# gabegrand/VQA-Counterexamples

Hardware: AMD Instinct MI355X
Metric: VQA-CX triplets/sec (24 candidates each), NeuralCX training step (higher is better)
Workload: dtype f32; 1 GPU; configs[1]: NeuralCX MLP train step (fwd+listwise loss/recall+bwd+Adam), synthetic 2048-d feats, 24 candidates, batch 512 per GPU (weak scaling: global batch 512), H=256, L=1, dropout 0.25, fp32; global_batch=512, per_rank_batch=512, candidates=24, dim_h=256, n_layers=1, parallelism=dp1, feature_table_rows=82783

## Files before the change

include/neuralcx.h:

```cpp
#ifndef NEURALCX_H
#define NEURALCX_H

#include <stddef.h>
#include <stdint.h>

#ifdef __cplusplus
extern "C" {
#endif

#define NCX_OK            0
#define NCX_E_NULL       -1
#define NCX_E_DIMS       -2
#define NCX_E_WORKSPACE  -3
#define NCX_E_FLAGS      -4
#define NCX_E_UNSUPPORTED -5
#define NCX_E_COMM       -6

#define NCX_F_V_MULT   (1u << 0)
#define NCX_F_V_DIST   (1u << 1)
#define NCX_F_V_RANK   (1u << 2)
#define NCX_F_A_EMB    (1u << 3)
#define NCX_F_ALL      (NCX_F_V_MULT | NCX_F_V_DIST | NCX_F_V_RANK | NCX_F_A_EMB)
#define NCX_F_BF16     (1u << 4)
#define NCX_F_REUSE_GT (1u << 5)
// ... 52 lines not shown
size_t ncx_workspace_bytes(const ncx_dims* d);

int ncx_forward(const ncx_dims* d, const ncx_inputs* in, const ncx_params* p,
                void* workspace, size_t workspace_bytes, float* scores, void* stream);

#define NCX_FWD_ALL     0
#define NCX_FWD_PRELUDE 1
#define NCX_FWD_REST    2
int ncx_forward_phase(const ncx_dims* d, const ncx_inputs* in, const ncx_params* p,
                      void* workspace, size_t workspace_bytes, float* scores, int32_t phase, void* stream);

int ncx_loss_rank(const float* scores, const int32_t* gt, int32_t B, int32_t K, float scale,
                  float* loss_rows, float* loss, float* dscores, int32_t* rank, int32_t* hits,
                  void* stream);

int ncx_backward(const ncx_dims* d, const ncx_inputs* in, const ncx_params* p,
                 void* workspace, size_t workspace_bytes, const float* dscores,
                 const ncx_grads* g, void* stream);

int ncx_backward_phase(const ncx_dims* d, const ncx_inputs* in, const ncx_params* p,
                       void* workspace, size_t workspace_bytes, const float* dscores,
                       const ncx_grads* g, int32_t phase, void* stream);

#define NCX_WS_DGT 1
#define NCX_WS_H1 2
#define NCX_WS_DPRE1 3
#define NCX_WS_DE_PERM 4
#define NCX_WS_H2 5
#define NCX_WS_H3 6
#define NCX_WS_DPRE2 7
#define NCX_WS_XC 8
#define NCX_WS_WC 9
#define NCX_WS_GT 10
int ncx_ws_region(const ncx_dims* d, int32_t which, size_t* offset, size_t* bytes);

int ncx_train_tail(const ncx_dims* d, const ncx_params* p, void* workspace, size_t workspace_bytes, const int32_t* gt,
                   float* scores, float* loss_rows, float* loss, float* dscores, int32_t* rank, int32_t* hits,
                   const ncx_grads* g, void* stream);

#define NCX_COMM_ID_BYTES 128
typedef struct ncx_comm ncx_comm;
int ncx_comm_unique_id(void* id128);
int ncx_comm_create(const void* id128, int32_t nranks, int32_t rank, ncx_comm** out);
int ncx_comm_destroy(ncx_comm* comm);
int ncx_allreduce(ncx_comm* comm, float* buf, size_t n, void* stream);

int ncx_adam_step(float* param, const float* grad, float* exp_avg, float* exp_avg_sq, size_t n,
                  float lr, float beta1, float beta2, float eps, int32_t step, float grad_scale,
                  void* stream);

typedef struct ncx_adam_state {
    float* param; const float* grad; float* exp_avg; float* exp_avg_sq;
    size_t n, n_emb;
    int32_t step;
    float lr, beta1, beta2, eps, grad_scale;
} ncx_adam_state;
int ncx_backward_adam(const ncx_dims* d, const ncx_inputs* in, const ncx_params* p,
                      void* workspace, size_t workspace_bytes, const float* dscores,
                      const ncx_grads* g, const ncx_adam_state* opt, void* stream);

typedef struct ncx_mutan_params {
    const float* wv;  const float* bv;
    const float* wq;  const float* bq;
    const float* whv; const float* bhv;
    const float* whq; const float* bhq;
    const float* wc;  const float* bc;
    int32_t dhv, dhq, R;
    int32_t act_v, act_q;
} ncx_mutan_params;

size_t ncx_vqa_workspace_bytes(const ncx_dims* d, const ncx_mutan_params* m);

int ncx_vqa_forward(const ncx_dims* d, const float* feats, const int32_t* img_idx, const float* q_emb,
                    const ncx_mutan_params* m, void* workspace, size_t workspace_bytes,
                    float* z_orig, float* z_knns, float* a_knns, float* a_orig, void* stream);

typedef struct ncx_mlb_params {
    const float* wv;  const float* bv;
    const float* wq;  const float* bq;
    const float* wc;  const float* bc;
    int32_t dh;
    int32_t act_v, act_q, act_c;
} ncx_mlb_params;

size_t ncx_mlb_workspace_bytes(const ncx_dims* d, const ncx_mlb_params* m);

int ncx_mlb_forward(const ncx_dims* d, const float* feats, const int32_t* img_idx, const float* q_emb,
                    const ncx_mlb_params* m, void* workspace, size_t workspace_bytes,
                    float* z_orig, float* z_knns, float* a_knns, float* a_orig, void* stream);

typedef struct ncx_mlb_att_dims {
    int32_t B, P, dv, dq, dh_att, G, dh_f, A, n_img;
} ncx_mlb_att_dims;
typedef struct ncx_mlb_att_params {
    const float* wv_att; const float* bv_att;
    const float* wq_att; const float* bq_att;
    const float* wa;     const float* ba;
    const float* wg;     const float* bg;
    const float* wqf;    const float* bqf;
    const float* wc;     const float* bc;
    int32_t act_v_att, act_q_att, act_mm;
    int32_t act_v, act_q, act_c;
} ncx_mlb_att_params;

size_t ncx_mlb_att_workspace_bytes(const ncx_mlb_att_dims* d, const ncx_mlb_att_params* m);

int ncx_mlb_att_forward(const ncx_mlb_att_dims* d, const float* feats, const int32_t* img_idx, const float* q_emb,
                        const ncx_mlb_att_params* m, void* workspace, size_t workspace_bytes,
                        float* logits, float* att, void* stream);
int ncx_mlb_att_forward_flags(const ncx_mlb_att_dims* d, const float* feats, const int32_t* img_idx, const float* q_emb,
                              const ncx_mlb_att_params* m, uint32_t flags, void* workspace, size_t workspace_bytes,
                              float* logits, float* att, void* stream);
int ncx_mlb_att_logits_form(const ncx_mlb_att_dims* d, uint32_t flags);

size_t ncx_knn_status_offset(int32_t n);
size_t ncx_knn_workspace_bytes(int32_t n, int32_t block_rows);
int ncx_knn(const float* table, int32_t n, const float* queries, int32_t nq, int32_t dv, int32_t k,
            int32_t norms_ready, void* workspace, size_t workspace_bytes, int64_t* out_idx, float* out_dist,
            void* stream);

size_t ncx_cosine_gram_workspace_bytes(int32_t A, int32_t da);
int ncx_cosine_gram(const float* emb, int32_t A, int32_t da, void* ws, size_t ws_bytes, float* gram, void* stream);
int ncx_semantic_scores(const float* a_knns, const int32_t* aid, int32_t B, int32_t K, int32_t A, const float* gram,
                        float lam, float* scores, float* raw, int32_t* bad_id_flag, void* stream);

int ncx_similarity_scores(const float* feats, const int32_t* img_idx, int32_t n_img, int32_t dv,
                          const float* z_orig, const float* z_knns, int32_t dz,
                          const float* a_knns, const int32_t* aid, int32_t A,
                          int32_t B, int32_t K,
                          float* scores , float* parts ,
                          int32_t* bad_id_flag, void* stream);

size_t ncx_gru_packed_bytes(int32_t dim_emb, int32_t dim_q);
int ncx_gru_pack(const float* w_ih, const float* w_hh, const float* b_ih, const float* b_hh, int32_t dim_emb, int32_t dim_q,
                 float* packed, void* stream);
size_t ncx_gru_workspace_bytes(int32_t B, int32_t T, int32_t dim_emb, int32_t dim_q);
int ncx_gru_encode(const int32_t* wids, int32_t B, int32_t T, const float* E, int32_t V1, int32_t dim_emb, int32_t dim_q,
                   const float* packed, void* workspace, size_t workspace_bytes, float* q_out, int32_t* bad_id_flag, void* stream);
int ncx_gru_encode_flags(const int32_t* wids, int32_t B, int32_t T, const float* E, int32_t V1, int32_t dim_emb, int32_t dim_q,
                         const float* packed, uint32_t flags, void* workspace, size_t workspace_bytes, float* q_out, int32_t* bad_id_flag,
                         void* stream);
int ncx_gru_step_form(int32_t B, int32_t T, int32_t dim_emb, int32_t dim_q, uint32_t flags);

size_t ncx_gru_train_workspace_bytes(int32_t B, int32_t T, int32_t dim_emb, int32_t dim_q);
size_t ncx_gru_packed_t_bytes(int32_t dim_emb, int32_t dim_q);
int ncx_gru_pack_t(const float* w_ih, const float* w_hh, int32_t dim_emb, int32_t dim_q, float* packed_t, void* stream);
int ncx_gru_train_forward(const int32_t* wids, int32_t B, int32_t T, const float* E, int32_t V1, int32_t dim_emb, int32_t dim_q,
                          const float* packed, void* workspace, size_t workspace_bytes, float* q_out, int32_t* bad_id_flag, void* stream);
int ncx_gru_train_forward_flags(const int32_t* wids, int32_t B, int32_t T, const float* E, int32_t V1, int32_t dim_emb, int32_t dim_q,
                                const float* packed, uint32_t flags, void* workspace, size_t workspace_bytes, float* q_out,
                                int32_t* bad_id_flag, void* stream);
int ncx_gru_train_backward(const int32_t* wids, int32_t B, int32_t T, const float* E, int32_t V1, int32_t dim_emb, int32_t dim_q,
                           const float* packed_t, void* workspace, size_t workspace_bytes, const float* dq_out,
                           float* dW_ih, float* dW_hh, float* db_ih, float* db_hh, float* dE , void* stream);
int ncx_gru_train_backward_flags(const int32_t* wids, int32_t B, int32_t T, const float* E, int32_t V1, int32_t dim_emb, int32_t dim_q,
                                 const float* packed_t, uint32_t flags, void* workspace, size_t workspace_bytes, const float* dq_out,
                                 float* dW_ih, float* dW_hh, float* db_ih, float* db_hh, float* dE , void* stream);
int ncx_gru_bwd_form(int32_t B, int32_t T, int32_t dim_emb, int32_t dim_q, uint32_t flags);

size_t ncx_lstm2_packed_bytes(int32_t emb, int32_t H);
int ncx_lstm2_pack(const float* w_ih0, const float* w_hh0, const float* b_ih0, const float* b_hh0, const float* w_ih1, const float* w_hh1,
                   const float* b_ih1, const float* b_hh1, int32_t emb, int32_t H, float* packed, void* stream);
size_t ncx_lstm2_workspace_bytes(int32_t B, int32_t T, int32_t emb, int32_t H);
int ncx_lstm2_encode(const int32_t* wids, int32_t B, int32_t T, const float* E, int32_t V1, int32_t emb, int32_t H, const float* packed,
                     void* workspace, size_t workspace_bytes, float* q_out, int32_t* bad_id_flag, void* stream);
int ncx_lstm2_encode_flags(const int32_t* wids, int32_t B, int32_t T, const float* E, int32_t V1, int32_t emb, int32_t H, const float* packed,
                           uint32_t flags, void* workspace, size_t workspace_bytes, float* q_out, int32_t* bad_id_flag, void* stream);
int ncx_lstm2_step_form(int32_t B, int32_t T, int32_t emb, int32_t H, uint32_t flags);

size_t ncx_lstm2_train_workspace_bytes(int32_t B, int32_t T, int32_t emb, int32_t H);
size_t ncx_lstm2_packed_t_bytes(int32_t emb, int32_t H);
int ncx_lstm2_pack_t(const float* w_ih0, const float* w_hh0, const float* w_ih1, const float* w_hh1, int32_t emb, int32_t H, float* packed_t,
                     void* stream);
int ncx_lstm2_train_forward(const int32_t* wids, int32_t B, int32_t T, const float* E, int32_t V1, int32_t emb, int32_t H, const float* packed,
                            void* workspace, size_t workspace_bytes, float* q_out, int32_t* bad_id_flag, void* stream);
int ncx_lstm2_train_forward_flags(const int32_t* wids, int32_t B, int32_t T, const float* E, int32_t V1, int32_t emb, int32_t H,
                                  const float* packed, uint32_t flags, void* workspace, size_t workspace_bytes, float* q_out,
                                  int32_t* bad_id_flag, void* stream);
int ncx_lstm2_train_backward(const int32_t* wids, int32_t B, int32_t T, const float* E, int32_t V1, int32_t emb, int32_t H, const float* packed_t,
                             void* workspace, size_t workspace_bytes, const float* dq_out, float* dW_ih0, float* dW_hh0, float* db_ih0,
                             float* db_hh0, float* dW_ih1, float* dW_hh1, float* db_ih1, float* db_hh1, float* dE , void* stream);

typedef struct ncx_scorer_dims {
    int32_t B, K, dv, dq, dz, A, n_img;
} ncx_scorer_dims;

typedef struct ncx_pairlin_params {
    const float* answer_embedding;
    const float* w;  const float* b;
    const float* w_out; const float* b_out;
} ncx_pairlin_params;
typedef struct ncx_pairlin_grads {
    float* answer_embedding; float* w; float* b; float* w_out; float* b_out;
} ncx_pairlin_grads;

size_t ncx_pairlin_workspace_bytes(const ncx_scorer_dims* d);
int ncx_pairlin_forward(const ncx_scorer_dims* d, const ncx_inputs* in, const ncx_pairlin_params* p, void* workspace,
                        size_t workspace_bytes, float* scores, int32_t* bad_id_flag, void* stream);
int ncx_pairlin_backward(const ncx_scorer_dims* d, const ncx_inputs* in, const ncx_pairlin_params* p, void* workspace,
                         size_t workspace_bytes, const float* dscores, const ncx_pairlin_grads* g, void* stream);
size_t ncx_linctx_workspace_bytes(const ncx_scorer_dims* d);
int ncx_linctx_forward(const ncx_scorer_dims* d, const float* z_knns, const float* w, const float* b, void* workspace,
                       size_t workspace_bytes, float* scores, void* stream);
int ncx_linctx_backward(const ncx_scorer_dims* d, const float* z_knns, const float* dscores, void* workspace,
                        size_t workspace_bytes, float* gw, float* gb, void* stream);

typedef struct ncx_contrastive_dims {
    int32_t B, P, dv, dz, n_img;
} ncx_contrastive_dims;
size_t ncx_contrastive_workspace_bytes(const ncx_contrastive_dims* d);
int ncx_contrastive_forward(const ncx_contrastive_dims* d, const ncx_inputs* in, const float* w, const float* b, void* workspace,
                            size_t workspace_bytes, float* h, int32_t* bad_id_flag, void* stream);
int ncx_contrastive_distances(const ncx_contrastive_dims* d, const float* h, void* workspace, size_t workspace_bytes, float* dist,
                              void* stream);
int ncx_contrastive_loss(const ncx_contrastive_dims* d, void* workspace, size_t workspace_bytes, float margin, float scale,
                         float* losses4, float* dist, void* stream);
int ncx_contrastive_backward(const ncx_contrastive_dims* d, const ncx_inputs* in, void* workspace, size_t workspace_bytes,
                             const float* dh, float* gw, float* gb, void* stream);

typedef struct ncx_vqa_train_dims {
    int32_t B, dv, dq, dz, A, n_img;
    float   p_v, p_q, p_c;
    int32_t dropout_mode;
    int32_t want_dq;
    int32_t pad_;
    uint64_t seed;
} ncx_vqa_train_dims;
typedef struct ncx_mutan_grads {
    float* wv;  float* bv;  float* wq;  float* bq;  float* whv; float* bhv; float* whq; float* bhq; float* wc;  float* bc;
} ncx_mutan_grads;
size_t ncx_vqa_train_workspace_bytes(const ncx_vqa_train_dims* d, const ncx_mutan_params* m);
int ncx_vqa_train_forward(const ncx_vqa_train_dims* d, const float* feats, const int32_t* img_idx, const float* q_emb,
                          const ncx_mutan_params* m, const float* masks, void* workspace, size_t workspace_bytes,
                          float* logits, float* z, void* stream);
int ncx_ce_loss(const float* logits, const int32_t* target, int32_t B, int32_t A, float scale, float* loss, float* dlogits,
                int32_t* hits_top1, int32_t* hits_top5, int32_t* bad_flag, float* rows, void* stream);
int ncx_vqa_train_backward(const ncx_vqa_train_dims* d, const ncx_mutan_params* m, const float* masks, void* workspace,
                           size_t workspace_bytes, const float* dlogits, const ncx_mutan_grads* g, float* dq_emb, void* stream);
#define NCX_VT_WS_VD 1
#define NCX_VT_WS_QD 2
#define NCX_VT_WS_ZC 3
int ncx_vqa_train_ws_region(const ncx_vqa_train_dims* d, const ncx_mutan_params* m, int32_t which, size_t* offset, size_t* bytes);

typedef struct ncx_mlb_grads {
    float* wv;  float* bv;  float* wq;  float* bq;  float* wc;  float* bc;
} ncx_mlb_grads;
size_t ncx_mlb_train_workspace_bytes(const ncx_vqa_train_dims* d, const ncx_mlb_params* m);
int ncx_mlb_train_forward(const ncx_vqa_train_dims* d, const float* feats, const int32_t* img_idx, const float* q_emb,
                          const ncx_mlb_params* m, const float* masks, void* workspace, size_t workspace_bytes,
                          float* logits, float* z, void* stream);
int ncx_mlb_train_backward(const ncx_vqa_train_dims* d, const ncx_mlb_params* m, const float* masks, void* workspace,
                           size_t workspace_bytes, const float* dlogits, const ncx_mlb_grads* g, float* dq_emb, void* stream);
int ncx_mlb_train_ws_region(const ncx_vqa_train_dims* d, const ncx_mlb_params* m, int32_t which, size_t* offset, size_t* bytes);

typedef struct ncx_mlb_att_train {
    float    p_att_v, p_att_q, p_att_mm, p_v, p_q, p_c;
    int32_t  dropout_mode;
    int32_t  want_dq;
    uint64_t seed;
} ncx_mlb_att_train;
typedef struct ncx_mlb_att_grads {
    float* wv_att; float* bv_att; float* wq_att; float* bq_att; float* wa; float* ba;
    float* wg;     float* bg;     float* wqf;    float* bqf;    float* wc; float* bc;
} ncx_mlb_att_grads;
size_t ncx_mlb_att_train_workspace_bytes(const ncx_mlb_att_dims* d, const ncx_mlb_att_train* t, const ncx_mlb_att_params* m);
int ncx_mlb_att_train_forward(const ncx_mlb_att_dims* d, const ncx_mlb_att_train* t, const float* feats, const int32_t* img_idx,
                              const float* q_emb, const ncx_mlb_att_params* m, const float* masks, void* workspace,
                              size_t workspace_bytes, float* logits, float* att, void* stream);
int ncx_mlb_att_train_forward_flags(const ncx_mlb_att_dims* d, const ncx_mlb_att_train* t, const float* feats, const int32_t* img_idx,
                                    const float* q_emb, const ncx_mlb_att_params* m, const float* masks, uint32_t flags, void* workspace,
                                    size_t workspace_bytes, float* logits, float* att, void* stream);
int ncx_mlb_att_train_backward(const ncx_mlb_att_dims* d, const ncx_mlb_att_train* t, const float* feats, const int32_t* img_idx,
                               const float* q_emb, const ncx_mlb_att_params* m, const float* masks, void* workspace,
                               size_t workspace_bytes, const float* att, const float* dlogits, const ncx_mlb_att_grads* g,
                               float* dq_emb, void* stream);
int ncx_mlb_att_train_backward_flags(const ncx_mlb_att_dims* d, const ncx_mlb_att_train* t, const float* feats, const int32_t* img_idx,
                                     const float* q_emb, const ncx_mlb_att_params* m, const float* masks, uint32_t flags, void* workspace,
                                     size_t workspace_bytes, const float* att, const float* dlogits, const ncx_mlb_att_grads* g,
                                     float* dq_emb, void* stream);
int ncx_mlb_att_dwv_form(const ncx_mlb_att_dims* d, uint32_t flags);
#define NCX_AT_WS_XV     1
#define NCX_AT_WS_VATT   2
#define NCX_AT_WS_T      3
#define NCX_AT_WS_VD     4
#define NCX_AT_WS_DWV    5
int ncx_mlb_att_train_ws_region(const ncx_mlb_att_dims* d, const ncx_mlb_att_train* t, const ncx_mlb_att_params* m, int32_t which,
                                size_t* offset, size_t* bytes);

#define NCX_GEMM_GT 0
#define NCX_GEMM_SH 1
#define NCX_GEMM_MAIN 2
#define NCX_GEMM_FWD_L 3
#define NCX_GEMM_DW1C 4
#define NCX_GEMM_DW1S 5
#define NCX_GEMM_DE 6
#define NCX_GEMM_DW1AK 7
#define NCX_GEMM_DAGT 8
#define NCX_GEMM_DWL 9
#define NCX_GEMM_DXL 10
#define NCX_QUERY_DW1_ROUTE 32
#define NCX_QUERY_FUSED_ADAM 33
#define NCX_QUERY_FWD_ROUTE 34
#define NCX_QUERY_BF16_ROUTE 35
int ncx_profile_begin(uint32_t gemm_mask , int32_t max_launches);
int ncx_profile_end(float* ms, int32_t* ids, int32_t cap);
int ncx_profile_stamps(unsigned long long* stamps, int64_t words);
int ncx_plan_query(const ncx_dims* d, int32_t gemm_id, int32_t* out6);
int ncx_bf16_layout(const ncx_dims* d, int32_t* out10);
int ncx_wgmap_check(int32_t tiles_m, int32_t tiles_n, int32_t S);

const char* ncx_version(void);

#ifdef __cplusplus
}
#endif
#endif
```

vqa-counterexamples_amd/csrc/ncx_diag.hip:

```cpp
#include "ncx_driver.h"
#include "ncx_bf16.h"
#include <stdlib.h>

using namespace ncx;
extern "C" {
int ncx_profile_begin(uint32_t gemm_mask, int32_t max_launches) {
    if (g_prof.on || gemm_mask == 0 || (gemm_mask >> U_COUNT) != 0 || max_launches < 1 || max_launches > 65536) return NCX_E_DIMS;
    g_prof.ev = (hipEvent_t*)malloc(sizeof(hipEvent_t) * 2 * (size_t)max_launches);
    g_prof.ids = (int*)malloc(sizeof(int) * (size_t)max_launches);
    if (!g_prof.ev || !g_prof.ids) return NCX_E_NULL;
    for (int i = 0; i < 2 * max_launches; ++i) NCX_HIP_TRY(hipEventCreate(&g_prof.ev[i]));
    g_prof.mask = gemm_mask; g_prof.n = 0; g_prof.cap = max_launches; g_prof.on = true;
    return NCX_OK;
}

int ncx_profile_end(float* ms, int32_t* ids, int32_t cap) {
    if (!g_prof.on) return NCX_E_FLAGS;
    int n = 0;
    for (int i = 0; i < g_prof.n; ++i) {
        if (hipEventSynchronize(g_prof.ev[2 * i + 1]) != hipSuccess) break;
        float t = 0.f;
        if (hipEventElapsedTime(&t, g_prof.ev[2 * i], g_prof.ev[2 * i + 1]) != hipSuccess) break;
        if (n < cap) { if (ms) ms[n] = t; if (ids) ids[n] = g_prof.ids[i]; }
        ++n;
    }
    for (int i = 0; i < 2 * g_prof.cap; ++i) (void)hipEventDestroy(g_prof.ev[i]);
    free(g_prof.ev); free(g_prof.ids);
    g_prof.ev = nullptr; g_prof.ids = nullptr; g_prof.on = false; g_prof.mask = 0; g_prof.n = 0; g_prof.cap = 0;
    return n < cap ? n : cap;
}

int ncx_profile_stamps(unsigned long long* stamps, int64_t words) {
    if ((stamps == nullptr) != (words == 0) || words < 0) return NCX_E_DIMS;
    int dev = 0;
    NCX_HIP_TRY(hipGetDevice(&dev));
    if (dev < 0 || dev >= 16) return NCX_E_DIMS;
    if (!stamps) { g_stamps[dev].ptr.store(nullptr, std::memory_order_release); g_stamps[dev].words.store(0, std::memory_order_release); }
    else { g_stamps[dev].ptr.store(nullptr, std::memory_order_release); g_stamps[dev].words.store(words, std::memory_order_release);
           g_stamps[dev].ptr.store(stamps, std::memory_order_release); }
    return NCX_OK;
}

int ncx_wgmap_check(int32_t tiles_m, int32_t tiles_n, int32_t S) {
    if (tiles_m < 1 || tiles_n < 1 || S < 1 || (long long)tiles_m * tiles_n * S > (1 << 24)) return NCX_E_DIMS;
    const WgMap w{tiles_m, tiles_n, S};
    const int total = tiles_m * tiles_n * S, count = w.count();
    if (count < total) return 1;
    unsigned char* seen = (unsigned char*)calloc((size_t)total, 1);
    if (!seen) return NCX_E_NULL;
    int bad = 0, nvalid = 0;
    for (int lw = 0; lw < count && !bad; ++lw) {
        int tm = -1, tn = -1, z = -1;
        if (!w.decode(lw, tm, tn, z)) continue;
        ++nvalid;
        if (tm < 0 || tm >= tiles_m || tn < 0 || tn >= tiles_n || z < 0 || z >= S) { bad = 2; break; }
        if (w.encode(tm, tn, z) != lw) { bad = 3; break; }
        unsigned char& f = seen[((size_t)z * tiles_m + tm) * tiles_n + tn];
        if (f) { bad = 4; break; }
        f = 1;
    }
    if (!bad && nvalid != total) bad = 5;
    free(seen);
    return bad;
}

int ncx_bf16_layout(const ncx_dims* d, int32_t* out10) {
    if (check_dims(d) != NCX_OK) return NCX_E_DIMS;
    if (!out10) return NCX_E_NULL;
    const Bf16Cols c = bf16_cols(*d);
    const int32_t v[10] = {c.c_vk, c.c_vm, c.c_misc, c.c_z, c.c_p, c.raw, c.kc, bf16_hp(*d), bf16_up128(d->da), bf16_up128(d->A)};
    for (int i = 0; i < 10; ++i) out10[i] = v[i];
    return NCX_OK;
}

int ncx_plan_query(const ncx_dims* d, int32_t gemm_id, int32_t* out6) {
    if (check_dims(d) != NCX_OK || !out6) return NCX_E_DIMS;
    if (gemm_id == NCX_QUERY_DW1_ROUTE) {
        const bool bf16 = d->flags & NCX_F_BF16;
        const StepRoutes r = routes(*d);
        out6[0] = r.km_form;
        out6[1] = (bf16 ? r.tn8_shared : r.tn8) ? (r.tn8_x6 ? 2 : 1) : 0;
        int grid = 0;
        out6[2] = dw_tn8_pieces(*d, bf16 ? TN8_LIST_SHARED : TN8_LIST_MAIN, &grid);
        out6[3] = grid;
        out6[4] = r.dw1ak_on_tn8(km_defers_to_side_stream(*d, r)) ? 1 : 0;
        out6[5] = TN8_MAX_SEG;
        return NCX_OK;
    }
    if (gemm_id == NCX_QUERY_FUSED_ADAM) {
        const bool on = fused_adam_route(*d, routes(*d)) && ((size_t)d->A * d->da) % 4 == 0;
        for (int i = 0; i < 6; ++i) out6[i] = 0;
        out6[0] = on ? 1 : 0;
        out6[1] = on ? main_adam_passengers() : 0;
        return NCX_OK;
    }
    if (gemm_id == NCX_QUERY_BF16_ROUTE) {
        for (int i = 0; i < 6; ++i) out6[i] = 0;
        if (!(d->flags & NCX_F_BF16)) { out6[0] = -1; return NCX_OK; }
        const Bf16Route b = bf16_route(*d);
        out6[0] = b.nt_form; out6[1] = b.tn8; out6[2] = b.S; out6[3] = b.chunk; out6[4] = b.nz; out6[5] = b.vec;
        return NCX_OK;
    }
    if (gemm_id == NCX_QUERY_FWD_ROUTE) {
        const StepRoutes r = routes(*d);
        GemmUse u[U_COUNT];
        list_uses(*d, r, u);
        const long long M = (long long)d->B * d->K;
        const bool bf16 = d->flags & NCX_F_BF16;
        for (int i = 0; i < 6; ++i) out6[i] = 0;
        if (bf16) out6[0] = 3;
        else if (main_fwd_dims_ok(*d)) {
            const FwdRoute f = forward_route(*d, r);
            const int sp = main_split(M, d->H, r.cand_ksteps);
            out6[0] = f.vfold ? 2 : 1;
            out6[1] = f.vfold ? main_fold_rows_eff(M, d->H, d->K) : main_chain_form(M, d->H, r.cand_ksteps, sp, false, true);
            out6[2] = sp;
            out6[3] = f.dist_in_main ? 1 : 0;
        } else { out6[1] = u[U_MAIN].plan.cfg; out6[2] = u[U_MAIN].plan.split; }
        if (d->L < 2) { out6[4] = -1; return NCX_OK; }
        if (hidden_fwd_dims_ok(*d) && !bf16) { out6[4] = 1; out6[5] = main_split(M, d->H, ksteps(d->H)); }
        else out6[5] = u[U_FWD_L].plan.split;
        return NCX_OK;
    }
    if (gemm_id < 0 || gemm_id >= U_COUNT) return NCX_E_DIMS;
    GemmUse u[U_COUNT];
    list_uses(*d, routes(*d), u);
    out6[0] = u[gemm_id].form; out6[1] = (int32_t)u[gemm_id].M; out6[2] = (int32_t)u[gemm_id].N;
    out6[3] = (int32_t)u[gemm_id].ksteps; out6[4] = u[gemm_id].plan.cfg; out6[5] = u[gemm_id].plan.split;
    const bool fast = (gemm_id == U_MAIN && main_fwd_dims_ok(*d)) || (gemm_id == U_FWD_L && hidden_fwd_dims_ok(*d) && !(d->flags & NCX_F_BF16));
    if (fast) {
        const long long M = (long long)d->B * d->K, T = u[gemm_id].ksteps;
        const int sp = main_split(M, d->H, T);
        const bool vfold = gemm_id == U_MAIN && (d->flags & NCX_F_V_MULT) && (d->K == 24 || (d->K == 48 && main_fold_rows(M, d->H) >= 96)) && d->dv % 32 == 0 && d->dv >= 64 && sp == 1;
        const long long tiles96 = ((M + 95) / 96) * ((d->H + 127) / 128);
        out6[4] = vfold ? (main_fold_rows(M, d->H) == 192 ? 8 : (main_fold_rows(M, d->H) == 96 || d->K == 48) ? 7 : 6) : (sp == 1 && tiles96 * 10 >= (long long)num_cus() * 9) ? CFG_96x128 : 5;
        out6[5] = sp;
    }
    return NCX_OK;
}
}
```

vqa-counterexamples_amd/csrc/ncx_forward.hip:

```cpp
#include "ncx_driver.h"
#include "ncx_wave.h"
#include "ncx_bf16.h"

namespace ncx {
__device__ __forceinline__ u16 f32_to_bf16(float x) { return __builtin_bit_cast(u16, (__bf16)x); }
__device__ __forceinline__ void store_bf16x4(u16* p, const float (&v)[4], int valid) {
    typedef unsigned short u16x4 __attribute__((ext_vector_type(4)));
    if (valid >= 4) { *(u16x4*)p = u16x4{f32_to_bf16(v[0]), f32_to_bf16(v[1]), f32_to_bf16(v[2]), f32_to_bf16(v[3])}; }
    else { for (int j = 0; j < valid; ++j) p[j] = f32_to_bf16(v[j]); }
}

struct PackArgs { const float* src[WPAD_N + 1]; float* dst[WPAD_N + 1]; long long lds[WPAD_N + 1]; int cols[WPAD_N + 1], ldd[WPAD_N + 1], zero_from[WPAD_N + 1]; int n, H; int nprep; };
__device__ __forceinline__ void pack_rows_block(const PackArgs& a, int idx) {
    const int h = idx % a.H, e = idx / a.H;
    float* drow = a.dst[e] + (long long)h * a.ldd[e];
    if (a.src[e]) {
        const float* srow = a.src[e] + (long long)h * a.lds[e];
        for (int c = threadIdx.x; c < a.cols[e]; c += 256) drow[c] = srow[c];
    }
    for (int c = a.zero_from[e] + threadIdx.x; c < a.ldd[e]; c += 256) drow[c] = 0.f;
}

template <bool RESIDENT>
__global__ __launch_bounds__(256) void k_prep(ncx_dims d, ncx_inputs in, int* __restrict__ idx_k,
                                              int* __restrict__ idx_o, int* __restrict__ idx_ob,
                                              float* __restrict__ mx, float* __restrict__ inv,
                                              float* __restrict__ misc, u16* __restrict__ xc, Bf16Cols cc, const PackArgs pk) {
    constexpr int NR = RESIDENT ? 8 : 1;
    const int lane = threadIdx.x & 63;
    const int M = d.B * d.K;
    const int nprep = pk.nprep;
    if ((int)blockIdx.x >= nprep) { pack_rows_block(pk, (int)blockIdx.x - nprep); return; }
    const int r = blockIdx.x * 4 + (threadIdx.x >> 6);
    if (r >= M) return;
    const int b = r / d.K, k = r - b * d.K;
    const bool aemb_ = d.flags & NCX_F_A_EMB;
    f32x4 ra[NR];
    if (RESIDENT && aemb_) {
        const float* arow = in.a_knns + (long long)r * d.A;
#pragma unroll
        for (int i = 0; i < NR; ++i) ra[i] = load_window(arow, lane * 4 + 256 * i, d.A);
    }
    const int io = in.img_idx[(long long)b * (d.K + 1)];
    const int ik = in.img_idx[(long long)b * (d.K + 1) + 1 + k];
    if (lane == 0) { idx_o[r] = io; idx_k[r] = ik; if (k == 0) idx_ob[b] = io; }
    const float* vo = in.feats + (long long)io * d.dv;
    const float* vk = in.feats + (long long)ik * d.dv;
    u16* xr = xc ? xc + (long long)r * cc.kc : nullptr;
    const bool own_dist = (d.flags & NCX_F_V_DIST) && !(d.flags & NCX_F_PRIV_DIST_IN_MAIN);
    const bool need_v = own_dist || xc;

    f32x4 ro[NR], rk[NR];
    if (RESIDENT && need_v) {
#pragma unroll
        for (int i = 0; i < NR; ++i) { ro[i] = load_window(vo, lane * 4 + 256 * i, d.dv); rk[i] = load_window(vk, lane * 4 + 256 * i, d.dv); }
        if (d.dv % 256 != 0) {
#pragma unroll
            for (int i = 0; i < NR; ++i) { ro[i] = fix_window(ro[i], lane * 4 + 256 * i, d.dv); rk[i] = fix_window(rk[i], lane * 4 + 256 * i, d.dv); }
        }
    }
    auto v_at = [&](int i, int c, f32x4& a, f32x4& e) __attribute__((always_inline)) {
        if (RESIDENT) { a = ro[i]; e = rk[i]; } else { a = load4(vo, c, d.dv); e = load4(vk, c, d.dv); }
    };
    float dist = 0.f;
    if (own_dist) {
        float s = 0.f;
        if (RESIDENT) {
#pragma unroll
            for (int i = 0; i < NR; ++i) {
                const int c = lane * 4 + 256 * i;
#pragma unroll
                for (int j = 0; j < 4; ++j)
                    if (c + j < d.dv) { const float t = ro[i][j] - rk[i][j] + 1e-6f; s += t * t; }
            }
        } else {
            for (int c = lane * 4; c < d.dv; c += 256) {
                f32x4 a, e; v_at(0, c, a, e);
#pragma unroll
                for (int j = 0; j < 4; ++j)
                    if (c + j < d.dv) { const float t = a[j] - e[j] + 1e-6f; s += t * t; }
            }
        }
        dist = sqrtf(wave_sum(s));
    }
    const int mw = pad_to(d.K + 1, 4);
    float* mrow = misc + (long long)r * mw;
    if (lane == 0) mrow[0] = dist;
    for (int j = lane; j < mw - 1; j += 64)
        mrow[1 + j] = j >= d.K ? 0.f : (d.flags & NCX_F_V_RANK) ? (j == k ? 1.f : 0.f) : in.v_rank[((long long)r) * d.K + j];
    if (xc) {
        if (RESIDENT) {
#pragma unroll
            for (int i = 0; i < NR; ++i) {
                const int c = lane * 4 + 256 * i;
                if (c < cc.c_vm) {
                    float pk[4], pm[4];
#pragma unroll
                    for (int j = 0; j < 4; ++j) { pk[j] = rk[i][j]; pm[j] = ro[i][j] * rk[i][j]; }
                    store_bf16x4(xr + cc.c_vk + c, pk, 4);
                    store_bf16x4(xr + cc.c_vm + c, pm, 4);
                }
            }
        } else {
            for (int c = lane * 4; c < cc.c_vm; c += 256) {
                f32x4 a, e; v_at(0, c, a, e);
                float pk[4], pm[4];
#pragma unroll
                for (int j = 0; j < 4; ++j) { pk[j] = e[j]; pm[j] = a[j] * e[j]; }
                store_bf16x4(xr + cc.c_vk + c, pk, 4);
                store_bf16x4(xr + cc.c_vm + c, pm, 4);
            }
        }
        for (int j = lane; j < cc.c_z - cc.c_misc; j += 64)
            xr[cc.c_misc + j] = f32_to_bf16(j == 0 ? dist : (j <= d.K && j - 1 == k ? 1.f : 0.f));
        const float* zk = in.z_knns + (long long)r * d.dz;
        for (int c = lane * 4; c < cc.c_p - cc.c_z; c += 256) {
            float pz[4];
            const f32x4 z4 = load4(zk, c, d.dz);
#pragma unroll
            for (int j = 0; j < 4; ++j) pz[j] = z4[j];
            store_bf16x4(xr + cc.c_z + c, pz, 4);
        }
        for (int c = cc.raw + lane; c < cc.kc; c += 64) xr[c] = 0;
    }

    if (d.flags & NCX_F_A_EMB) {
        const float* a = in.a_knns + (long long)r * d.A;
        if (RESIDENT && d.A % 256 != 0) {
#pragma unroll
            for (int i = 0; i < NR; ++i) ra[i] = fix_window(ra[i], lane * 4 + 256 * i, d.A);
        }
        float m = -INFINITY;
        if (RESIDENT) {
#pragma unroll
            for (int i = 0; i < NR; ++i)
#pragma unroll
                for (int j = 0; j < 4; ++j) if (lane * 4 + 256 * i + j < d.A) m = fmaxf(m, ra[i][j]);
        } else {
            for (int c = lane * 4; c < d.A; c += 256) {
                const f32x4 v = load4(a, c, d.A);
#pragma unroll
                for (int j = 0; j < 4; ++j) if (c + j < d.A) m = fmaxf(m, v[j]);
            }
        }
        m = wave_max(m);
        float s = 0.f;
        if (RESIDENT) {
#pragma unroll
            for (int i = 0; i < NR; ++i)
#pragma unroll
                for (int j = 0; j < 4; ++j) if (lane * 4 + 256 * i + j < d.A) s += __expf(ra[i][j] - m);
        } else {
            for (int c = lane * 4; c < d.A; c += 256) {
                const f32x4 v = load4(a, c, d.A);
#pragma unroll
                for (int j = 0; j < 4; ++j) if (c + j < d.A) s += __expf(v[j] - m);
            }
        }
        s = wave_sum(s);
        const float lse2 = m * 1.44269504088896341f + __log2f(s);
        if (lane == 0) { mx[r] = lse2; inv[r] = 0.f; }
        if (xc) {
            u16* xp = xr + cc.c_p;
            if (RESIDENT) {
#pragma unroll
                for (int i = 0; i < NR; ++i) {
                    const int c = lane * 4 + 256 * i;
                    if (c < d.A) {
                        float e[4];
#pragma unroll
                        for (int j = 0; j < 4; ++j) e[j] = __builtin_amdgcn_exp2f(__builtin_fmaf(ra[i][j], 1.44269504088896341f, -lse2));
                        store_bf16x4(xp + c, e, d.A - c);
                    }
                }
            } else {
                for (int c = lane * 4; c < d.A; c += 256) {
                    const f32x4 v = load4(a, c, d.A);
                    float e[4];
#pragma unroll
                    for (int j = 0; j < 4; ++j) e[j] = __builtin_amdgcn_exp2f(__builtin_fmaf(v[j], 1.44269504088896341f, -lse2));
                    store_bf16x4(xp + c, e, d.A - c);
                }
            }
        }
    }
}

__global__ __launch_bounds__(256) void k_scores(const float* __restrict__ h, const float* __restrict__ w,
                                                const float* __restrict__ bias, float* __restrict__ scores,
                                                int M, int H) {
    const int lane = threadIdx.x & 63;
    const int r = blockIdx.x * 4 + (threadIdx.x >> 6);
    if (r >= M) return;
    const float* row = h + (long long)r * H;
    float s = 0.f;
    for (int c = lane * 4; c < H; c += 256) {
        const f32x4 a = load4(row, c, H), e = load4(w, c, H);
        s += dot4(a, e);
    }
    s = wave_sum(s);
    if (lane == 0) scores[r] = s + bias[0];
}

FwdRoute forward_route(const ncx_dims& d, const StepRoutes& r) {
    const long long M = (long long)d.B * d.K, H = d.H, din = seg_offsets(d).din;
    const long long main_T = r.cand_ksteps;
    FwdRoute f{};
    f.vfold = main_fwd_dims_ok(d) && (d.flags & NCX_F_V_MULT) && (d.K == 24 || (d.K == 48 && (main_fold_rows(M, H) >= 96 || hook_env("NCX_FOLD4") || hook_env("NCX_FOLD8")))) && d.dv % 32 == 0 && d.dv >= 64 &&
              main_split(M, H, main_T) == 1 && !hook_env("NCX_NO_VFOLD") &&
              (long long)d.n_img * d.dv * 4 < (1ll << 32) - 65536 && (long long)H * din * 4 < (1ll << 32) - 65536;
    f.dist_in_fold = f.vfold && d.K == 24 && main_fold_rows_eff(M, H, d.K) >= 96 && !(d.flags & NCX_F_X6) && hook_env("NCX_DIST_IN_FOLD");
    f.dist_in_main = main_fwd_dims_ok(d) && (d.flags & NCX_F_V_DIST) && (d.flags & NCX_F_V_MULT) && d.dv % 32 == 0 &&
                     main_split(M, H, main_T) == 1 && (!f.vfold || f.dist_in_fold) && !(hook_env("NCX_NO_DIST_IN_MAIN"));
    return f;
}
}

using namespace ncx;
extern "C" {
const char* ncx_version(void) { return "neuralcx-hip gfx950 fp32-mfma r4 (" __DATE__ ")"; }

int64_t ncx_input_size(const ncx_dims* d) { return d ? (int64_t)seg_offsets(*d).din : 0; }

size_t ncx_workspace_bytes(const ncx_dims* d) {
    if (check_dims(d) != NCX_OK) return 0;
    return ws_layout(*d).total;
}

static int forward_impl(const ncx_dims* dp, const ncx_inputs* in, const ncx_params* p, void* workspace,
                        size_t workspace_bytes, float* scores, void* stream_, int phase) {
    int rc = check_dims(dp);
    if (rc != NCX_OK) return rc;
    const bool do_pre = phase != 2, do_rest = phase != 1;
    if (!in || !p || !workspace || (do_rest && !scores && !(dp->flags & NCX_F_FUSED_TAIL))) return NCX_E_NULL;
    const ncx_dims& d = *dp;
    const bool aemb = d.flags & NCX_F_A_EMB;
    if (!in->feats || !in->img_idx || !in->q_emb || !in->z_orig || !in->z_knns || !in->a_knns) return NCX_E_NULL;
    if (aemb && (!in->answer_aids || !p->answer_embedding)) return NCX_E_NULL;
    if (!aemb && !in->a_emb_gt) return NCX_E_FLAGS;
    if (!(d.flags & NCX_F_V_RANK) && !in->v_rank) return NCX_E_FLAGS;
    if (!p->w1 || !p->b1 || !p->w_out || !p->b_out) return NCX_E_NULL;
    if (d.L >= 2 && (!p->w2 || !p->b2)) return NCX_E_NULL;
    if (d.L >= 3 && (!p->w3 || !p->b3)) return NCX_E_NULL;
    const StepRoutes r = routes(d);
    const WsLayout w = ws_layout(d, r);
    if (workspace_bytes < w.total || ((uintptr_t)workspace & 255)) return NCX_E_WORKSPACE;
    hipStream_t s = (hipStream_t)stream_;
    char* ws = (char*)workspace;
    const int M = d.B * d.K, H = d.H;
    const SegOffsets o = seg_offsets(d);
    const long long din = o.din;
    int* idx_k = (int*)(ws + w.idx_k); int* idx_o = (int*)(ws + w.idx_o); int* idx_ob = (int*)(ws + w.idx_ob);
    float* mx = (float*)(ws + w.mx); float* inv = (float*)(ws + w.inv); float* misc = (float*)(ws + w.misc);
    float* gt = (float*)(ws + w.gt); float* sh = (float*)(ws + w.sh); float* slab = (float*)(ws + w.slab);
    GemmUse u[U_COUNT];
    list_uses(d, r, u);

    SideStream* ss = side_stream();
    if (ss && ss->mode == 3) ss = nullptr;
    hipStream_t s2 = ss ? ss->s : s;
    float* slab_side = ss ? (float*)(ws + w.slab2) : slab;
    const size_t slab_side_bytes = ss ? w.slab2_bytes : w.slab_bytes;
    if (ss) { rc = side_fork(ss, s); if (rc) return rc; }
    const bool bf16 = d.flags & NCX_F_BF16;
    u16* xc = bf16 ? (u16*)(ws + w.xc) : nullptr;
    struct { const float* ptr[WPAD_N]; int width[WPAD_N]; } wp{};
    PackArgs pk{}; pk.H = H;
    {
        const float* srcs[WPAD_N] = {p->w1 + o.v_other, p->w1 + o.v_mult, p->w1 + o.v_dist, p->w1 + o.z_other, p->w1 + o.a_other, p->w2, p->w3};
        float* cur = (float*)(ws + w.wpad);
        for (int i = 0; i < WPAD_N; ++i) {
            wp.width[i] = wpad_width(d, i); wp.ptr[i] = cur;
            if (!wp.width[i]) continue;
            const int e = pk.n++;
            pk.src[e] = srcs[i]; pk.lds[e] = (i == 5 || i == 6) ? H : din; pk.cols[e] = wpad_cols(d, i); pk.dst[e] = cur; pk.ldd[e] = wp.width[i]; pk.zero_from[e] = pk.cols[e];
            cur += (size_t)H * wp.width[i];
        }
        if (aemb && w.ldgt > d.A) { const int e = pk.n++; pk.src[e] = nullptr; pk.dst[e] = gt; pk.ldd[e] = w.ldgt; pk.zero_from[e] = d.A; pk.cols[e] = 0; }
        if (d.flags & NCX_F_REUSE_GT) pk.n = 0;
    }
    const FwdRoute fr = forward_route(d, r);
    const bool vfold = fr.vfold, dist_in_main = fr.dist_in_main;
    ncx_dims dprep = d;
    if (dist_in_main) dprep.flags |= NCX_F_PRIV_DIST_IN_MAIN;
    if (!do_rest) pk.n = 0;
    pk.nprep = do_pre ? (int)cdiv(M, 4) : 0;
    const unsigned prep_grid = (unsigned)(pk.nprep + (long long)H * pk.n);
    if (prep_grid > 0) {
        if (d.dv <= 2048 && d.A <= 2048)
            hipLaunchKernelGGL(k_prep<true>, dim3(prep_grid), dim3(256), 0, s, dprep, *in, idx_k, idx_o, idx_ob, mx, inv, misc, xc, bf16_cols(d), pk);
        else
            hipLaunchKernelGGL(k_prep<false>, dim3(prep_grid), dim3(256), 0, s, dprep, *in, idx_k, idx_o, idx_ob, mx, inv, misc, xc, bf16_cols(d), pk);
        NCX_HIP_TRY(hipGetLastError());
    }
    if (!do_rest) {
        if (ss) { rc = side_join(ss, s); if (rc) return rc; }
        return NCX_OK;
    }

    FixupArgs fix_gt{}, fix_sh{};
    const bool merge_fix = !ss && !bf16 && aemb && !(d.flags & NCX_F_REUSE_GT) && u[U_GT].plan.cfg == u[U_SH].plan.cfg &&
                           !hook_env("NCX_NO_MERGE_FIX");
    if (aemb && bf16 && !(d.flags & NCX_F_REUSE_GT)) {
        const Bf16Emb m = bf16_emb_layout(d, ws + w.bf_emb);
        rc = bf16_pack_embedding(d, p->answer_embedding, p->w1, m, s2); if (rc) return rc;
        rc = profiled(U_GT, s2, [&] { return bf16_gt(d, m, gt, s2); }); if (rc) return rc;
    } else if (aemb && !(d.flags & NCX_F_REUSE_GT)) {
        GemmArgs a{}; a.mode = MODE_CHAIN; a.nseg = 1; a.M = H;
        a.a[0] = x_plain(p->w1 + o.a_other, din, H, d.da);
        a.b[0] = x_plain(p->answer_embedding, d.da, d.A, d.da);
        a.klen[0] = d.da; a.out[0] = gt; a.ldo[0] = w.ldgt; a.n_cols[0] = d.A;
        if (merge_fix) a.defer_fix = &fix_gt;
        rc = run_gemm(U_GT, a, FORM_NT, u[U_GT].plan, merge_fix ? (float*)(ws + w.slab2) : slab_side,
                      merge_fix ? w.slab2_bytes : slab_side_bytes, nullptr, s2);
        if (rc) return rc;
    }
    {
        GemmArgs a{}; a.mode = MODE_CHAIN; a.nseg = 4; a.M = d.B;
        a.a[0] = ss ? x_gather_strided(in->feats, d.dv, in->img_idx, d.K + 1, d.B, d.dv)
                    : x_gather(in->feats, d.dv, idx_ob, d.B, d.dv);
        a.b[0] = x_plain(p->w1 + o.v_orig, din, H, d.dv); a.klen[0] = d.dv;
        a.a[1] = x_plain(in->q_emb, d.dq, d.B, d.dq);            a.b[1] = x_plain(p->w1 + o.q_emb, din, H, d.dq);  a.klen[1] = d.dq;
        a.a[2] = x_plain(in->z_orig, d.dz, d.B, d.dz);           a.b[2] = x_plain(p->w1 + o.z_orig, din, H, d.dz); a.klen[2] = d.dz;
        a.a[3] = aemb ? x_gather(p->answer_embedding, d.da, in->answer_aids, d.B, d.da)
                      : x_plain(in->a_emb_gt, d.da, d.B, d.da);
        a.b[3] = x_plain(p->w1 + o.a_gt, din, H, d.da); a.klen[3] = d.da;
        a.out[0] = sh; a.ldo[0] = H; a.n_cols[0] = H;
        if (merge_fix) a.defer_fix = &fix_sh;
        rc = run_gemm(U_SH, a, FORM_NT, u[U_SH].plan, slab_side, slab_side_bytes, p->b1, s2);
        if (rc) return rc;
        if (merge_fix) { rc = run_fixup2(fix_gt, fix_sh, u[U_SH].plan.cfg, s); if (rc) return rc; }
        if (ss) { rc = side_join(ss, s); if (rc) return rc; }
    }
    if (bf16) {
        rc = bf16_pack_wc(d, p->w1, gt, (u16*)(ws + w.wc), s); if (rc) return rc;
        EpiArgs e{};
        e.rowadd = sh; e.ld_rowadd = H; e.rowdiv = d.K;
        set_dropout(e, d, *in, 1, M);
        rc = profiled(U_MAIN, s, [&] { return bf16_main_forward(d, xc, (const u16*)(ws + w.wc), e, (float*)(ws + w.h[0]), s); }); if (rc) return rc;
    } else if (main_fwd_dims_ok(d)) {
        MainArgs a{}; a.M = M; a.N = H; a.x6 = (d.flags & NCX_F_X6) && !hook_env("NCX_NO_X6") && !hook_env("NCX_NO_MAIN_X6");
        int n = 0;
        auto seg = [&](int kind, const float* x, long long lda, int klen, const int* i1, const int* i2, const float* lse, int slot, const float* wgt, long long ldb) {
            MainSeg& g = a.seg[n++]; g.kind = kind; g.a = x; g.lda = lda; g.idx = i1; g.idx2 = i2; g.lse = lse; g.klen = klen;
            if (slot >= 0 && wp.width[slot]) { g.b = wp.ptr[slot]; g.ldb = wp.width[slot]; } else { g.b = wgt; g.ldb = ldb; } };
        if (vfold) {
            seg(MK_VFOLD, in->feats, d.dv, d.dv, idx_k, idx_o, nullptr, -1, p->w1 + o.v_other, din);
            a.seg[0].b2 = p->w1 + o.v_mult;
        } else {
            seg(MK_GATHER, in->feats, d.dv, d.dv, idx_k, nullptr, nullptr, 0, p->w1 + o.v_other, din);
            if (d.flags & NCX_F_V_MULT) seg(MK_GATHER_MUL, in->feats, d.dv, d.dv, idx_k, idx_o, nullptr, 1, p->w1 + o.v_mult, din);
        }
        seg(MK_PLAIN, misc, w.ldm, w.ldm, nullptr, nullptr, nullptr, 2, p->w1 + o.v_dist, din);
        seg(MK_PLAIN, in->z_knns, d.dz, d.dz, nullptr, nullptr, nullptr, 3, p->w1 + o.z_other, din);
        if (aemb) seg(MK_SOFTMAX, in->a_knns, d.A, d.A, nullptr, nullptr, mx, -1, gt, w.ldgt);
        else      seg(MK_PLAIN, in->a_knns, d.da, d.da, nullptr, nullptr, nullptr, 4, p->w1 + o.a_other, din);
        a.nseg = n;
        a.out = (float*)(ws + w.h[0]); a.ldo = H;
        a.epi.rowadd = sh; a.epi.ld_rowadd = H; a.epi.rowdiv = d.K;
        set_dropout(a.epi, d, *in, 1, M);
        if (dist_in_main) { a.dist_out = misc; a.ld_dist = w.ldm; }
        {
            long long T = 0; for (int i = 0; i < n; ++i) T += ksteps(a.seg[i].klen);
            a.split = main_split(M, H, T); a.slab = (float*)(ws + w.mslab);
            if (a.split > 1 && (size_t)a.split * M * H * 4 > w.mslab_bytes) return NCX_E_WORKSPACE;
        }
        if (a.split <= 1) a.stamps = stamps_for_current_device((long long)(((M + 47) / 48 + 7) / 8 * 8) * ((H + 63) / 64) * 16);
        rc = profiled(U_MAIN, s, [&] { return main_forward(a, s); }); if (rc) return rc;
    } else {
        GemmArgs a{}; a.mode = MODE_CHAIN; a.M = M;
        int n = 0;
        a.a[n] = x_gather(in->feats, d.dv, idx_k, M, d.dv); a.b[n] = x_plain(p->w1 + o.v_other, din, H, d.dv); a.klen[n] = d.dv; ++n;
        if (d.flags & NCX_F_V_MULT) {
            a.a[n] = x_gather_mul(in->feats, d.dv, idx_k, idx_o, M, d.dv); a.b[n] = x_plain(p->w1 + o.v_mult, din, H, d.dv); a.klen[n] = d.dv; ++n;
        }
        a.a[n] = x_plain(misc, w.ldm, M, d.K + 1); a.b[n] = x_plain(p->w1 + o.v_dist, din, H, d.K + 1); a.klen[n] = d.K + 1; ++n;
        a.a[n] = x_plain(in->z_knns, d.dz, M, d.dz); a.b[n] = x_plain(p->w1 + o.z_other, din, H, d.dz); a.klen[n] = d.dz; ++n;
        if (aemb) { a.a[n] = x_softmax(in->a_knns, d.A, mx, inv, M, d.A); a.b[n] = x_plain(gt, w.ldgt, H, d.A); a.klen[n] = d.A; ++n; }
        else      { a.a[n] = x_plain(in->a_knns, d.da, M, d.da); a.b[n] = x_plain(p->w1 + o.a_other, din, H, d.da); a.klen[n] = d.da; ++n; }
        a.nseg = n;
        a.out[0] = (float*)(ws + w.h[0]); a.ldo[0] = H; a.n_cols[0] = H;
        a.epi.rowadd = sh; a.epi.ld_rowadd = H; a.epi.rowdiv = d.K;
        set_dropout(a.epi, d, *in, 1, M);
        rc = run_gemm(U_MAIN, a, FORM_NT, u[U_MAIN].plan, slab, w.slab_bytes, nullptr, s);
        if (rc) return rc;
    }
    for (int l = 2; l <= d.L; ++l) {
        const float* wl = l == 2 ? p->w2 : p->w3;
        const float* bl = l == 2 ? p->b2 : p->b3;
        if (hidden_fwd_dims_ok(d) && !bf16) {
            MainArgs a{}; a.M = M; a.N = H; a.nseg = 1;
            MainSeg& g = a.seg[0]; g.kind = MK_PLAIN; g.a = (const float*)(ws + w.h[l - 2]); g.lda = H; g.klen = H;
            const int slot = 3 + l;
            if (wp.width[slot]) { g.b = wp.ptr[slot]; g.ldb = wp.width[slot]; } else { g.b = wl; g.ldb = H; }
            a.out = (float*)(ws + w.h[l - 1]); a.ldo = H;
            a.epi.bias = bl;
            set_dropout(a.epi, d, *in, l, M);
            a.split = main_split(M, H, ksteps(H)); a.slab = (float*)(ws + w.mslab);
            if (a.split > 1 && (size_t)a.split * M * H * 4 > w.mslab_bytes) return NCX_E_WORKSPACE;
            rc = profiled(U_FWD_L, s, [&] { return main_forward(a, s); }); if (rc) return rc;
        } else {
            GemmArgs a{}; a.mode = MODE_CHAIN; a.nseg = 1; a.M = M;
            a.a[0] = x_plain((const float*)(ws + w.h[l - 2]), H, M, H); a.b[0] = x_plain(wl, H, H, H); a.klen[0] = H;
            a.out[0] = (float*)(ws + w.h[l - 1]); a.ldo[0] = H; a.n_cols[0] = H;
            a.epi.bias = bl;
            set_dropout(a.epi, d, *in, l, M);
            rc = run_gemm(U_FWD_L, a, FORM_NT, u[U_FWD_L].plan, slab, w.slab_bytes, nullptr, s);
            if (rc) return rc;
        }
    }
    if (d.flags & NCX_F_FUSED_TAIL) return NCX_OK;
    hipLaunchKernelGGL(k_scores, dim3((unsigned)cdiv(M, 4)), dim3(256), 0, s, (const float*)(ws + w.h[d.L - 1]),
                       p->w_out, p->b_out, scores, M, H);
    NCX_HIP_TRY(hipGetLastError());
    return NCX_OK;
}

int ncx_forward(const ncx_dims* dp, const ncx_inputs* in, const ncx_params* p, void* workspace,
                size_t workspace_bytes, float* scores, void* stream_) {
    return forward_impl(dp, in, p, workspace, workspace_bytes, scores, stream_, 0);
}

int ncx_forward_phase(const ncx_dims* dp, const ncx_inputs* in, const ncx_params* p, void* workspace,
                      size_t workspace_bytes, float* scores, int32_t phase, void* stream_) {
    if (phase < 0 || phase > 2) return NCX_E_FLAGS;
    return forward_impl(dp, in, p, workspace, workspace_bytes, scores, stream_, phase);
}
}
```

vqa-counterexamples_amd/csrc/ncx_internal.h:

```cpp
#pragma once
#include "ncx_common.h"
#include "ncx_gemm.h"
#include "ncx_adam.h"

namespace ncx {

enum TileCfg : int { CFG_64x64 = 0, CFG_128x128 = 1, CFG_96x128 = 2, CFG_96x64 = 3, CFG_128x64 = 4 };
enum GemmForm : int { FORM_NT = 0, FORM_TN = 1, FORM_NN = 2 };

int run_gemm_nt(GemmArgs& a, int cfg, hipStream_t s);
int run_fixup2(const FixupArgs& a, const FixupArgs& b, int cfg, hipStream_t s);
int run_gemm_nt_fold(GemmArgs& a, hipStream_t s);
int run_gemm_tn(GemmArgs& a, int cfg, hipStream_t s);
int run_gemm_nn(GemmArgs& a, int cfg, hipStream_t s);
int occupancy_nt(int cfg);
int occupancy_tn(int cfg);
int occupancy_nn(int cfg);

struct SegOffsets {
    int v_orig, v_other, v_mult, v_dist, v_rank, q_emb, z_orig, z_other, a_gt, a_other, din;
};
static inline SegOffsets seg_offsets(const ncx_dims& d) {
    SegOffsets o; int c = 0;
    o.v_orig = c;  c += d.dv;
    o.v_other = c; c += d.dv;
    o.v_mult = c;  c += d.dv;
    o.v_dist = c;  c += 1;
    o.v_rank = c;  c += d.K;
    o.q_emb = c;   c += d.dq;
    o.z_orig = c;  c += d.dz;
    o.z_other = c; c += d.dz;
    o.a_gt = c;    c += d.da;
    o.a_other = c; c += d.da;
    o.din = c;
    return o;
}

struct GemmPlan { int cfg; int split; };
GemmPlan plan_gemm(int form, long long M, long long N, long long ksteps, bool allow_96);
int num_cus();
static inline long long cdiv(long long a, long long b) { return (a + b - 1) / b; }
static inline long long ksteps(long long k) { return cdiv(k, GEMM_BK); }
__attribute__((visibility("hidden"))) size_t gemm_slab_bytes(GemmArgs a, const GemmPlan& pl);
__attribute__((visibility("hidden"))) int run_gemm_planned(GemmArgs& a, int form, const GemmPlan& pl, float* slab, size_t slab_bytes,
                                                           const float* reduce_bias, hipStream_t s);
__attribute__((visibility("hidden"))) hipError_t colsum_rows(const float* in, long long ld, int R, int cols, float* out, hipStream_t s);

struct WsLayout {
    size_t idx_k, idx_o, idx_ob;
    size_t mx, inv;
    size_t misc;
    size_t gt;
    size_t sh;
    size_t h[3];
    size_t dpre[2];
    size_t dsh;
    size_t dgt;
    size_t dagt;
    size_t dgtT;
    size_t dgtT2;
    size_t de_perm;
    size_t w1aT;
    size_t partial;
    size_t slab;
    size_t slab_bytes;
    size_t slab2, slab2_bytes;
    size_t xc, wc, dpre_bf, bf_slab;
    size_t bf_emb;
    size_t km_slab;
    size_t mslab, mslab_bytes;
    size_t wpad;
    int ldm;
    int ldgt;
    size_t total;
};
constexpr int NCX_COLSUM_CHUNKS = 256;
constexpr int NCX_PRELUDE_WAVES = 1024;

enum MainKind : int { MK_PLAIN = 0, MK_GATHER = 1, MK_GATHER_MUL = 2, MK_SOFTMAX = 3,
                      MK_VFOLD = 4 };
constexpr int MAIN_MAX_SEG = 5;
struct MainSeg {
    const float* a;
    const int*   idx;
    const int*   idx2;
    const float* lse;
    const float* b;
    const float* b2;
    long long lda, ldb;
    int kind, klen;
};
struct MainArgs {
    MainSeg seg[MAIN_MAX_SEG]; int nseg, M, N, split; float* out; long long ldo; EpiArgs epi;
    float* slab;
    float* dist_out; long long ld_dist;
    unsigned long long* stamps;
    int x6;
    float* t_out; float* t_out0;
    AdamFuse adam;
};
int main_forward(MainArgs& a, hipStream_t s);
int main_forward_rowmap(MainArgs& a, hipStream_t s);
bool main_short_form(long long M, long long N, long long T, int split);
int main_chain_form(long long M, long long N, long long T, int split, bool single_gather, bool wide_ok);
int main_forward_adam(MainArgs& a, bool rowmap, hipStream_t s);
int main_adam_passengers();
int main_forward_mlb(MainArgs& a, hipStream_t s);
int main_split(long long M, long long N, long long T);
int main_fold_rows_eff(long long M, long long N, int rowdiv);
int main_fold_rows(long long M, long long N);

constexpr int DW_KM_SPLIT = 8;
bool dw_km_supported(const ncx_dims& d);
enum DwKmForm : int { KM_FORM_NONE = 0, KM_FORM_8 = 1, KM_FORM_X6 = 2, KM_FORM_GENERIC = 3, KM_FORM_GROUPED = 4 };
int dw_km_form(const ncx_dims& d);
size_t dw_km_slab_bytes(const ncx_dims& d);
int dw_km(const ncx_dims& d, const float* dpre, const float* feats, const int* idx_k, const int* idx_o, float* slab,
          float* g_vother, float* g_vmult, long long din, hipStream_t s, bool finish = true);
int dw_km_finish(const ncx_dims& d, const float* slab, float* g_vother, float* g_vmult, long long din, const FixupArgs* fix, int fix_cfg,
                 hipStream_t s);
constexpr int TN8_MAX_PROB = 8;
constexpr int TN8_MAX_SEG = 16;
struct Tn8Prob {
    const float* A;
    const float* X; long long ldx;
    const float* lse;
    int gsel;
    int rows, N;
    float* out; long long ldo; int n_valid;
    int rows_valid;
    float* outT; float* outT2; long long ldT; int padT2;
};
bool dw_tn8_supported(const ncx_dims& d);
bool dw_tn8_shapes_ok(const ncx_dims& d);
bool dw_tn8_shared_ok(const ncx_dims& d);
enum Tn8List : int { TN8_LIST_MAIN = 0, TN8_LIST_SHARED = 1, TN8_LIST_AK = 2 };
int dw_tn8_pieces(const ncx_dims& d, int list, int* grid);
bool dw_tn8_x6(const ncx_dims& d);
size_t dw_tn8_slab_bytes(const ncx_dims& d);
int dw_tn8(const ncx_dims& d, const Tn8Prob* probs, int np, int n_al, bool do_al, bool do_rest, const int* idx_ob, const int* aid,
           float* slab, size_t slab_bytes, hipStream_t s);
bool mutan_fold_supported(const ncx_dims& d, const ncx_mutan_params& m);
int mutan_fold(const ncx_dims& d, const ncx_mutan_params& m, const float* xv, const float* hq, float* z_orig, float* z_knns, hipStream_t s);
__attribute__((visibility("hidden"))) hipError_t pad_rows(const float* src, long long ld_src, int cols, float* dst, int ldd, int rows, hipStream_t s);
WsLayout ws_layout(const ncx_dims& d);
__host__ __device__ static inline int pad_to(int x, int m) { return (x + m - 1) / m * m; }
static inline bool main_fwd_extents_ok(const ncx_dims& d) {
    const long long lim = (1ll << 32) - 65536, M = (long long)d.B * d.K, wa = d.A > d.da ? d.A : d.da;
    return (long long)d.n_img * d.dv * 4 < lim && M * wa * 4 < lim && M * (long long)d.H * 4 < lim && M * (long long)d.dz * 4 < lim && (long long)d.A * wa * 4 < lim &&
           (long long)d.H * (2ll * d.dv + d.dq + 2ll * d.dz + 2ll * d.da + d.K + 2) * 4 < lim;
}
static inline bool main_fwd_dims_ok(const ncx_dims& d) {
    return d.dv % 4 == 0 && d.dz % 4 == 0 && ((d.flags & NCX_F_A_EMB) ? d.A : d.da) % 4 == 0 && !(d.flags & NCX_F_BF16) && main_fwd_extents_ok(d);
}
static inline bool hidden_fwd_dims_ok(const ncx_dims& d) { return d.H % 4 == 0 && main_fwd_extents_ok(d); }
constexpr uint32_t NCX_F_PRIV_DIST_IN_MAIN = 1u << 30;


}
```

vqa-counterexamples_amd/csrc/ncx_main.h:

```cpp
#pragma once
#include "ncx_internal.h"
#include "ncx_adam.h"
#include "ncx_x6.h"
#include <type_traits>

namespace ncx {

constexpr int MF_BK = 32, MF_P = MF_BK + 4, MF_T = 256;

enum { LK_PLAIN = 0, LK_MUL = 1, LK_SOFTMAX = 2 };
template <int V> struct IntC { static constexpr int value = V; };

constexpr int MF6_P = 80;
template <int BM_, int BN_, int WGM_, int WGN_, int DEPTH_, int OCC_, int T_ = MF_T, bool X6_ = false>
struct MainCfg {
    static constexpr int BM = BM_, BN = BN_, WGM = WGM_, WGN = WGN_, DEPTH = DEPTH_, OCC = OCC_, T = T_;
    static constexpr bool X6 = X6_;
    static constexpr int EPI = 0;
    static constexpr bool ADAM = false;
    static constexpr int RP = T / 8;
    static constexpr int BM_LDS = (BM + RP - 1) / RP * RP;
    static constexpr int LDS6 = 2 * 3 * (BM_LDS + BN) * MF6_P;
    static constexpr int LDS_FOLD6 = 2 * (3 * 208 * MF6_P + 8 * 32 * 4 + 128 * MF_P * 4);
    static constexpr int LDS_LOOP = 2 * (BM_LDS + BN) * MF_P * 4;
    static constexpr int LDS_STAGE = BM * (BN + 4) * 4;
    static constexpr int LDS32 = LDS_LOOP > LDS_STAGE ? LDS_LOOP : LDS_STAGE;
    static constexpr int LDS = !X6_ ? LDS32 : (LDS_FOLD6 > LDS6 ? (LDS_FOLD6 > LDS32 ? LDS_FOLD6 : LDS32) : (LDS6 > LDS32 ? LDS6 : LDS32));
    static constexpr int LDS_FOLD = BM % 96 == 0 ? 2 * (32 * (T / 64) + 128) * MF_P * 4
                                                 : 2 * (80 + 2 * 64) * MF_P * 4;
};

enum { EPI_STD = 0, EPI_MLB = 1, EPI_ROWMAP = 2 };
template <class CFG> struct WithMlbEpi : CFG { static constexpr int EPI = EPI_MLB; };
template <class CFG> struct WithRowMap : CFG { static constexpr int EPI = EPI_ROWMAP; };
template <class CFG> struct WithAdam : CFG { static constexpr bool ADAM = true; };

typedef const __attribute__((address_space(1))) float* gfptr;
typedef const __attribute__((address_space(1))) int* giptr;
typedef const __attribute__((address_space(1))) f32x4u* gf4ptr;

template <class CFG, bool DIST, int K0, int K1 = -1, int K2 = -1, int K3 = -1, int K4 = -1>
__global__ __launch_bounds__(CFG::T, CFG::OCC) void k_main_fwd(const MainArgs args) {
    constexpr bool VFOLD = K0 == MK_VFOLD;
    constexpr int DIST_SEG = VFOLD ? 1 : 2;
    static_assert(!DIST || (VFOLD ? K1 == MK_PLAIN : (K1 == MK_GATHER_MUL && K2 == MK_PLAIN)), "DIST: v_o, v_k segment followed by the dist | rank segment");
    static_assert(!VFOLD || (CFG::BM == 48 && CFG::BN == 64 && CFG::WGM == 1 && CFG::WGN == 4 && CFG::DEPTH == 2) ||
                            (CFG::BM == 96 && CFG::BN == 64 && CFG::WGM == 2 && CFG::WGN == 2 && CFG::DEPTH == 2) ||
                            (CFG::BM == 192 && CFG::BN == 64 && CFG::T == 512 && CFG::WGM == 4 && CFG::WGN == 2 && CFG::DEPTH == 2), "fold: 48 x 64, 96 x 64 or (8 waves) 192 x 64 tiles");
    static_assert(!(DIST && CFG::X6), "the X6 form leaves the distance to k_prep");
    constexpr int KS[6] = {K0, K1, K2, K3, K4, -1};
    constexpr int NSEG = K1 < 0 ? 1 : K2 < 0 ? 2 : K3 < 0 ? 3 : K4 < 0 ? 4 : 5;
    constexpr int BM = CFG::BM, BN = CFG::BN, BK = MF_BK, P = MF_P, DEPTH = CFG::DEPTH, BML = CFG::BM_LDS;
    constexpr int WTM = BM / CFG::WGM, WTN = BN / CFG::WGN, WM = WTM / 16, WN = WTN / 16, NSUB = BK / 8, NMF = 2 * WM * WN;
    constexpr int MT = CFG::T, RP = CFG::RP;
    static_assert(CFG::WGM * CFG::WGN == MT / 64 && WTM % 16 == 0 && WTN % 16 == 0 && BN % RP == 0 && NSUB == 4, "tile");
    static_assert(MT == 256 || !VFOLD || BM % 96 == 0, "the 48-row fold is a 256-thread form");
    constexpr int NA = BML / RP, NB = BN / RP;
    extern __shared__ __attribute__((aligned(16))) float mf_smem[];
    float* const lds_a = mf_smem;
    float* const lds_b = mf_smem + 2 * BML * P;
    const int tid = threadIdx.x, lane = tid & 63, wave = tid >> 6, li = lane & 15, lk = lane >> 4;
    const int wm0 = (wave / CFG::WGN) * WTM, wn0 = (wave % CFG::WGN) * WTN;
    const int M = args.M, N = args.N;
    const int tiles_m = (M + BM - 1) / BM, tiles_n = (N + BN - 1) / BN;
    const int S = args.split > 1 ? args.split : 1;
    int bid = blockIdx.x;
    if constexpr (CFG::ADAM) {
        const int pa = args.adam.pass_at, np = args.adam.n_pass;
        if (bid >= pa && bid < pa + np) { adam_passenger(args.adam, bid - pa, tid, MT); return; }
        if (bid >= pa + np) bid -= np;
    }
    const int id = bid, xcd = id & 7, local = id >> 3;
    const int tn = local % tiles_n, unit = (local / tiles_n) * 8 + xcd;
    if (unit >= tiles_m * S) return;
    const int tm = unit / S, z = unit - tm * S;
    const int m0 = tm * BM, n0 = tn * BN;
    const int quad = tid & 7, trow = tid >> 3;
    unsigned long long* const stamps = args.stamps ? args.stamps + (size_t)blockIdx.x * 16 : nullptr;
    auto stamp = [&](int slot) __attribute__((always_inline)) {
        if (stamps && tid == 0) stamps[slot] = __builtin_readcyclecounter();
    };
    if (stamps && tid == 0) { stamps[14] = __builtin_amdgcn_s_memrealtime(); stamps[13] = __builtin_amdgcn_s_getreg((3 << 11) | (0 << 6) | 20); }
    stamp(0);

    f32x4 acc[WM][WN];
#pragma unroll
    for (int i = 0; i < WM; ++i)
#pragma unroll
        for (int j = 0; j < WN; ++j) acc[i][j] = f32x4{0.f, 0.f, 0.f, 0.f};
    f32x2 afA[WM], bfA[WN], afB[WM], bfB[WN];
#pragma unroll
    for (int i = 0; i < WM; ++i) afB[i] = f32x2{0.f, 0.f};
#pragma unroll
    for (int j = 0; j < WN; ++j) bfB[j] = f32x2{0.f, 0.f};

    auto read_frags = [&](int buf, int s, f32x2 (&af)[WM], f32x2 (&bf)[WN]) __attribute__((always_inline)) {
        const float* a = lds_a + buf * BML * P + (wm0 + li) * P + 8 * s + 2 * lk;
        const float* b = lds_b + buf * BN * P + (wn0 + li) * P + 8 * s + 2 * lk;
#pragma unroll
        for (int i = 0; i < WM; ++i) af[i] = *(const f32x2*)(a + i * 16 * P);
#pragma unroll
        for (int j = 0; j < WN; ++j) bf[j] = *(const f32x2*)(b + j * 16 * P);
    };
    auto mfma = [&](const f32x2 (&af)[WM], const f32x2 (&bf)[WN]) __attribute__((always_inline)) {
#pragma unroll
        for (int e = 0; e < 2; ++e)
#pragma unroll
            for (int i = 0; i < WM; ++i)
#pragma unroll
                for (int j = 0; j < WN; ++j) acc[i][j] = __builtin_amdgcn_mfma_f32_16x16x4f32(af[i][e], bf[j][e], acc[i][j], 0, 0, 0);
    };

    constexpr bool X6 = CFG::X6;
    static_assert(!X6 || (VFOLD && BM == 192 && WM == 3 && WN == 2 && DEPTH == 2), "X6: the 8-wave 192 x 64 fold form only");
    constexpr int P6 = MF6_P, A6_PL = BML * P6, PL6 = (BML + BN) * P6, BUF6 = 3 * PL6;
    unsigned char* const lds6 = (unsigned char*)mf_smem;
    x6_bf16x8 xa[2][3], xb[2][X6 ? WN : 1][3];
    auto read_a6 = [&](int buf, int i, x6_bf16x8 (&f)[3]) __attribute__((always_inline)) {
        const unsigned char* a = lds6 + buf * BUF6 + (wm0 + 16 * i + li) * P6 + 16 * lk;
#pragma unroll
        for (int p = 0; p < 3; ++p) f[p] = *(const x6_bf16x8*)(a + p * PL6);
    };
    auto read_b6 = [&](int buf, x6_bf16x8 (&f)[X6 ? WN : 1][3]) __attribute__((always_inline)) {
        const unsigned char* b = lds6 + buf * BUF6 + A6_PL + (wn0 + li) * P6 + 16 * lk;
#pragma unroll
        for (int j = 0; j < (X6 ? WN : 1); ++j)
#pragma unroll
            for (int p = 0; p < 3; ++p) f[j][p] = *(const x6_bf16x8*)(b + j * 16 * P6 + p * PL6);
    };
    auto mfma6 = [&](const x6_bf16x8 (&a)[3], const x6_bf16x8 (&b)[X6 ? WN : 1][3], f32x4 (&c)[WN]) __attribute__((always_inline)) {
        if constexpr (X6) {
#pragma unroll
            for (int q = 0; q < 6; ++q)
#pragma unroll
                for (int j = 0; j < WN; ++j) c[j] = __builtin_amdgcn_mfma_f32_16x16x32_bf16(a[X6_A[q]], b[j][X6_B[q]], c[j], 0, 0, 0);
        }
    };

    int nsteps[MAIN_MAX_SEG], total_steps = 0;
#pragma unroll
    for (int i = 0; i < MAIN_MAX_SEG; ++i) { nsteps[i] = i < NSEG ? (args.seg[i].klen + BK - 1) / BK : 0; total_steps += nsteps[i]; }
    constexpr bool ROWMAP = CFG::EPI == EPI_ROWMAP;
    static_assert(!ROWMAP || (K0 == MK_GATHER && K1 == MK_GATHER && NSEG == 2 && !DIST && !X6), "row map: two gathered segments");
    const int g0 = (int)((long long)total_steps * z / S), g1_all = (int)((long long)total_steps * (z + 1) / S);
    const int g1 = [&]() __attribute__((always_inline)) {
        if constexpr (ROWMAP) return m0 >= ((giptr)args.seg[0].idx)[M] ? min(g1_all, nsteps[0]) : g1_all;
        else return g1_all;
    }();

    f32x4 va[DEPTH][NA], vm[DEPTH][NA], vb[DEPTH][NB];
    typedef unsigned int bu32x4 __attribute__((ext_vector_type(4)));
    __amdgpu_buffer_rsrc_t rsPA = __builtin_amdgcn_make_buffer_rsrc((void*)nullptr, 0, 0, 0x00020000), rsPB = rsPA;
    unsigned roA[NA], roM[NA], roB[NB]; float lse[NA];
    float dacc[NA];
    constexpr int FOLD_DIST_OFF = 2 * (BML + BN) * P > 32 * (MT / 64) * 68 ? 2 * (BML + BN) * P : 32 * (MT / 64) * 68;
#pragma unroll
    for (int i = 0; i < NA; ++i) dacc[i] = 0.f;
    auto setup = [&](auto kind_c, const MainSeg& g) __attribute__((always_inline)) {
        constexpr int KIND = decltype(kind_c)::value;
#pragma unroll
        for (int i = 0; i < NA; ++i) {
            const int r = min(m0 + min(trow + RP * i, BM - 1), M - 1);
            constexpr bool GAT = KIND == MK_GATHER || KIND == MK_GATHER_MUL;
            const unsigned row = GAT ? (unsigned)((giptr)g.idx)[r] : (unsigned)r;
            roA[i] = row * (unsigned)(g.lda * 4);
            roM[i] = KIND == MK_GATHER_MUL ? (unsigned)((giptr)g.idx2)[r] * (unsigned)(g.lda * 4) : roA[i];
            lse[i] = KIND == MK_SOFTMAX ? ((gfptr)g.lse)[r] : 0.f;
        }
#pragma unroll
        for (int i = 0; i < NB; ++i) roB[i] = (unsigned)min(n0 + trow + RP * i, N - 1) * (unsigned)(g.ldb * 4) + 16u * quad;
        rsPA = __builtin_amdgcn_make_buffer_rsrc(const_cast<float*>(g.a), 0, 0xFFFFFFF0u, 0x00020000);
        rsPB = __builtin_amdgcn_make_buffer_rsrc(const_cast<float*>(g.b), 0, 0xFFFFFFF0u, 0x00020000);
    };
    auto issue = [&](auto set_c, auto mul_c, int klen, int nst, int t) __attribute__((always_inline)) {
        constexpr int S = decltype(set_c)::value;
        const int tk4 = min(t, nst - 1) * (BK * 4);
        const unsigned ca4 = (unsigned)min(tk4 + 16 * quad, (klen - 4) * 4);
#pragma unroll
        for (int i = 0; i < NA; ++i) va[S][i] = __builtin_bit_cast(f32x4, (bu32x4)__builtin_amdgcn_raw_buffer_load_b128(rsPA, roA[i] + ca4, 0, 0));
        if (decltype(mul_c)::value) {
#pragma unroll
            for (int i = 0; i < NA; ++i) vm[S][i] = __builtin_bit_cast(f32x4, (bu32x4)__builtin_amdgcn_raw_buffer_load_b128(rsPA, roM[i] + ca4, 0, 0));
        }
#pragma unroll
        for (int i = 0; i < NB; ++i) vb[S][i] = __builtin_bit_cast(f32x4, (bu32x4)__builtin_amdgcn_raw_buffer_load_b128(rsPB, roB[i], tk4, 0));
    };
    typedef IntC<0> S0; typedef IntC<DEPTH - 1> S1;
    typedef std::true_type Tt; typedef std::false_type Ff;

    auto run_seg = [&](auto idx_c, const int t0, const int t1, const bool pf_next) __attribute__((always_inline)) {
        constexpr int I = decltype(idx_c)::value;
        constexpr int KIND = KS[I], NKIND = KS[I + 1];
        constexpr int LKIND = KIND == MK_GATHER_MUL ? LK_MUL : KIND == MK_SOFTMAX ? LK_SOFTMAX : LK_PLAIN;
        typedef std::integral_constant<bool, LKIND == LK_MUL> MULC;
        const MainSeg& sg = args.seg[I];
        const int klen = sg.klen;
        const int nst = (klen + BK - 1) / BK;
        float lse_c[NA];
#pragma unroll
        for (int i = 0; i < NA; ++i) lse_c[i] = lse[i];
        auto stash = [&](auto set_c, auto patch_c, int buf, int h0, int h1) __attribute__((always_inline)) {
            constexpr int S = decltype(set_c)::value;
            constexpr bool PATCH = decltype(patch_c)::value;
#pragma unroll
            for (int i = 0; i < NA; ++i) {
                if (i < h0 || i >= h1) continue;
                f32x4 v = va[S][i];
                if (DIST && LKIND == LK_MUL) {
                    const f32x4 df = vm[S][i] - va[S][i] + 1e-6f;
                    dacc[i] += (df[0] * df[0] + df[1] * df[1]) + (df[2] * df[2] + df[3] * df[3]);
                }
                if (PATCH) v[0] = quad == 0 ? dacc[i] : v[0];
                if (LKIND == LK_MUL) v = v * vm[S][i];
                if (LKIND == LK_SOFTMAX) {
#pragma unroll
                    for (int j = 0; j < 4; ++j) v[j] = __builtin_amdgcn_exp2f(__builtin_fmaf(v[j], 1.44269504088896341f, -lse_c[i]));
                }
                if constexpr (X6) x6_split_store(v, lds6 + buf * BUF6 + (trow + RP * i) * P6 + 8 * quad, PL6);
                else
                *(f32x4*)(lds_a + buf * BML * P + (trow + RP * i) * P + 4 * quad) = v;
            }
#pragma unroll
            for (int i = 0; i < NB; ++i) {
                if (i + NA < h0 || i + NA >= h1) continue;
                if constexpr (X6) x6_split_store(vb[S][i], lds6 + buf * BUF6 + A6_PL + (trow + RP * i) * P6 + 8 * quad, PL6);
                else
                *(f32x4*)(lds_b + buf * BN * P + (trow + RP * i) * P + 4 * quad) = vb[S][i];
            }
        };
        if constexpr (DIST && I == DIST_SEG) {
#pragma unroll
            for (int i = 0; i < NA; ++i) {
                if constexpr (VFOLD && BM % 96 == 0) {
                    dacc[i] = mf_smem[FOLD_DIST_OFF + min(trow + RP * i, BM - 1)];
                } else {
                float d2 = dacc[i];
                d2 += __shfl_xor(d2, 1, 64); d2 += __shfl_xor(d2, 2, 64); d2 += __shfl_xor(d2, 4, 64);
                dacc[i] = sqrtf(d2);
                }
                const int r = m0 + trow + RP * i;
                if (quad == 0 && tn == 0 && trow + RP * i < BM && r < M) args.dist_out[(long long)r * args.ld_dist] = dacc[i];
            }
            stash(S0{}, Tt{}, 0, 0, NA + NB);
        } else
        stash(S0{}, Ff{}, 0, 0, NA + NB);
        issue(S0{}, MULC{}, klen, nst, t0 + DEPTH);
        __syncthreads();

        auto step = [&](auto par_c, auto last_c, int t) __attribute__((always_inline)) {
            constexpr int PAR = decltype(par_c)::value;
            constexpr bool LAST = decltype(last_c)::value;
            typedef IntC<DEPTH == 2 ? (PAR ^ 1) : 0> SS;
            if constexpr (X6) {
                read_b6(PAR, xb[PAR]);
                read_a6(PAR, 0, xa[PAR]);
                mfma6(xa[PAR ^ 1], xb[PAR ^ 1], acc[2]);
#pragma unroll
                for (int q = 0; q < 6 * WN; ++q) { __builtin_amdgcn_sched_group_barrier(0x008, 1, 0); __builtin_amdgcn_sched_group_barrier(0x100, 1, 0); }
                __builtin_amdgcn_sched_barrier(0);
                if (LAST && NKIND >= 0 && pf_next) {
                    const MainSeg& nx = args.seg[I + 1 < MAIN_MAX_SEG ? I + 1 : I];
                    setup(IntC<NKIND>{}, nx);
                    const int kn = nx.klen, nn = (kn + BK - 1) / BK;
                    typedef std::integral_constant<bool, NKIND == MK_GATHER_MUL> NM;
                    issue(S0{}, NM{}, kn, nn, 0);
                    issue(S1{}, NM{}, kn, nn, 1);
                }
#pragma unroll
                for (int i = 0; i < 2; ++i) {
                    read_a6(PAR, i + 1, xa[PAR ^ 1 ^ i]);
                    if (!LAST) {
                        if (i == 0) stash(SS{}, Ff{}, PAR ^ 1, 0, (NA + NB) / 2);
                        if (i == 1) { stash(SS{}, Ff{}, PAR ^ 1, (NA + NB) / 2, NA + NB); issue(SS{}, MULC{}, klen, nst, t + 1 + DEPTH); }
                    }
                    mfma6(xa[PAR ^ i], xb[PAR], acc[i]);
#pragma unroll
                    for (int q = 0; q < 6 * WN; ++q) {
                        __builtin_amdgcn_sched_group_barrier(0x008, 1, 0);
                        __builtin_amdgcn_sched_group_barrier(0x100, 1, 0);
                        __builtin_amdgcn_sched_group_barrier(0x002, 4, 0);
                        __builtin_amdgcn_sched_group_barrier(0x200, 1, 0);
                        __builtin_amdgcn_sched_group_barrier(0x020, 1, 0);
                    }
                    __builtin_amdgcn_sched_barrier(0);
                }
                if (LAST) {
                    mfma6(xa[PAR], xb[PAR], acc[2]);
                    const x6_bf16x8 z8 = {0, 0, 0, 0, 0, 0, 0, 0};
#pragma unroll
                    for (int p = 0; p < 3; ++p) { xa[0][p] = z8; xa[1][p] = z8; }
                }
                __syncthreads();
                return;
            }
            read_frags(PAR, 0, afA, bfA);
            mfma(afB, bfB);
#pragma unroll
            for (int q = 0; q < NMF; ++q) { __builtin_amdgcn_sched_group_barrier(0x008, 1, 0); __builtin_amdgcn_sched_group_barrier(0x100, 1, 0); }
            __builtin_amdgcn_sched_barrier(0);
            if (LAST && NKIND >= 0 && pf_next) {
                const MainSeg& nx = args.seg[I + 1 < MAIN_MAX_SEG ? I + 1 : I];
                setup(IntC<NKIND>{}, nx);
                const int kn = nx.klen, nn = (kn + BK - 1) / BK;
                typedef std::integral_constant<bool, NKIND == MK_GATHER_MUL> NM;
                issue(S0{}, NM{}, kn, nn, 0);
                if (DEPTH == 2) issue(S1{}, NM{}, kn, nn, 1);
            }
#pragma unroll
            for (int s = 0; s < NSUB - 1; ++s) {
                auto& afc = (s & 1) ? afB : afA; auto& bfc = (s & 1) ? bfB : bfA;
                auto& afn = (s & 1) ? afA : afB; auto& bfn = (s & 1) ? bfA : bfB;
                read_frags(PAR, s + 1, afn, bfn);
                if (!LAST) {
                    if (s == 0) stash(SS{}, Ff{}, PAR ^ 1, 0, (NA + NB) / 2);
                    if (s == 1) stash(SS{}, Ff{}, PAR ^ 1, (NA + NB) / 2, NA + NB);
                    if (s == 2) issue(SS{}, MULC{}, klen, nst, t + 1 + DEPTH);
                }
                mfma(afc, bfc);
#pragma unroll
                for (int q = 0; q < NMF; ++q) {
                    __builtin_amdgcn_sched_group_barrier(0x008, 1, 0);
                    __builtin_amdgcn_sched_group_barrier(0x100, 1, 0);
                    __builtin_amdgcn_sched_group_barrier(0x002, 4, 0);
                    __builtin_amdgcn_sched_group_barrier(0x200, 1, 0);
                    __builtin_amdgcn_sched_group_barrier(0x020, 1, 0);
                }
                __builtin_amdgcn_sched_barrier(0);
            }
            __syncthreads();
        };
        typedef IntC<0> P0; typedef IntC<1> P1;
        int t = t0;
        for (; t + 2 < t1; t += 2) { step(P0{}, Ff{}, t); step(P1{}, Ff{}, t + 1); }
        if (t + 1 < t1) { step(P0{}, Ff{}, t); step(P1{}, Tt{}, t + 1); }
        else step(P0{}, Tt{}, t);
    };

    auto run_vfold = [&](const MainSeg& sg, const bool pf_next) __attribute__((always_inline)) {
        constexpr int AR = 80;
        float* const fa = mf_smem;
        float* const fb = mf_smem + 2 * AR * P;
        const int klen = sg.klen, nst = klen / BK;
        const int wr = wave >> 1, wc = wave & 1;
        gfptr pk[2], pwk[2], pwm[2], po[2];
        int lrow[2];
#pragma unroll
        for (int i = 0; i < 2; ++i) {
            const int rho = trow + 32 * i;
            const int r = min(m0 + min(rho, BM - 1), M - 1);
            pk[i] = (gfptr)sg.a + (long long)((giptr)sg.idx)[r] * sg.lda;
            lrow[i] = rho < 24 ? rho : rho < 48 ? rho + 8 : 64 + (rho - 48);
            const int n = min(n0 + trow + 32 * i, N - 1);
            pwk[i] = (gfptr)sg.b + (long long)n * sg.ldb;
            pwm[i] = (gfptr)sg.b2 + (long long)n * sg.ldb;
            po[i] = (gfptr)sg.a + (long long)((giptr)sg.idx2)[min(m0 + 24 * i, M - 1)] * sg.lda;
        }
        const int t_of0 = trow < 24 ? 0 : 1;
        f32x4 vk[2][2], vo[2][2], vwk[2][2], vwm[2][2];
        auto vissue = [&](auto set_c, int t) __attribute__((always_inline)) {
            constexpr int S = decltype(set_c)::value;
            const int c = min(t, nst - 1) * BK + 4 * quad;
#pragma unroll
            for (int i = 0; i < 2; ++i) {
#ifndef NCX_ABL_FOLD
                vk[S][i] = *(gf4ptr)(pk[i] + c); vo[S][i] = *(gf4ptr)(po[i] + c); vwk[S][i] = *(gf4ptr)(pwk[i] + c); vwm[S][i] = *(gf4ptr)(pwm[i] + c);
#else
                if (NCX_ABL_FOLD != 4 || t == 0) vk[S][i] = *(gf4ptr)(pk[i] + c);
                if (NCX_ABL_FOLD != 2 || t == 0) vo[S][i] = *(gf4ptr)(po[i] + c);
                if (NCX_ABL_FOLD != 3 || t == 0) vwk[S][i] = *(gf4ptr)(pwk[i] + c);
                if ((NCX_ABL_FOLD != 3 && NCX_ABL_FOLD != 1) || t == 0) vwm[S][i] = *(gf4ptr)(pwm[i] + c);
#endif
            }
        };
        auto vstash = [&](auto set_c, int buf, int part) __attribute__((always_inline)) {
            constexpr int S = decltype(set_c)::value;
            if (part == 0) {
#pragma unroll
                for (int i = 0; i < 2; ++i) {
                    if (DIST) {
                        const f32x4 ov = i == 0 ? (t_of0 == 0 ? vo[S][0] : vo[S][1]) : vo[S][1];
                        const f32x4 df = ov - vk[S][i] + 1e-6f;
                        dacc[i] += (df[0] * df[0] + df[1] * df[1]) + (df[2] * df[2] + df[3] * df[3]);
                    }
                    *(f32x4*)(fa + buf * AR * P + lrow[i] * P + 4 * quad) = vk[S][i];
                }
            }
#pragma unroll
// ... 228 lines not shown
                    __builtin_amdgcn_sched_group_barrier(0x100, 1, 0);
                    __builtin_amdgcn_sched_group_barrier(0x002, DIST ? 4 : 3, 0);
                    __builtin_amdgcn_sched_group_barrier(0x200, 1, 0);
                    __builtin_amdgcn_sched_group_barrier(0x020, 1, 0);
                }
                __builtin_amdgcn_sched_barrier(0);
            }
            __syncthreads();
        };
        int t = 0;
        for (; t + 2 < nst; t += 2) { vstep(V0{}, Ff{}, t); vstep(V1{}, Ff{}, t + 1); }
        if (t + 1 < nst) { vstep(V0{}, Ff{}, t); vstep(V1{}, Tt{}, t + 1); }
        else vstep(V0{}, Tt{}, t);
        fmfma(x1);
        if constexpr (DIST) {
#pragma unroll
            for (int i = 0; i < 3; ++i) {
                float d2 = dsum[i];
                d2 += __shfl_xor(d2, 1, 64); d2 += __shfl_xor(d2, 2, 64); d2 += __shfl_xor(d2, 4, 64);
                if (quad == 0) mf_smem[FOLD_DIST_OFF + 24 * wave + (lane >> 3) + 8 * i] = sqrtf(d2);
            }
        }
        constexpr int CP = 68;
        float* const fc = mf_smem;
#pragma unroll
        for (int i = 0; i < 2; ++i)
#pragma unroll
            for (int j = 0; j < 4; ++j)
#pragma unroll
                for (int q = 0; q < 4; ++q) fc[(32 * wave + 16 * i + 4 * lk + q) * CP + 16 * j + li] = acc4[i][j][q];
        __syncthreads();
#pragma unroll
        for (int i = 0; i < WM; ++i)
#pragma unroll
            for (int j = 0; j < WN; ++j)
#pragma unroll
                for (int q = 0; q < 4; ++q) {
                    const int rho = wm0 + 16 * i + 4 * lk + q;
                    acc[i][j][q] = fc[(blk * (rho / kr) + rho % kr) * CP + wn0 + 16 * j + li];
                }
        __syncthreads();
      }
    };

    auto run_vfold6 = [&](const MainSeg& sg, const bool pf_next) __attribute__((always_inline)) {
      if constexpr (X6) {
        constexpr int ARC = 208;
        constexpr int A_PLX = ARC * P6, VO_OFF = 3 * A_PLX, W_OFF = VO_OFF + 8 * 32 * 4, BUFX = W_OFF + 128 * P * 4;
        static_assert(2 * BUFX <= CFG::LDS, "fold tile (X6)");
        static_assert(RP == 64, "fold loader (X6)");
        const int klen = sg.klen, nst = klen / BK;
        const __amdgpu_buffer_rsrc_t rsA = __builtin_amdgcn_make_buffer_rsrc(const_cast<float*>(sg.a), 0, 0xFFFFFFF0u, 0x00020000);
        const __amdgpu_buffer_rsrc_t rsK = __builtin_amdgcn_make_buffer_rsrc(const_cast<float*>(sg.b), 0, 0xFFFFFFF0u, 0x00020000);
        const __amdgpu_buffer_rsrc_t rsM = __builtin_amdgcn_make_buffer_rsrc(const_cast<float*>(sg.b2), 0, 0xFFFFFFF0u, 0x00020000);
        typedef unsigned int bu32x4 __attribute__((ext_vector_type(4)));
        unsigned voA[3], voB;
#pragma unroll
        for (int i = 0; i < 3; ++i) voA[i] = (unsigned)((giptr)sg.idx)[min(m0 + trow + 64 * i, M - 1)] * (unsigned)(sg.lda * 4) + 16u * quad;
        const int vo_t = (tid >> 5) & 7, vo_c = tid & 31;
        const unsigned voV = (unsigned)((giptr)sg.idx2)[min(m0 + 24 * vo_t, M - 1)] * (unsigned)(sg.lda * 4) + 4u * vo_c;
        voB = (unsigned)min(n0 + trow, N - 1) * (unsigned)(sg.ldb * 4) + 16u * quad;
        f32x4 va4[2][3], vb4[2][2];
        float vv[2];
        auto vissue = [&](auto set_c, int t) __attribute__((always_inline)) {
            constexpr int SS_ = decltype(set_c)::value;
            const int so = min(t, nst - 1) * (BK * 4);
#pragma unroll
            for (int i = 0; i < 3; ++i) va4[SS_][i] = __builtin_bit_cast(f32x4, (bu32x4)__builtin_amdgcn_raw_buffer_load_b128(rsA, voA[i], so, 0));
            vv[SS_] = __builtin_bit_cast(float, (unsigned)__builtin_amdgcn_raw_buffer_load_b32(rsA, voV, so, 0));
            vb4[SS_][0] = __builtin_bit_cast(f32x4, (bu32x4)__builtin_amdgcn_raw_buffer_load_b128(rsK, voB, so, 0));
            vb4[SS_][1] = __builtin_bit_cast(f32x4, (bu32x4)__builtin_amdgcn_raw_buffer_load_b128(rsM, voB, so, 0));
        };
        auto cut4_fold = [&](const float (&x)[4], unsigned (&w1)[2], unsigned (&w2)[2], unsigned (&w3)[2]) __attribute__((always_inline)) {
            unsigned p1[4], p2[4], p3[4];
#pragma unroll
            for (int j = 0; j < 4; ++j) x6_cut1(x[j], p1[j], p2[j], p3[j]);
#pragma unroll
            for (int h = 0; h < 2; ++h) {
                w1[h] = __builtin_amdgcn_perm(p1[2 * h + 1], p1[2 * h], 0x07060302u);
                w2[h] = __builtin_amdgcn_perm(p2[2 * h + 1], p2[2 * h], 0x07060302u);
                w3[h] = __builtin_amdgcn_perm(p3[2 * h + 1], p3[2 * h], 0x07060302u);
            }
        };
        auto vstash = [&](auto set_c, int buf, int part) __attribute__((always_inline)) {
            constexpr int SS_ = decltype(set_c)::value;
            unsigned char* const bb = lds6 + buf * BUFX;
#pragma unroll
            for (int i = 0; i < 3; ++i) {
                if ((i < 2) != (part == 0) || part == 2) continue;
                const f32x4 v = va4[SS_][i];
                const float x[4] = {v[0], v[1], v[2], v[3]};
                unsigned w1[2], w2[2], w3[2];
                cut4_fold(x, w1, w2, w3);
                unsigned char* d = bb + (trow + 64 * i) * P6 + 8 * quad;
                *(x6_u32x2*)(d) = x6_u32x2{w1[0], w1[1]}; *(x6_u32x2*)(d + A_PLX) = x6_u32x2{w2[0], w2[1]}; *(x6_u32x2*)(d + 2 * A_PLX) = x6_u32x2{w3[0], w3[1]};
            }
            if (part == 1) *(float*)(bb + VO_OFF + (vo_t * 32 + vo_c) * 4) = vv[SS_];
            if (part == 2) {
#pragma unroll
                for (int i = 0; i < 2; ++i) *(f32x4*)(bb + W_OFF + ((trow + 64 * i) * P + 4 * quad) * 4) = vb4[SS_][i];
            }
        };
        f32x4 acc4[2][4];
#pragma unroll
        for (int i = 0; i < 2; ++i)
#pragma unroll
            for (int j = 0; j < 4; ++j) acc4[i][j] = f32x4{0.f, 0.f, 0.f, 0.f};
        struct Raw { f32x4 wk[2], wm[2]; };
        const x6_bf16x8 z8 = {0, 0, 0, 0, 0, 0, 0, 0};
        x6_bf16x8 af[2][2][3];
        x6_bf16x8 bq[2][3];
        f32x4 vo[2];
#pragma unroll
        for (int p = 0; p < 3; ++p) { af[1][0][p] = z8; af[1][1][p] = z8; bq[1][p] = z8; }
        auto read_af = [&](int buf, x6_bf16x8 (&f)[2][3]) __attribute__((always_inline)) {
            const unsigned char* a = lds6 + buf * BUFX + (24 * wave + li) * P6 + 16 * lk;
#pragma unroll
            for (int i = 0; i < 2; ++i)
#pragma unroll
                for (int p = 0; p < 3; ++p) f[i][p] = *(const x6_bf16x8*)(a + i * 16 * P6 + p * A_PLX);
        };
        auto read_vo = [&](int buf) __attribute__((always_inline)) {
            const unsigned char* v = lds6 + buf * BUFX + VO_OFF + (wave * 32 + 8 * lk) * 4;
            vo[0] = *(const f32x4*)(v); vo[1] = *(const f32x4*)(v + 16);
        };
        auto read_w = [&](int buf, int j, Raw& r) __attribute__((always_inline)) {
            const unsigned char* b = lds6 + buf * BUFX + W_OFF + ((16 * j + li) * P + 8 * lk) * 4;
            r.wk[0] = *(const f32x4*)(b); r.wk[1] = *(const f32x4*)(b + 16);
            r.wm[0] = *(const f32x4*)(b + 64 * P * 4); r.wm[1] = *(const f32x4*)(b + 64 * P * 4 + 16);
        };
        auto build = [&](const Raw& r, x6_bf16x8 (&o)[3]) __attribute__((always_inline)) {
            unsigned w1[4], w2[4], w3[4];
#pragma unroll
            for (int h = 0; h < 2; ++h) {
                float x[4];
#pragma unroll
                for (int e = 0; e < 4; ++e) { const float v_ = vo[h][e], m_ = r.wm[h][e], k_ = r.wk[h][e]; x[e] = __builtin_fmaf(v_, m_, k_); }
                unsigned a1[2], a2[2], a3[2];
                cut4_fold(x, a1, a2, a3);
                w1[2 * h] = a1[0]; w1[2 * h + 1] = a1[1]; w2[2 * h] = a2[0]; w2[2 * h + 1] = a2[1]; w3[2 * h] = a3[0]; w3[2 * h + 1] = a3[1];
            }
            typedef unsigned int mu32x4 __attribute__((ext_vector_type(4)));
            o[0] = __builtin_bit_cast(x6_bf16x8, mu32x4{w1[0], w1[1], w1[2], w1[3]});
            o[1] = __builtin_bit_cast(x6_bf16x8, mu32x4{w2[0], w2[1], w2[2], w2[3]});
            o[2] = __builtin_bit_cast(x6_bf16x8, mu32x4{w3[0], w3[1], w3[2], w3[3]});
        };
        auto fmfma = [&](const x6_bf16x8 (&a)[2][3], const x6_bf16x8 (&b)[3], int j) __attribute__((always_inline)) {
#pragma unroll
            for (int q = 0; q < 6; ++q)
#pragma unroll
                for (int i = 0; i < 2; ++i) acc4[i][j] = __builtin_amdgcn_mfma_f32_16x16x32_bf16(a[i][X6_A[q]], b[X6_B[q]], acc4[i][j], 0, 0, 0);
        };
        auto pin6 = [&]() __attribute__((always_inline)) {
#pragma unroll
            for (int q = 0; q < 12; ++q) {
                __builtin_amdgcn_sched_group_barrier(0x008, 1, 0);
                __builtin_amdgcn_sched_group_barrier(0x100, 1, 0);
                __builtin_amdgcn_sched_group_barrier(0x002, 5, 0);
                __builtin_amdgcn_sched_group_barrier(0x200, 1, 0);
                __builtin_amdgcn_sched_group_barrier(0x020, 1, 0);
            }
            __builtin_amdgcn_sched_barrier(0);
        };
        typedef IntC<0> V0; typedef IntC<1> V1;
        vissue(V0{}, 0);
        vissue(V1{}, 1);
        vstash(V0{}, 0, 0); vstash(V0{}, 0, 1); vstash(V0{}, 0, 2);
        vissue(V0{}, 2);
        __syncthreads();
        auto vstep = [&](auto par_c, auto last_c, int t) __attribute__((always_inline)) {
            constexpr int PAR = decltype(par_c)::value;
            constexpr bool LAST = decltype(last_c)::value;
            typedef IntC<PAR ^ 1> SS;
            Raw r0, r1;
            read_vo(PAR);
            read_w(PAR, 0, r0);
            read_af(PAR, af[PAR]);
            read_w(PAR, 1, r1);
            fmfma(af[PAR ^ 1], bq[1], 3);
            build(r0, bq[0]);
            pin6();
            if (LAST && pf_next) {
                const MainSeg& nx = args.seg[1];
                setup(IntC<K1 < 0 ? 0 : K1>{}, nx);
                const int kn = nx.klen, nn = (kn + BK - 1) / BK;
                issue(S0{}, Ff{}, kn, nn, 0);
                issue(S1{}, Ff{}, kn, nn, 1);
            }
            read_w(PAR, 2, r0);
            if (!LAST) vstash(SS{}, PAR ^ 1, 0);
            fmfma(af[PAR], bq[0], 0);
            build(r1, bq[1]);
            pin6();
            read_w(PAR, 3, r1);
            if (!LAST) vstash(SS{}, PAR ^ 1, 1);
            fmfma(af[PAR], bq[1], 1);
            build(r0, bq[0]);
            pin6();
            if (!LAST) { vstash(SS{}, PAR ^ 1, 2); vissue(SS{}, t + 3); }
            fmfma(af[PAR], bq[0], 2);
            build(r1, bq[1]);
            pin6();
            __syncthreads();
        };
        int t = 0;
        for (; t + 2 < nst; t += 2) { vstep(V0{}, Ff{}, t); vstep(V1{}, Ff{}, t + 1); }
        if (t + 1 < nst) { vstep(V0{}, Ff{}, t); vstep(V1{}, Tt{}, t + 1); fmfma(af[1], bq[1], 3); }
        else { vstep(V0{}, Tt{}, t); fmfma(af[0], bq[1], 3); }
        constexpr int CP = 68;
        float* const fc = mf_smem;
#pragma unroll
        for (int i = 0; i < 2; ++i)
#pragma unroll
            for (int j = 0; j < 4; ++j)
#pragma unroll
                for (int q = 0; q < 4; ++q) fc[(32 * wave + 16 * i + 4 * lk + q) * CP + 16 * j + li] = acc4[i][j][q];
        __syncthreads();
#pragma unroll
        for (int i = 0; i < WM; ++i)
#pragma unroll
            for (int j = 0; j < WN; ++j)
#pragma unroll
                for (int q = 0; q < 4; ++q) {
                    const int rho = wm0 + 16 * i + 4 * lk + q;
                    acc[i][j][q] = fc[(32 * (rho / 24) + rho % 24) * CP + wn0 + 16 * j + li];
                }
        __syncthreads();
      }
    };

    bool started = false;
    int base = 0;
    auto seg_pass = [&](auto idx_c) __attribute__((always_inline)) {
        constexpr int I = decltype(idx_c)::value;
        const int nst = nsteps[I];
        const int lo = min(max(g0 - base, 0), nst), hi = min(max(g1 - base, 0), nst);
        base += nst;
        if (lo < hi) {
            if (!started) {
                const MainSeg& g = args.seg[I];
                setup(IntC<KS[I]>{}, g);
                typedef std::integral_constant<bool, KS[I] == MK_GATHER_MUL> MI;
                issue(S0{}, MI{}, g.klen, nst, lo);
                if (DEPTH == 2) issue(S1{}, MI{}, g.klen, nst, lo + 1);
                started = true;
            }
            run_seg(idx_c, lo, hi, g1 > base);
        }
        stamp(1 + I);
    };
    if constexpr (VFOLD) {
        if constexpr (X6) {
            run_vfold6(args.seg[0], NSEG > 1);
            const x6_bf16x8 z8 = {0, 0, 0, 0, 0, 0, 0, 0};
#pragma unroll
            for (int q = 0; q < 2; ++q)
#pragma unroll
                for (int p = 0; p < 3; ++p) {
                    xa[q][p] = z8;
#pragma unroll
                    for (int j = 0; j < WN; ++j) xb[q][j][p] = z8;
                }
        }
        else if constexpr (BM % 96 == 0) run_vfold4(args.seg[0], NSEG > 1);
        else run_vfold(args.seg[0], NSEG > 1);
        base = nsteps[0]; started = true;
        stamp(1);
    } else {
        seg_pass(IntC<0>{});
    }
    if constexpr (NSEG > 1) seg_pass(IntC<1>{});
    if constexpr (NSEG > 2) seg_pass(IntC<2>{});
    if constexpr (NSEG > 3) seg_pass(IntC<3>{});
    if constexpr (NSEG > 4) seg_pass(IntC<4>{});
    constexpr int NP = CFG::ADAM ? BM * (BN / 4) / MT : 1;
    static_assert(!CFG::ADAM || (BM * (BN / 4) % MT == 0 && NP == 4), "ADAM: four 16-byte pieces per thread (64 x 64 tiles, 256 threads)");
    int pf_row[NP];
    f32x4 pf_p[NP], pf_m[NP], pf_v[NP];
    if constexpr (CFG::ADAM) {
#pragma unroll
        for (int i = 0; i < NP; ++i) {
            const int rc = min(m0 + (tid + i * MT) / (BN / 4), M - 1);
            if constexpr (ROWMAP) pf_row[i] = ((giptr)args.seg[0].idx)[rc];
            else pf_row[i] = rc;
        }
    }
    if constexpr (!X6) mfma(afB, bfB);
    if constexpr (CFG::ADAM) {
        const AdamFuse& ad = args.adam;
#pragma unroll
        for (int i = 0; i < NP; ++i) {
            const int n = n0 + 4 * ((tid + i * MT) % (BN / 4));
            const long long off = (long long)pf_row[i] * args.ldo + (n + 3 < N ? n : N - 4);
            pf_p[i] = *(gf4ptr)(ad.p + off); pf_m[i] = *(gf4ptr)(ad.m + off); pf_v[i] = *(gf4ptr)(ad.v + off);
        }
        __builtin_amdgcn_sched_barrier(0);
    }

    constexpr int SP = BN + 4;
    float* const stage = mf_smem;
    static_assert(BM * SP * 4 <= CFG::LDS, "the staged tile lies inside the launch's LDS (MainCfg::LDS_STAGE)");
    constexpr int QR = BN / 4;
    const EpiArgs& e = args.epi;
    float* const dst = S > 1 ? args.slab + (long long)z * M * N : args.out;
    const long long ldd = S > 1 ? (long long)N : args.ldo;
    const bool plain = CFG::ADAM || S > 1 || !(e.rowadd || e.bias || e.relu || e.dropout || e.gate);
    auto item = [&](int f, int& r, int& n, int& nl) __attribute__((always_inline)) {
        const int rr = f / QR, cq = f - rr * QR;
        r = m0 + rr; n = n0 + 4 * cq;
        nl = min(n, N - 4 >= 0 ? N - 4 : 0);
        return rr * SP + 4 * cq;
    };
    auto win = [&](const float* p, int nl, int sh) __attribute__((always_inline)) {
        const f32x4 w = *(const f32x4u*)(p + nl);
        f32x4 o;
#pragma unroll
        for (int jj = 0; jj < 4; ++jj) { const int sj = jj + sh; o[jj] = sj == 0 ? w[0] : sj == 1 ? w[1] : sj == 2 ? w[2] : sj == 3 ? w[3] : 0.f; }
        return o;
    };
    const bool use_add = !plain && e.rowadd;
    const int rdiv = use_add ? e.rowdiv : 1;
    auto fetch_add = [&](int f) __attribute__((always_inline)) -> f32x4 {
        int r2, n2, nl2; item(f, r2, n2, nl2);
        const int n2c = min(n2, N - 1), nl2c = min(nl2, n2c);
        return win(e.rowadd + (long long)(min(r2, M - 1) / rdiv) * e.ld_rowadd, nl2c, n2c - nl2c);
    };
    constexpr int LAST_F = BM * QR - 1;
    f32x4 add0 = {0.f, 0.f, 0.f, 0.f}, add1 = add0, add2 = add0;
    if (use_add) { add0 = fetch_add(min(tid, LAST_F)); add1 = fetch_add(min(tid + MT, LAST_F)); add2 = fetch_add(min(tid + 2 * MT, LAST_F)); }
    int orow_v = 0;
    if constexpr (ROWMAP && !CFG::ADAM) orow_v = ((giptr)args.seg[0].idx)[min(m0 + min(tid, BM - 1), M - 1)];
#pragma unroll
    for (int i = 0; i < WM; ++i)
#pragma unroll
        for (int j = 0; j < WN; ++j)
#pragma unroll
            for (int q = 0; q < 4; ++q) stage[(wm0 + 16 * i + 4 * lk + q) * SP + wn0 + 16 * j + li] = acc[i][j][q];
    int* const orow = (int*)(stage + BM * SP);
    if constexpr (ROWMAP && !CFG::ADAM) {
        static_assert(!ROWMAP || (BM <= MT && (BM * SP + BM) * 4 <= CFG::LDS), "row map: one thread per tile row, table behind the staged tile");
        if (tid < BM) orow[tid] = orow_v;
    }
    __syncthreads();
    auto piece = [&](const int f, const int i) __attribute__((always_inline)) {
        int r, n, nl;
        const int so = item(f, r, n, nl);
        const f32x4 addv = add0;
        add0 = add1; add1 = add2;
        if (use_add) add2 = fetch_add(min(f + 3 * MT, LAST_F));
        if (r >= M || n >= N) return;
        f32x4 v = *(const f32x4*)(stage + so);
        const int sh = n - nl;
        if (!plain) {
            f32x4 add = addv, msk = {1.f, 1.f, 1.f, 1.f}, gte = {1.f, 1.f, 1.f, 1.f};
            if (e.bias) add += win(e.bias, nl, sh);
            if (e.dropout == 2) msk = win(e.keep_mask + (long long)r * e.ld_mask, nl, sh);
            if (e.gate) gte = win(e.gate + (long long)r * e.ld_gate, nl, sh);
#pragma unroll
            for (int jj = 0; jj < 4; ++jj) {
                float x = v[jj] + add[jj];
                if (e.relu == 1) x = x > 0.f ? x : 0.f;
                else if (e.relu == 2) x = tanhf(x);
                if (e.dropout == 1)
                    x = dropout_keep(e.seed_lo, e.seed_hi, e.layer, (unsigned long long)r * (unsigned)N + (unsigned)(n + jj), e.drop_p) ? x * e.drop_scale : 0.f;
                else if (e.dropout == 2)
                    x = msk[jj] != 0.f ? x * e.drop_scale : 0.f;
                if (e.gate) x = gte[jj] > 0.f ? x * e.gate_scale : 0.f;
                v[jj] = x;
            }
        }
        if constexpr (CFG::EPI == EPI_MLB) {
            const int g = e.rowsplit_g, b = r / g, jr = r - b * g;
            const f32x4 xq = win(e.fold_mul + (long long)b * e.ld_fold, nl, sh);
            v *= xq;
            const long long ro = jr == 0 ? (long long)b : (long long)b * (g - 1) + jr - 1;
            float* oz = (jr == 0 ? e.out0 + ro * e.ldo0 : args.out + ro * args.ldo) + n;
            if (n + 3 < N) *(f32x4u*)oz = v;
            else { oz[0] = v[0]; if (n + 1 < N) oz[1] = v[1]; if (n + 2 < N) oz[2] = v[2]; }
            if (args.t_out) {
                float* ot = (jr == 0 ? args.t_out0 : args.t_out) + ro * N + n;
                f32x4 t;
#pragma unroll
                for (int jj = 0; jj < 4; ++jj) t[jj] = tanhf(v[jj]);
                if (n + 3 < N) *(f32x4u*)ot = t;
                else { ot[0] = t[0]; if (n + 1 < N) ot[1] = t[1]; if (n + 2 < N) ot[2] = t[2]; }
            }
            return;
        }
        float* o = dst + (long long)r * ldd + n;
        if constexpr (CFG::ADAM) o = dst + (long long)pf_row[i] * ldd + n;
        else if constexpr (ROWMAP) o = dst + (long long)orow[f / QR] * ldd + n;
        if (n + 3 < N) *(f32x4u*)o = v;
        else { o[0] = v[0]; if (n + 1 < N) o[1] = v[1]; if (n + 2 < N) o[2] = v[2]; }
        if constexpr (CFG::ADAM) {
            const AdamFuse& ad = args.adam;
            const long long off = o - dst;
            float* const pp = ad.p + off; float* const pm = ad.m + off; float* const pv = ad.v + off;
            if (n + 3 < N) {
                f32x4 p4 = pf_p[i], m4 = pf_m[i], v4 = pf_v[i];
#pragma unroll
                for (int jj = 0; jj < 4; ++jj) {
                    float pj = p4[jj], mj = m4[jj], vj = v4[jj];
                    adam_update(pj, v[jj], mj, vj, ad.s.step_size, ad.s.b1, ad.s.b2, ad.s.eps, ad.s.inv_bc2_sqrt, ad.s.gscale);
                    p4[jj] = pj; m4[jj] = mj; v4[jj] = vj;
                }
                *(f32x4u*)pp = p4; *(f32x4u*)pm = m4; *(f32x4u*)pv = v4;
            } else {
#pragma unroll
                for (int jj = 0; jj < 3; ++jj) {
                    if (n + jj >= N) break;
                    float pj = pp[jj], mj = pm[jj], vj = pv[jj];
                    adam_update(pj, v[jj], mj, vj, ad.s.step_size, ad.s.b1, ad.s.b2, ad.s.eps, ad.s.inv_bc2_sqrt, ad.s.gscale);
                    pp[jj] = pj; pm[jj] = mj; pv[jj] = vj;
                }
            }
        }
    };
    if constexpr (CFG::ADAM) {
#pragma unroll
        for (int i = 0; i < NP; ++i) piece(tid + i * MT, i);
    } else {
#pragma unroll 1
        for (int f = tid; f < BM * QR; f += MT) piece(f, 0);
    }
    stamp(8);
    if (stamps && tid == 0) stamps[15] = __builtin_amdgcn_s_memrealtime();
}

__global__ __launch_bounds__(256) void k_main_fixup(const MainArgs a) {
    const int M = a.M, N = a.N, S = a.split;
    const int nq = (N + 3) / 4;
    const long long i = (long long)blockIdx.x * 256 + threadIdx.x;
    if (i >= (long long)M * nq) return;
    const int r = (int)(i / nq), n0 = (int)(i - (long long)r * nq) * 4;
    float v[4] = {0.f, 0.f, 0.f, 0.f};
    const long long mn = (long long)M * N, off = (long long)r * N + n0;
    for (int z = 0; z < S; ++z)
#pragma unroll
        for (int j = 0; j < 4; ++j) if (n0 + j < N) v[j] += a.slab[z * mn + off + j];
    const EpiArgs& e = a.epi;
#pragma unroll
    for (int j = 0; j < 4; ++j) {
        const int n = n0 + j;
        if (n >= N) break;
        a.out[(long long)r * a.ldo + n] = apply_epilogue(e, v[j], r, n, N);
    }
}

static inline bool main_fwd_operand_ok(int klen) { return klen >= 4 && klen % 4 == 0; }

template <int K0, int... REST> struct FirstKind { static constexpr int value = K0; };

template <class CFG, bool DIST, int... KINDS>
static inline int launch_main_fwd_seq(MainArgs& a, hipStream_t s) {
    static_assert(!CFG::ADAM, "launch_main_fwd_adam sizes the grid of the forms with passengers");
    constexpr int lds = FirstKind<KINDS...>::value == MK_VFOLD ? (CFG::LDS_FOLD > CFG::LDS ? CFG::LDS_FOLD : CFG::LDS) : CFG::LDS;
    static DevMask attr{0};
    NCX_HIP_TRY(set_max_lds_once(attr, (const void*)k_main_fwd<CFG, DIST, KINDS...>, lds));
    const int tiles_m = (a.M + CFG::BM - 1) / CFG::BM, tiles_n = (a.N + CFG::BN - 1) / CFG::BN;
    const int S = a.split > 1 ? a.split : 1;
    const int grid = ((tiles_m * S + 7) / 8) * 8 * tiles_n;
    hipLaunchKernelGGL((k_main_fwd<CFG, DIST, KINDS...>), dim3(grid), dim3(CFG::T), lds, s, a);
    NCX_HIP_TRY(hipGetLastError());
    if (S > 1) {
        const long long nthreads = (long long)a.M * ((a.N + 3) / 4);
        hipLaunchKernelGGL(k_main_fixup, dim3((unsigned)((nthreads + 255) / 256)), dim3(256), 0, s, a);
        NCX_HIP_TRY(hipGetLastError());
    }
    return NCX_OK;
}

template <class CFG>
static inline int launch_main_fwd(MainArgs& a, hipStream_t s) {
    if (a.nseg < 1 || a.nseg > MAIN_MAX_SEG || a.M < 1 || a.N < 1) return NCX_E_DIMS;
    for (int i = 0; i < a.nseg; ++i) if (!main_fwd_operand_ok(a.seg[i].klen)) return NCX_E_DIMS;
    if (a.epi.rowadd && a.epi.rowdiv < 3) return NCX_E_DIMS;
    if (a.split > 1 && !a.slab) return NCX_E_WORKSPACE;
    auto is = [&](std::initializer_list<int> ks) { if ((int)ks.size() != a.nseg) return false; int i = 0; for (int k : ks) if (a.seg[i++].kind != k) return false; return true; };
    constexpr int G = MK_GATHER, X = MK_GATHER_MUL, P = MK_PLAIN, S = MK_SOFTMAX;
    constexpr int V = MK_VFOLD;
    if constexpr (CFG::EPI == EPI_ROWMAP) {
        const EpiArgs& e = a.epi;
        if (!is({G, G}) || a.split > 1 || a.dist_out || !a.out || !a.seg[0].idx || a.seg[0].idx != a.seg[1].idx ||
            e.rowadd || e.bias || e.relu || e.dropout || e.gate)
            return NCX_E_FLAGS;
        return launch_main_fwd_seq<CFG, false, G, G>(a, s);
    } else
    if constexpr (CFG::EPI == EPI_MLB) {
        if (!is({G}) || a.split > 1 || a.dist_out || a.N < 4 || !a.epi.bias || !a.epi.fold_mul || a.epi.rowsplit_g < 2 || !a.epi.out0 ||
            !a.out || (a.t_out && !a.t_out0))
            return NCX_E_FLAGS;
        return launch_main_fwd_seq<CFG, false, G>(a, s);
    } else {
    if (a.seg[0].kind == V) {
        if constexpr (CFG::BM == 48 && CFG::BN == 64 && CFG::WGM == 1 && CFG::DEPTH == 2) {
            if (a.split > 1 || a.seg[0].klen % MF_BK || a.seg[0].klen < 2 * MF_BK || !a.epi.rowadd || a.epi.rowdiv != 24) return NCX_E_FLAGS;
            if (a.dist_out) {
                if (is({V, P, P, S})) return launch_main_fwd_seq<CFG, true, V, P, P, S>(a, s);
                if (is({V, P, P, P})) return launch_main_fwd_seq<CFG, true, V, P, P, P>(a, s);
            } else {
                if (is({V, P, P, S})) return launch_main_fwd_seq<CFG, false, V, P, P, S>(a, s);
                if (is({V, P, P, P})) return launch_main_fwd_seq<CFG, false, V, P, P, P>(a, s);
            }
        }
        if constexpr (CFG::BM % 96 == 0 && CFG::BN == 64 && CFG::WGM * CFG::WGN == CFG::T / 64 && CFG::DEPTH == 2) {
            if (a.split > 1 || a.seg[0].klen % MF_BK || a.seg[0].klen < 2 * MF_BK || !a.epi.rowadd || (a.epi.rowdiv != 24 && a.epi.rowdiv != 48))
                return NCX_E_FLAGS;
            if (a.dist_out) {
                if constexpr (CFG::X6) return NCX_E_FLAGS;
                else {
                    if (a.epi.rowdiv != 24) return NCX_E_FLAGS;
                    if (is({V, P, P, S})) return launch_main_fwd_seq<CFG, true, V, P, P, S>(a, s);
                    if (is({V, P, P, P})) return launch_main_fwd_seq<CFG, true, V, P, P, P>(a, s);
                    return NCX_E_FLAGS;
                }
            }
            if (is({V, P, P, S})) return launch_main_fwd_seq<CFG, false, V, P, P, S>(a, s);
            if (is({V, P, P, P})) return launch_main_fwd_seq<CFG, false, V, P, P, P>(a, s);
        }
        return NCX_E_FLAGS;
    }
    if constexpr (CFG::X6) return NCX_E_FLAGS;
    else {
    if (a.dist_out) {
        if (a.split > 1 || a.nseg < 3 || a.seg[1].klen % MF_BK) return NCX_E_FLAGS;
        if (is({G, X, P, P, S})) return launch_main_fwd_seq<CFG, true, G, X, P, P, S>(a, s);
        if (is({G, X, P, P, P})) return launch_main_fwd_seq<CFG, true, G, X, P, P, P>(a, s);
        return NCX_E_FLAGS;
    }
    if (is({G, X, P, P, S})) return launch_main_fwd_seq<CFG, false, G, X, P, P, S>(a, s);
    if (is({P}))             return launch_main_fwd_seq<CFG, false, P>(a, s);
    if (is({G}))             return launch_main_fwd_seq<CFG, false, G>(a, s);
    if (is({G, P, P, S}))    return launch_main_fwd_seq<CFG, false, G, P, P, S>(a, s);
    if (is({G, X, P, P, P})) return launch_main_fwd_seq<CFG, false, G, X, P, P, P>(a, s);
    if (is({G, P, P, P}))    return launch_main_fwd_seq<CFG, false, G, P, P, P>(a, s);
    if (is({P, P}))          return launch_main_fwd_seq<CFG, false, P, P>(a, s);
    return NCX_E_FLAGS;
    }
    }
}


template <class CFG>
static inline int launch_main_fwd_adam(MainArgs& a, int n_pass, int pass_at_hint, hipStream_t s) {
    static_assert(CFG::ADAM && CFG::EPI != EPI_MLB && !CFG::X6, "the answer-embedding gradient's forms");
    if (a.nseg != 2 || a.M < 1 || a.N < 1 || a.split > 1 || a.dist_out || !a.out) return NCX_E_FLAGS;
    if (a.N < 4) return NCX_E_DIMS;
    for (int i = 0; i < 2; ++i) if (!main_fwd_operand_ok(a.seg[i].klen)) return NCX_E_DIMS;
    const EpiArgs& e = a.epi;
    if (e.rowadd || e.bias || e.relu || e.dropout || e.gate) return NCX_E_FLAGS;
    AdamFuse& ad = a.adam;
    if (!ad.p || !ad.m || !ad.v || (ad.tn && (!ad.tp || !ad.tg || !ad.tm || !ad.tv))) return NCX_E_NULL;
    constexpr bool RM = CFG::EPI == EPI_ROWMAP;
    constexpr int KIND = RM ? MK_GATHER : MK_PLAIN;
    if (a.seg[0].kind != KIND || a.seg[1].kind != KIND) return NCX_E_FLAGS;
    if (RM && (!a.seg[0].idx || a.seg[0].idx != a.seg[1].idx)) return NCX_E_FLAGS;
    constexpr int lds = CFG::LDS;
    static DevMask attr{0};
    NCX_HIP_TRY(set_max_lds_once(attr, (const void*)k_main_fwd<CFG, false, KIND, KIND>, lds));
    const int tiles_m = (a.M + CFG::BM - 1) / CFG::BM, tiles_n = (a.N + CFG::BN - 1) / CFG::BN;
    const int grid = ((tiles_m + 7) / 8) * 8 * tiles_n;
    ad.n_pass = ad.tn ? (n_pass > 0 ? n_pass : 1) : 0;
    ad.pass_at = pass_at_hint >= 0 && pass_at_hint < grid ? pass_at_hint : grid;
    hipLaunchKernelGGL((k_main_fwd<CFG, false, KIND, KIND>), dim3(grid + ad.n_pass), dim3(CFG::T), lds, s, a);
    NCX_HIP_TRY(hipGetLastError());
    return NCX_OK;
}

}
```

vqa-counterexamples_amd/csrc/ncx_main.hip:

```cpp
#include "ncx_main.h"

namespace ncx {

typedef MainCfg<48, 128, 1, 4, 2, 2> MainCfg0;
typedef MainCfg<96, 64, 2, 2, 1, 2> MainCfg1;
typedef MainCfg<96, 128, 2, 2, 2, 1> MainCfg2;
typedef MainCfg<160, 128, 2, 2, 2, 1> MainCfgW;
typedef MainCfg<64, 64, 2, 2, 2, 3> MainCfg3;
typedef MainCfg<48, 64, 1, 4, 2, 2> MainCfgFold;
typedef MainCfg<96, 64, 2, 2, 2, 2> MainCfgFold4;
typedef MainCfg<192, 64, 4, 2, 2, 2, 512, true> MainCfgFold8X6;
typedef MainCfg<192, 64, 4, 2, 2, 2, 512> MainCfgFold8;

bool main_short_form(long long M, long long N, long long T, int split) {
    return split <= 1 && T <= 32 && ((M + 63) / 64) * ((N + 63) / 64) >= 2 * num_cus() && !hook_env("NCX_MAIN_CFG");
}

int main_chain_form(long long M, long long N, long long T, int split, bool single_gather, bool wide_ok) {
    if (main_short_form(M, N, T, split)) return 4;
    const long long tiles96 = (long long)((M + 95) / 96) * ((N + 127) / 128);
    if (wide_ok && split <= 1 && single_gather && !hook_env("NCX_MAIN_CFG")) {
        const long long cus = num_cus(), tiles160 = (long long)((M + 159) / 160) * ((N + 127) / 128);
        const double e96 = (double)tiles96 / (double)(((tiles96 + cus - 1) / cus) * cus), e160 = (double)tiles160 / (double)(((tiles160 + cus - 1) / cus) * cus);
        if (tiles160 * 10 >= cus * 7 && e160 > e96 + 0.1) return 3;
    }
    int cfg = (split <= 1 && tiles96 * 10 >= (long long)num_cus() * 9) ? 2 : 0;
    if (const char* e = hook_env("NCX_MAIN_CFG")) cfg = atoi(e);
    return cfg >= 1 && cfg <= 3 ? cfg : 0;
}

template <class C> using AsIs = C;
template <template <class> class W>
static int main_forward_chain(MainArgs& a, hipStream_t s) {
    long long T = 0;
    for (int i = 0; i < a.nseg; ++i) T += (a.seg[i].klen + MF_BK - 1) / MF_BK;
    constexpr bool wide_ok = W<MainCfgW>::EPI != EPI_ROWMAP;
    switch (main_chain_form(a.M, a.N, T, a.split, a.nseg == 1 && a.seg[0].kind == MK_GATHER, wide_ok)) {
    case 4: return launch_main_fwd<W<MainCfg3>>(a, s);
    case 3:
        if constexpr (wide_ok) return launch_main_fwd<W<MainCfgW>>(a, s);
        else return NCX_E_FLAGS;
    case 1: return launch_main_fwd<W<MainCfg1>>(a, s);
    case 2: return launch_main_fwd<W<MainCfg2>>(a, s);
    default: return launch_main_fwd<W<MainCfg0>>(a, s);
    }
}

int main_forward(MainArgs& a, hipStream_t s) {
    if (a.nseg > 0 && a.seg[0].kind == MK_VFOLD) {
        const int rows = main_fold_rows_eff(a.M, a.N, a.epi.rowdiv);
        if (rows == 192 && a.x6 && a.epi.rowdiv == 24) return launch_main_fwd<MainCfgFold8X6>(a, s);
        return rows == 192 ? launch_main_fwd<MainCfgFold8>(a, s) : rows == 96 ? launch_main_fwd<MainCfgFold4>(a, s) : launch_main_fwd<MainCfgFold>(a, s);
    }
    return main_forward_chain<AsIs>(a, s);
}

int main_forward_rowmap(MainArgs& a, hipStream_t s) {
    if (a.nseg != 2 || a.seg[0].kind != MK_GATHER) return NCX_E_FLAGS;
    return main_forward_chain<WithRowMap>(a, s);
}

int main_adam_passengers() {
    if (const char* e = hook_env("NCX_ADAM_PASS")) { const int n = atoi(e); if (n > 0) return n; }
    return num_cus();
}

int main_forward_adam(MainArgs& a, bool rowmap, hipStream_t s) {
    long long T = 0;
    for (int i = 0; i < a.nseg; ++i) T += (a.seg[i].klen + MF_BK - 1) / MF_BK;
    if (!main_short_form(a.M, a.N, T, a.split)) return NCX_E_FLAGS;
    int at = 0;
    if (const char* e = hook_env("NCX_ADAM_PASS_AT")) at = atoi(e);
    const int np = main_adam_passengers();
    return rowmap ? launch_main_fwd_adam<WithAdam<WithRowMap<MainCfg3>>>(a, np, at, s) : launch_main_fwd_adam<WithAdam<MainCfg3>>(a, np, at, s);
}

int main_forward_mlb(MainArgs& a, hipStream_t s) {
    const long long tiles96 = (long long)((a.M + 95) / 96) * ((a.N + 127) / 128);
    if (tiles96 * 10 >= (long long)num_cus() * 9) return launch_main_fwd<WithMlbEpi<MainCfg2>>(a, s);
    return launch_main_fwd<WithMlbEpi<MainCfg0>>(a, s);
}

int main_fold_rows_eff(long long M, long long N, int rowdiv) {
    int rows = main_fold_rows(M, N);
    if (rowdiv == 48 && rows == 48) rows = 96;
    if (const char* f4 = hook_env("NCX_FOLD4")) rows = atoi(f4) != 0 ? 96 : (rowdiv == 48 ? 96 : 48);
    if (const char* f8 = hook_env("NCX_FOLD8")) rows = atoi(f8) != 0 ? 192 : (rows == 192 ? 96 : rows);
    return rows;
}

int main_fold_rows(long long M, long long N) {
    const long long cus = num_cus();
    const long long wg96 = ((M + 95) / 96) * ((N + 63) / 64), wg192 = ((M + 191) / 192) * ((N + 63) / 64);
    if (wg96 * 4 < cus * 2 * 3) return 48;
    const double e8 = (double)wg192 / (double)(((wg192 + cus - 1) / cus) * cus), e4 = (double)wg96 / (double)(((wg96 + 2 * cus - 1) / (2 * cus)) * 2 * cus);
    return e8 + 0.03 >= e4 ? 192 : 96;
}

int main_split(long long M, long long N, long long T) {
    const long long tiles = ((M + 47) / 48) * ((N + 127) / 128), cus = num_cus();
    if (tiles >= cus) return 1;
    long long S = 2 * cus / tiles;
    if (S > T / 8) S = T / 8;
    if (const char* e = hook_env("NCX_MAIN_SPLIT")) S = atoll(e);
    return (int)(S < 1 ? 1 : S);
}

}
```

vqa-counterexamples_amd/csrc/ncx_plan.h:

```cpp
#pragma once
#include "ncx_internal.h"

#pragma GCC visibility push(hidden)
namespace ncx {
constexpr int NCX_SCATTER_MAX_B = 32768;
constexpr int NCX_PERM_MAX_A = 32768;
int check_dims(const ncx_dims* d);

struct StepRoutes {
    bool km;
    int km_form;
    bool tn8;
    bool tn8_shared;
    bool tn8_x6;
    bool emb_nt;
    bool de_skip;
    long long cand_ksteps;
    bool dw1ak_on_tn8(bool side) const { return tn8 && emb_nt && !side; }
};
StepRoutes routes(const ncx_dims& d);
struct FwdRoute { bool vfold, dist_in_fold, dist_in_main; };
FwdRoute forward_route(const ncx_dims& d, const StepRoutes& r);

struct GemmUse { int form; long long M, N, ksteps; bool allow96; GemmPlan plan; long long slab_elems; long long tiles; long long wgs; };
enum { U_GT = 0, U_SH, U_MAIN, U_FWD_L, U_DW1C, U_DW1S, U_DE, U_DW1AK, U_DAGT, U_DWL, U_DXL, U_COUNT };
void list_uses(const ncx_dims& d, const StepRoutes& r, GemmUse* u);
int dw1c_seg_split(long long cols, int S, long long ksteps);
WsLayout ws_layout(const ncx_dims& d, const StepRoutes& r);

constexpr int WPAD_N = 7;
int wpad_cols(const ncx_dims& d, int i);
int wpad_width(const ncx_dims& d, int i);
}
#pragma GCC visibility pop
```

vqa-counterexamples_amd/csrc/ncx_plan.hip:

```cpp
#include "ncx_plan.h"
#include "ncx_bf16.h"
#include <stdio.h>

namespace ncx {
int check_dims(const ncx_dims* d) {
    if (!d) return NCX_E_NULL;
    if (d->B < 1 || d->K < 1 || d->K > 64 || d->dv < 1 || d->dq < 1 || d->dz < 1 || d->da < 1 || d->A < 1 ||
        d->H < 1 || d->L < 1 || d->L > 3 || d->n_img < 1)
        return NCX_E_DIMS;
    if ((long long)d->B * d->K > (1ll << 30) / 4 || d->B > NCX_SCATTER_MAX_B) return NCX_E_DIMS;
    if (d->dv < 4 || d->dq < 4 || d->dz < 4 || d->da < 4 || d->A < 4 || d->H < 4 || d->K < 3) return NCX_E_DIMS;
    if (d->drop_p < 0.f || d->drop_p >= 1.f) return NCX_E_DIMS;
    if (d->flags & ~(NCX_F_ALL | NCX_F_BF16 | NCX_F_REUSE_GT | NCX_F_FUSED_TAIL | NCX_F_X6)) return NCX_E_FLAGS;
    if ((d->flags & NCX_F_BF16) && (d->flags & NCX_F_ALL) != NCX_F_ALL) return NCX_E_FLAGS;
    return NCX_OK;
}

int wpad_cols(const ncx_dims& d, int i) {
    const int c[WPAD_N] = {d.dv, (d.flags & NCX_F_V_MULT) ? d.dv : 0, d.K + 1, d.dz, (d.flags & NCX_F_A_EMB) ? 0 : d.da, d.L >= 2 ? d.H : 0, d.L >= 3 ? d.H : 0};
    return c[i];
}
int wpad_width(const ncx_dims& d, int i) {
    const int c = wpad_cols(d, i);
    if (d.flags & NCX_F_BF16) return 0;
    return (c == 0 || c % 32 == 0) ? 0 : pad_to(c, 32);
}

int num_cus() {
    static int n = 0;
    if (!n) {
        int dev = 0, v = 0;
        if (hipGetDevice(&dev) == hipSuccess && hipDeviceGetAttribute(&v, hipDeviceAttributeMultiprocessorCount, dev) == hipSuccess && v > 0) n = v;
        else { (void)hipGetLastError(); n = 256; }
    }
    return n;
}

static int choose_split(long long tiles, long long ksteps, long long slots) {
    if (tiles >= slots) return 1;
    long long sp = cdiv(6 * slots, tiles);
    const long long smax = ksteps / 24 > 1 ? ksteps / 24 : 1;
    if (sp > smax) sp = smax;
    if (tiles * sp < slots) {
        const long long smax2 = ksteps / 8 > 1 ? ksteps / 8 : 1;
        sp = cdiv(slots, tiles);
        if (sp > smax2) sp = smax2;
    }
    return (int)(sp < 1 ? 1 : sp);
}

static GemmPlan plan_from_tiles(int form, long long tiles_big, long long tiles_small, long long ksteps, bool big_ok) {
    GemmPlan p; p.split = 1;
    const long long cus = num_cus();
    const double eff_big = (double)tiles_big / (double)(cdiv(tiles_big, cus) * cus);
    if (big_ok && tiles_big >= 192 && ksteps >= 64 && eff_big >= 0.75) { p.cfg = CFG_128x128; return p; }
    p.cfg = CFG_64x64;
    const int occ = form == FORM_NT ? occupancy_nt(p.cfg) : form == FORM_TN ? occupancy_tn(p.cfg) : occupancy_nn(p.cfg);
    p.split = choose_split(tiles_small, ksteps, (long long)occ * num_cus());
    return p;
}

GemmPlan plan_gemm(int form, long long M, long long N, long long ksteps, bool allow_96) {
    if (form == FORM_NT && allow_96 && ksteps <= 32 && M * N >= 64 * 64 * 512) {
        GemmPlan p; p.cfg = CFG_64x64; p.split = 1; return p;
    }
    if (form == FORM_NT && allow_96 && M >= 96 && N >= 128) {
        const double cus = (double)num_cus();
        const double t128 = (double)(cdiv(M, 128) * cdiv(N, 128)), t96 = (double)(cdiv(M, 96) * cdiv(N, 128));
        const double waste128 = (double)(cdiv(M, 128) * 128 * cdiv(N, 128) * 128) / (double)(M * N);
        const double waste96 = (double)(cdiv(M, 96) * 96 * cdiv(N, 128) * 128) / (double)(M * N);
        const double e128 = (t128 / cus) / (double)cdiv((long long)t128, (long long)cus) / waste128;
        const double e96 = (t96 / cus) / (double)cdiv((long long)t96, (long long)cus) / waste96;
        if (t96 >= 0.75 * cus || t128 >= 0.75 * cus) {
            GemmPlan p; p.split = 1; p.cfg = e96 > e128 * 1.02 ? CFG_96x128 : CFG_128x128; return p;
        }
    }
    const bool big_ok = M >= 96 && N >= 96;
    return plan_from_tiles(form, cdiv(M, 128) * cdiv(N, 128), cdiv(M, 64) * cdiv(N, 64), ksteps, big_ok);
}

StepRoutes routes(const ncx_dims& d) {
    StepRoutes r{};
    const bool bf16 = d.flags & NCX_F_BF16, aemb = d.flags & NCX_F_A_EMB, km_ok = dw_km_supported(d);
    r.km = km_ok && !bf16;
    r.km_form = bf16 ? KM_FORM_NONE : km_ok ? dw_km_form(d) : KM_FORM_GROUPED;
    r.tn8 = dw_tn8_supported(d);
    r.tn8_shared = dw_tn8_shared_ok(d);
    r.tn8_x6 = dw_tn8_x6(d);
    r.emb_nt = aemb && !bf16 && !hook_env("NCX_NO_EMB_NT");
    r.de_skip = r.emb_nt && d.A <= NCX_PERM_MAX_A && !hook_env("NCX_NO_DE_SKIP");
    r.cand_ksteps = ksteps(d.dv) * ((d.flags & NCX_F_V_MULT) ? 2 : 1) + ksteps(d.K + 1) + ksteps(d.dz) + ksteps(aemb ? d.A : d.da);
    return r;
}

int dw1c_seg_split(long long cols, int S, long long ksteps) {
    long long narrow = 512;
    if (const char* e = hook_env("NCX_SMALL_COLS")) narrow = atoll(e);
    if (S <= 1 || cols > narrow) return S;
    int mult = 2;
    if (const char* e = hook_env("NCX_SMALL_MULT")) mult = atoi(e) > 0 ? atoi(e) : 1;
    long long sp = (long long)S * mult;
    const long long smax = ksteps / 8 > 1 ? ksteps / 8 : 1;
    if (sp > smax) sp = smax;
    return (int)(sp < S ? S : sp);
}

void list_uses(const ncx_dims& d, const StepRoutes& r, GemmUse* u) {
    const long long M = (long long)d.B * d.K, H = d.H;
    const bool aemb = d.flags & NCX_F_A_EMB;
    const long long cand_cols = (long long)d.dv * ((d.flags & NCX_F_V_MULT) ? 2 : 1) + d.K + 1 + d.dz + (aemb ? d.A : d.da);
    const long long sh_k = ksteps(d.dv) + ksteps(d.dq) + ksteps(d.dz) + ksteps(d.da);
    const long long sh_cols = (long long)d.dv + d.dq + d.dz + d.da;
    u[U_GT]    = {FORM_NT, H, d.A, ksteps(d.da), false};
    u[U_SH]    = {FORM_NT, d.B, H, sh_k, false};
    u[U_MAIN]  = {FORM_NT, M, H, r.cand_ksteps, true};
    u[U_FWD_L] = {FORM_NT, M, H, ksteps(H), true};
    u[U_DW1C]  = {FORM_TN, H, cand_cols, ksteps(M), false};
    u[U_DW1S]  = {FORM_TN, H, sh_cols, ksteps(d.B), false};
    u[U_DE]    = {FORM_TN, d.A, d.da, 2 * ksteps(H), false};
    u[U_DW1AK] = {FORM_NN, H, d.da, ksteps(d.A), false};
    u[U_DAGT]  = {FORM_NN, 1, 1, 1, false};
    u[U_DWL]   = {FORM_TN, H, H, ksteps(M), false};
    u[U_DXL]   = {FORM_NN, M, H, ksteps(H), false};
    const bool hooks = experiment_hooks_on();
    const bool km = r.km, tn8 = r.tn8, tn8s = r.tn8_shared;
    const long long segs_c[5] = {km ? 0 : d.dv, (!km && (d.flags & NCX_F_V_MULT)) ? d.dv : 0, tn8 ? 0 : d.K + 1, tn8 ? 0 : d.dz, tn8 ? 0 : (aemb ? d.A : d.da)};
    const long long segs_s[5] = {tn8s ? 0 : d.dv, tn8s ? 0 : d.dq, tn8s ? 0 : d.dz, tn8s ? 0 : d.da, 0};
    for (int i = 0; i < U_COUNT; ++i) {
        const bool grouped = i == U_DW1C || i == U_DW1S;
        auto grouped_tiles = [&](int bm, int bn) {
            const long long* sg = i == U_DW1C ? segs_c : segs_s;
            long long t = 0;
            for (int q = 0; q < 5; ++q) t += cdiv(H, bm) * cdiv(sg[q], bn);
            return t;
        };
        if (grouped && grouped_tiles(64, 64) == 0) {
            u[i].plan.cfg = CFG_128x64; u[i].plan.split = 1;
        } else if (grouped) {
            u[i].plan = plan_from_tiles(FORM_TN, grouped_tiles(128, 128), grouped_tiles(64, 64), u[i].ksteps, false);
            if (i == U_DW1C && H >= 128 && u[i].plan.split > 1) {
                u[i].plan.cfg = CFG_128x64;
                const long long slots = (long long)occupancy_tn(CFG_128x64) * num_cus();
                long long sp = cdiv(3 * slots, grouped_tiles(128, 64));
                const long long smax = u[i].ksteps / 24 > 1 ? u[i].ksteps / 24 : 1;
                if (sp > 8) sp = 8;
                u[i].plan.split = (int)(sp > smax ? smax : sp < 1 ? 1 : sp);
            }
        } else {
            u[i].plan = plan_gemm(u[i].form, u[i].M, u[i].N, u[i].ksteps, u[i].allow96);
        }
        if (i == U_MAIN || i == U_FWD_L || i == U_DXL) u[i].plan.split = 1;
        if (hooks) {
            char name[32];
            snprintf(name, sizeof name, "NCX_CFG_%d", i);
            const char* c = getenv(name);
            if (c) u[i].plan.cfg = atoi(c);
            snprintf(name, sizeof name, "NCX_SPLIT_%d", i);
            const char* e = getenv(name);
            if (e && i != U_MAIN && i != U_FWD_L && i != U_DXL) u[i].plan.split = atoi(e) > 1 ? atoi(e) : 1;
        }
        int bm, bn; cfg_tile(u[i].plan.cfg, bm, bn);
        long long tiles = cdiv(u[i].M, bm) * cdiv(u[i].N, bn);
        if (grouped) tiles = grouped_tiles(bm, bn);
        u[i].tiles = tiles;
        const int S = u[i].plan.split > 1 ? u[i].plan.split : 1;
        long long wgs = 0;
        if (grouped) {
            const long long* sg = i == U_DW1C ? segs_c : segs_s;
            for (int q = 0; q < 5; ++q)
                if (sg[q] > 0) wgs += WgMap{(int)cdiv(H, bm), (int)cdiv(sg[q], bn), i == U_DW1C ? dw1c_seg_split(sg[q], S, u[i].ksteps) : S}.count();
        } else {
            wgs = WgMap{(int)cdiv(u[i].M, bm), (int)cdiv(u[i].N, bn), S}.count();
        }
        u[i].wgs = wgs;
        u[i].slab_elems = S > 1 ? wgs * bm * bn : 0;
    }
    u[U_DW1S].plan.cfg = u[U_DW1C].plan.cfg;
    {
        int bm, bn; cfg_tile(u[U_DW1C].plan.cfg, bm, bn);
        const int S = u[U_DW1S].plan.split > 1 ? u[U_DW1S].plan.split : 1;
        u[U_DW1S].tiles = 0; u[U_DW1S].wgs = 0;
        for (int q = 0; q < 4; ++q) {
            if (segs_s[q] == 0) continue;
            u[U_DW1S].tiles += cdiv(H, bm) * cdiv(segs_s[q], bn);
            u[U_DW1S].wgs += WgMap{(int)cdiv(H, bm), (int)cdiv(segs_s[q], bn), S}.count();
        }
        u[U_DW1C].slab_elems = (u[U_DW1C].wgs + u[U_DW1S].wgs) * bm * bn;
        u[U_DW1S].slab_elems = 0;
    }
}

WsLayout ws_layout(const ncx_dims& d) { return ws_layout(d, routes(d)); }
WsLayout ws_layout(const ncx_dims& d, const StepRoutes& r) {
    WsLayout w{};
    const size_t M = (size_t)d.B * d.K, H = d.H;
    size_t off = 0;
    auto take = [&](size_t bytes) { size_t o = off; off = align_up(off + bytes, 256); return o; };
    w.idx_k = take(M * 4); w.idx_o = take(M * 4); w.idx_ob = take((size_t)d.B * 4);
    w.mx = take(M * 4); w.inv = take(M * 4);
    w.ldm = pad_to(d.K + 1, 4);
    w.ldgt = (d.flags & NCX_F_BF16) ? d.A : pad_to(d.A, 32);
    w.misc = take(M * w.ldm * 4);
    w.gt = take(H * w.ldgt * 4);
    w.sh = take((size_t)d.B * H * 4);
    for (int l = 0; l < 3; ++l) w.h[l] = l < d.L ? take(M * H * 4) : 0;
    w.dpre[0] = take(M * H * 4);
    w.dpre[1] = d.L >= 2 ? take(M * H * 4) : 0;
    w.dsh = take((size_t)d.B * H * 4);
    w.dgt = take(2 * H * d.A * 4);
    w.dagt = w.dgt + H * d.A * 4;
    w.dgtT = take((size_t)2 * d.A * pad_to(d.H, 4) * 4);
    w.w1aT = take((size_t)2 * d.da * pad_to(d.H, 32) * 4);
    w.dgtT2 = take(r.tn8 ? (size_t)pad_to(d.A, 32) * pad_to(d.H, 4) * 4 : 0);
    w.de_perm = take(r.emb_nt ? ((size_t)d.A + 1) * 4 : 0);
    w.partial = take((size_t)NCX_PRELUDE_WAVES * H * 4 * 2 + (size_t)NCX_PRELUDE_WAVES * 4 + 256);
    GemmUse u[U_COUNT];
    list_uses(d, r, u);
    long long slab = 0;
    for (int i = 0; i < U_COUNT; ++i) slab = u[i].slab_elems > slab ? u[i].slab_elems : slab;
    w.slab_bytes = (size_t)slab * 4;
    if (dw_tn8_slab_bytes(d) > w.slab_bytes) w.slab_bytes = dw_tn8_slab_bytes(d);
    w.slab = take(w.slab_bytes);
    {
        long long s2 = u[U_GT].slab_elems;
        if (u[U_SH].slab_elems > s2) s2 = u[U_SH].slab_elems;
        if (u[U_DW1AK].slab_elems > s2) s2 = u[U_DW1AK].slab_elems;
        if (u[U_DE].slab_elems > s2) s2 = u[U_DE].slab_elems;
        w.slab2_bytes = (size_t)s2 * 4;
        w.slab2 = take(w.slab2_bytes);
    }
    w.km_slab = take(dw_km_slab_bytes(d));
    {
        auto need = [&](long long m, long long n, long long t) { const int sp = main_split(m, n, t); return sp > 1 ? (size_t)sp * m * n * 4 : (size_t)0; };
        size_t b = need((long long)M, (long long)H, r.cand_ksteps);
        if (d.L >= 2) b = b > need((long long)M, (long long)H, ksteps(H)) ? b : need((long long)M, (long long)H, ksteps(H));
        w.mslab_bytes = b;
        w.mslab = take(b);
    }
    {
        size_t e = 0;
        for (int i = 0; i < WPAD_N; ++i) e += (size_t)H * wpad_width(d, i);
        w.wpad = take(e * 4);
    }
    if (d.flags & NCX_F_BF16) {
        w.xc = take(bf16_xc_bytes(d)); w.wc = take(bf16_wc_bytes(d));
        w.dpre_bf = take(bf16_dpre_bytes(d)); w.bf_slab = take(bf16_slab_bytes(d));
        w.bf_emb = take(bf16_emb_bytes(d));
    }
    w.total = off;
    return w;
}
}
```

vqa-counterexamples_amd/neuralcx/_lib.py:

```python
import ctypes as C
import os

_HERE = os.path.dirname(os.path.abspath(__file__))
LIB_PATH = os.environ.get("NCX_LIB") or os.path.join(os.path.dirname(_HERE), "lib", "libneuralcx_hip.so")

NCX_F_V_MULT, NCX_F_V_DIST, NCX_F_V_RANK, NCX_F_A_EMB = 1, 2, 4, 8
NCX_F_ALL = 15
NCX_F_REUSE_GT = 32
NCX_F_FUSED_TAIL = 64
NCX_F_X6 = 128
NCX_F_BF16 = 16

EXPORTS = ("ncx_input_size", "ncx_workspace_bytes", "ncx_forward", "ncx_forward_phase", "ncx_loss_rank", "ncx_backward", "ncx_backward_phase",
           "ncx_adam_step", "ncx_backward_adam", "ncx_version", "ncx_profile_begin", "ncx_profile_end", "ncx_plan_query",
           "ncx_vqa_workspace_bytes", "ncx_vqa_forward", "ncx_mlb_workspace_bytes", "ncx_mlb_forward", "ncx_mlb_att_workspace_bytes", "ncx_mlb_att_forward", "ncx_mlb_att_forward_flags", "ncx_mlb_att_logits_form", "ncx_knn_workspace_bytes", "ncx_knn_status_offset", "ncx_knn", "ncx_cosine_gram_workspace_bytes", "ncx_cosine_gram", "ncx_semantic_scores",
           "ncx_similarity_scores",
           "ncx_gru_packed_bytes", "ncx_gru_pack", "ncx_gru_workspace_bytes", "ncx_gru_encode", "ncx_gru_encode_flags", "ncx_gru_step_form",
           "ncx_gru_train_workspace_bytes", "ncx_gru_packed_t_bytes", "ncx_gru_pack_t", "ncx_gru_train_forward", "ncx_gru_train_forward_flags", "ncx_gru_train_backward",
           "ncx_gru_train_backward_flags", "ncx_gru_bwd_form",
           "ncx_lstm2_packed_bytes", "ncx_lstm2_pack", "ncx_lstm2_workspace_bytes", "ncx_lstm2_encode", "ncx_lstm2_encode_flags", "ncx_lstm2_step_form",
           "ncx_lstm2_train_workspace_bytes", "ncx_lstm2_packed_t_bytes", "ncx_lstm2_pack_t", "ncx_lstm2_train_forward", "ncx_lstm2_train_forward_flags", "ncx_lstm2_train_backward",
           "ncx_ws_region", "ncx_wgmap_check", "ncx_bf16_layout",
           "ncx_comm_unique_id", "ncx_comm_create", "ncx_comm_destroy", "ncx_allreduce", "ncx_train_tail", "ncx_profile_stamps",
           "ncx_pairlin_workspace_bytes", "ncx_pairlin_forward", "ncx_pairlin_backward",
# ... 86 lines not shown


_PL_NAMES = ("answer_embedding", "w", "b", "w_out", "b_out")


class NcxPairlinParams(C.Structure):
    _fields_ = [(n, C.c_void_p) for n in _PL_NAMES]


class NcxPairlinGrads(C.Structure):
    _fields_ = [(n, C.c_void_p) for n in _PL_NAMES]


class NcxError(RuntimeError):
    pass


_ERR = {-1: "NCX_E_NULL (required pointer is NULL)", -2: "NCX_E_DIMS (dimension out of range)",
        -3: "NCX_E_WORKSPACE (workspace too small or misaligned)", -4: "NCX_E_FLAGS (inconsistent lesion inputs)",
        -5: "NCX_E_UNSUPPORTED (RCCL could not be loaded)", -6: "NCX_E_COMM (RCCL reported an error)"}

_lib = None


def lib():
    global _lib
    if _lib is not None:
        return _lib
    if not os.path.exists(LIB_PATH):
        raise NcxError("HIP library not built: %s is missing. Run `python -c 'import __graft_entry__ as g; "
                       "g.build()'` or `make -C vqa-counterexamples_amd`." % LIB_PATH)
    import torch
    L = C.CDLL(LIB_PATH)
    L.ncx_version.restype = C.c_char_p
    L.ncx_input_size.restype = C.c_int64
    L.ncx_input_size.argtypes = [C.POINTER(NcxDims)]
    L.ncx_workspace_bytes.restype = C.c_size_t
    L.ncx_workspace_bytes.argtypes = [C.POINTER(NcxDims)]
    L.ncx_forward.restype = C.c_int
    L.ncx_forward.argtypes = [C.POINTER(NcxDims), C.POINTER(NcxInputs), C.POINTER(NcxParams), C.c_void_p,
                              C.c_size_t, C.c_void_p, C.c_void_p]
    L.ncx_forward_phase.restype = C.c_int
    L.ncx_forward_phase.argtypes = [C.POINTER(NcxDims), C.POINTER(NcxInputs), C.POINTER(NcxParams), C.c_void_p,
                                    C.c_size_t, C.c_void_p, C.c_int32, C.c_void_p]
    L.ncx_loss_rank.restype = C.c_int
    L.ncx_loss_rank.argtypes = [C.c_void_p, C.c_void_p, C.c_int32, C.c_int32, C.c_float, C.c_void_p,
                                C.c_void_p, C.c_void_p, C.c_void_p, C.c_void_p, C.c_void_p]
    L.ncx_backward.restype = C.c_int
    L.ncx_backward.argtypes = [C.POINTER(NcxDims), C.POINTER(NcxInputs), C.POINTER(NcxParams), C.c_void_p,
                               C.c_size_t, C.c_void_p, C.POINTER(NcxGrads), C.c_void_p]
    L.ncx_backward_phase.restype = C.c_int
    L.ncx_backward_phase.argtypes = [C.POINTER(NcxDims), C.POINTER(NcxInputs), C.POINTER(NcxParams), C.c_void_p,
                                     C.c_size_t, C.c_void_p, C.POINTER(NcxGrads), C.c_int32, C.c_void_p]
    L.ncx_adam_step.restype = C.c_int
    L.ncx_adam_step.argtypes = [C.c_void_p, C.c_void_p, C.c_void_p, C.c_void_p, C.c_size_t, C.c_float,
                                C.c_float, C.c_float, C.c_float, C.c_int32, C.c_float, C.c_void_p]
    L.ncx_backward_adam.restype = C.c_int
    L.ncx_backward_adam.argtypes = [C.POINTER(NcxDims), C.POINTER(NcxInputs), C.POINTER(NcxParams), C.c_void_p,
                                    C.c_size_t, C.c_void_p, C.POINTER(NcxGrads), C.POINTER(NcxAdamState), C.c_void_p]
    L.ncx_vqa_workspace_bytes.restype = C.c_size_t
    L.ncx_vqa_workspace_bytes.argtypes = [C.POINTER(NcxDims), C.POINTER(NcxMutanParams)]
    L.ncx_vqa_forward.restype = C.c_int
    L.ncx_vqa_forward.argtypes = [C.POINTER(NcxDims), C.c_void_p, C.c_void_p, C.c_void_p, C.POINTER(NcxMutanParams), C.c_void_p,
                                  C.c_size_t, C.c_void_p, C.c_void_p, C.c_void_p, C.c_void_p, C.c_void_p]
    L.ncx_mlb_workspace_bytes.restype = C.c_size_t
    L.ncx_mlb_workspace_bytes.argtypes = [C.POINTER(NcxDims), C.POINTER(NcxMlbParams)]
    L.ncx_mlb_forward.restype = C.c_int
    L.ncx_mlb_forward.argtypes = [C.POINTER(NcxDims), C.c_void_p, C.c_void_p, C.c_void_p, C.POINTER(NcxMlbParams), C.c_void_p,
                                  C.c_size_t, C.c_void_p, C.c_void_p, C.c_void_p, C.c_void_p, C.c_void_p]
    L.ncx_mlb_att_workspace_bytes.restype = C.c_size_t
    L.ncx_mlb_att_workspace_bytes.argtypes = [C.POINTER(NcxMlbAttDims), C.POINTER(NcxMlbAttParams)]
    L.ncx_mlb_att_forward.restype = C.c_int
    L.ncx_mlb_att_forward.argtypes = [C.POINTER(NcxMlbAttDims), C.c_void_p, C.c_void_p, C.c_void_p, C.POINTER(NcxMlbAttParams), C.c_void_p,
                                      C.c_size_t, C.c_void_p, C.c_void_p, C.c_void_p]
    L.ncx_mlb_att_forward_flags.restype = C.c_int
    L.ncx_mlb_att_forward_flags.argtypes = [C.POINTER(NcxMlbAttDims), C.c_void_p, C.c_void_p, C.c_void_p, C.POINTER(NcxMlbAttParams), C.c_uint32,
                                            C.c_void_p, C.c_size_t, C.c_void_p, C.c_void_p, C.c_void_p]
    L.ncx_mlb_att_logits_form.restype = C.c_int
    L.ncx_mlb_att_logits_form.argtypes = [C.POINTER(NcxMlbAttDims), C.c_uint32]
    L.ncx_knn_workspace_bytes.restype = C.c_size_t
    L.ncx_knn_workspace_bytes.argtypes = [C.c_int32, C.c_int32]
    L.ncx_knn_status_offset.restype = C.c_size_t
    L.ncx_knn_status_offset.argtypes = [C.c_int32]
    L.ncx_knn.restype = C.c_int
    L.ncx_knn.argtypes = [C.c_void_p, C.c_int32, C.c_void_p, C.c_int32, C.c_int32, C.c_int32, C.c_int32, C.c_void_p,
                          C.c_size_t, C.c_void_p, C.c_void_p, C.c_void_p]
    L.ncx_cosine_gram_workspace_bytes.restype = C.c_size_t
    L.ncx_cosine_gram_workspace_bytes.argtypes = [C.c_int32, C.c_int32]
    L.ncx_cosine_gram.restype = C.c_int
    L.ncx_cosine_gram.argtypes = [C.c_void_p, C.c_int32, C.c_int32, C.c_void_p, C.c_size_t, C.c_void_p, C.c_void_p]
    L.ncx_semantic_scores.restype = C.c_int
    L.ncx_semantic_scores.argtypes = [C.c_void_p, C.c_void_p, C.c_int32, C.c_int32, C.c_int32, C.c_void_p, C.c_float,
                                      C.c_void_p, C.c_void_p, C.c_void_p, C.c_void_p]
    L.ncx_similarity_scores.restype = C.c_int
    L.ncx_similarity_scores.argtypes = [C.c_void_p, C.c_void_p, C.c_int32, C.c_int32, C.c_void_p, C.c_void_p, C.c_int32, C.c_void_p,
                                        C.c_void_p, C.c_int32, C.c_int32, C.c_int32, C.c_void_p, C.c_void_p, C.c_void_p, C.c_void_p]
    L.ncx_gru_packed_bytes.restype = C.c_size_t
    L.ncx_gru_packed_bytes.argtypes = [C.c_int32, C.c_int32]
    L.ncx_gru_pack.restype = C.c_int
    L.ncx_gru_pack.argtypes = [C.c_void_p, C.c_void_p, C.c_void_p, C.c_void_p, C.c_int32, C.c_int32, C.c_void_p, C.c_void_p]
    L.ncx_gru_workspace_bytes.restype = C.c_size_t
    L.ncx_gru_workspace_bytes.argtypes = [C.c_int32, C.c_int32, C.c_int32, C.c_int32]
    L.ncx_gru_encode.restype = C.c_int
    L.ncx_gru_encode.argtypes = [C.c_void_p, C.c_int32, C.c_int32, C.c_void_p, C.c_int32, C.c_int32, C.c_int32, C.c_void_p, C.c_void_p,
                                 C.c_size_t, C.c_void_p, C.c_void_p, C.c_void_p]
    L.ncx_gru_encode_flags.restype = C.c_int
    L.ncx_gru_encode_flags.argtypes = L.ncx_gru_encode.argtypes[:8] + [C.c_uint32] + L.ncx_gru_encode.argtypes[8:]
    L.ncx_gru_step_form.restype = C.c_int
    L.ncx_gru_step_form.argtypes = [C.c_int32, C.c_int32, C.c_int32, C.c_int32, C.c_uint32]
    L.ncx_gru_train_workspace_bytes.restype = C.c_size_t
    L.ncx_gru_train_workspace_bytes.argtypes = [C.c_int32, C.c_int32, C.c_int32, C.c_int32]
    L.ncx_gru_packed_t_bytes.restype = C.c_size_t
    L.ncx_gru_packed_t_bytes.argtypes = [C.c_int32, C.c_int32]
    L.ncx_gru_pack_t.restype = C.c_int
    L.ncx_gru_pack_t.argtypes = [C.c_void_p, C.c_void_p, C.c_int32, C.c_int32, C.c_void_p, C.c_void_p]
    L.ncx_gru_train_forward.restype = C.c_int
    L.ncx_gru_train_forward.argtypes = L.ncx_gru_encode.argtypes
    L.ncx_gru_train_forward_flags.restype = C.c_int
    L.ncx_gru_train_forward_flags.argtypes = L.ncx_gru_encode_flags.argtypes
    L.ncx_gru_train_backward.restype = C.c_int
    L.ncx_gru_train_backward.argtypes = [C.c_void_p, C.c_int32, C.c_int32, C.c_void_p, C.c_int32, C.c_int32, C.c_int32, C.c_void_p, C.c_void_p,
                                         C.c_size_t] + [C.c_void_p] * 7
    L.ncx_gru_train_backward_flags.restype = C.c_int
    L.ncx_gru_train_backward_flags.argtypes = L.ncx_gru_train_backward.argtypes[:8] + [C.c_uint32] + L.ncx_gru_train_backward.argtypes[8:]
    L.ncx_gru_bwd_form.restype = C.c_int
    L.ncx_gru_bwd_form.argtypes = L.ncx_gru_step_form.argtypes
    L.ncx_lstm2_packed_bytes.restype = C.c_size_t
    L.ncx_lstm2_packed_bytes.argtypes = [C.c_int32, C.c_int32]
    L.ncx_lstm2_pack.restype = C.c_int
    L.ncx_lstm2_pack.argtypes = [C.c_void_p] * 8 + [C.c_int32, C.c_int32, C.c_void_p, C.c_void_p]
    L.ncx_lstm2_workspace_bytes.restype = C.c_size_t
    L.ncx_lstm2_workspace_bytes.argtypes = [C.c_int32, C.c_int32, C.c_int32, C.c_int32]
    L.ncx_lstm2_encode.restype = C.c_int
    L.ncx_lstm2_encode.argtypes = L.ncx_gru_encode.argtypes
    L.ncx_lstm2_encode_flags.restype = C.c_int
    L.ncx_lstm2_encode_flags.argtypes = L.ncx_gru_encode_flags.argtypes
    L.ncx_lstm2_step_form.restype = C.c_int
    L.ncx_lstm2_step_form.argtypes = [C.c_int32, C.c_int32, C.c_int32, C.c_int32, C.c_uint32]
    L.ncx_lstm2_train_workspace_bytes.restype = C.c_size_t
    L.ncx_lstm2_train_workspace_bytes.argtypes = [C.c_int32, C.c_int32, C.c_int32, C.c_int32]
    L.ncx_lstm2_packed_t_bytes.restype = C.c_size_t
    L.ncx_lstm2_packed_t_bytes.argtypes = [C.c_int32, C.c_int32]
    L.ncx_lstm2_pack_t.restype = C.c_int
    L.ncx_lstm2_pack_t.argtypes = [C.c_void_p] * 4 + [C.c_int32, C.c_int32, C.c_void_p, C.c_void_p]
    L.ncx_lstm2_train_forward.restype = C.c_int
    L.ncx_lstm2_train_forward.argtypes = L.ncx_gru_encode.argtypes
    L.ncx_lstm2_train_forward_flags.restype = C.c_int
    L.ncx_lstm2_train_forward_flags.argtypes = L.ncx_gru_encode_flags.argtypes
    L.ncx_lstm2_train_backward.restype = C.c_int
    L.ncx_lstm2_train_backward.argtypes = [C.c_void_p, C.c_int32, C.c_int32, C.c_void_p, C.c_int32, C.c_int32, C.c_int32, C.c_void_p, C.c_void_p,
                                           C.c_size_t] + [C.c_void_p] * 11
    L.ncx_ws_region.restype = C.c_int
    L.ncx_ws_region.argtypes = [C.POINTER(NcxDims), C.c_int32, C.POINTER(C.c_size_t), C.POINTER(C.c_size_t)]
    L.ncx_profile_begin.restype = C.c_int
    L.ncx_profile_begin.argtypes = [C.c_uint32, C.c_int32]
    L.ncx_profile_end.restype = C.c_int
    L.ncx_profile_end.argtypes = [C.POINTER(C.c_float), C.POINTER(C.c_int32), C.c_int32]
    L.ncx_profile_stamps.restype = C.c_int
    L.ncx_profile_stamps.argtypes = [C.c_void_p, C.c_int64]
    L.ncx_train_tail.restype = C.c_int
    L.ncx_train_tail.argtypes = [C.POINTER(NcxDims), C.POINTER(NcxParams), C.c_void_p, C.c_size_t] + [C.c_void_p] * 7 + [C.POINTER(NcxGrads), C.c_void_p]
    L.ncx_comm_unique_id.restype = C.c_int; L.ncx_comm_unique_id.argtypes = [C.c_void_p]
    L.ncx_comm_create.restype = C.c_int; L.ncx_comm_create.argtypes = [C.c_void_p, C.c_int32, C.c_int32, C.POINTER(C.c_void_p)]
    L.ncx_comm_destroy.restype = C.c_int; L.ncx_comm_destroy.argtypes = [C.c_void_p]
    L.ncx_allreduce.restype = C.c_int; L.ncx_allreduce.argtypes = [C.c_void_p, C.c_void_p, C.c_size_t, C.c_void_p]
    L.ncx_bf16_layout.restype = C.c_int
    L.ncx_bf16_layout.argtypes = [C.POINTER(NcxDims), C.POINTER(C.c_int32)]
    L.ncx_plan_query.restype = C.c_int
    L.ncx_plan_query.argtypes = [C.POINTER(NcxDims), C.c_int32, C.POINTER(C.c_int32)]
    P_SD = C.POINTER(NcxScorerDims)
    L.ncx_pairlin_workspace_bytes.restype = C.c_size_t
    L.ncx_pairlin_workspace_bytes.argtypes = [P_SD]
    L.ncx_pairlin_forward.restype = C.c_int
    L.ncx_pairlin_forward.argtypes = [P_SD, C.POINTER(NcxInputs), C.POINTER(NcxPairlinParams), C.c_void_p, C.c_size_t,
                                      C.c_void_p, C.c_void_p, C.c_void_p]
    L.ncx_pairlin_backward.restype = C.c_int
    L.ncx_pairlin_backward.argtypes = [P_SD, C.POINTER(NcxInputs), C.POINTER(NcxPairlinParams), C.c_void_p, C.c_size_t,
                                       C.c_void_p, C.POINTER(NcxPairlinGrads), C.c_void_p]
    L.ncx_linctx_workspace_bytes.restype = C.c_size_t
    L.ncx_linctx_workspace_bytes.argtypes = [P_SD]
    L.ncx_linctx_forward.restype = C.c_int
    L.ncx_linctx_forward.argtypes = [P_SD, C.c_void_p, C.c_void_p, C.c_void_p, C.c_void_p, C.c_size_t, C.c_void_p, C.c_void_p]
    L.ncx_linctx_backward.restype = C.c_int
    L.ncx_linctx_backward.argtypes = [P_SD, C.c_void_p, C.c_void_p, C.c_void_p, C.c_size_t, C.c_void_p, C.c_void_p, C.c_void_p]
    P_CD = C.POINTER(NcxContrastiveDims)
    L.ncx_contrastive_workspace_bytes.restype = C.c_size_t
    L.ncx_contrastive_workspace_bytes.argtypes = [P_CD]
    L.ncx_contrastive_forward.restype = C.c_int
    L.ncx_contrastive_forward.argtypes = [P_CD, C.POINTER(NcxInputs), C.c_void_p, C.c_void_p, C.c_void_p, C.c_size_t, C.c_void_p,
                                          C.c_void_p, C.c_void_p]
    L.ncx_contrastive_distances.restype = C.c_int
    L.ncx_contrastive_distances.argtypes = [P_CD, C.c_void_p, C.c_void_p, C.c_size_t, C.c_void_p, C.c_void_p]
    L.ncx_contrastive_loss.restype = C.c_int
    L.ncx_contrastive_loss.argtypes = [P_CD, C.c_void_p, C.c_size_t, C.c_float, C.c_float, C.c_void_p, C.c_void_p, C.c_void_p]
    L.ncx_contrastive_backward.restype = C.c_int
    L.ncx_contrastive_backward.argtypes = [P_CD, C.POINTER(NcxInputs), C.c_void_p, C.c_size_t, C.c_void_p, C.c_void_p, C.c_void_p,
                                           C.c_void_p]
    P_VT, P_MP = C.POINTER(NcxVqaTrainDims), C.POINTER(NcxMutanParams)
    L.ncx_vqa_train_workspace_bytes.restype = C.c_size_t
    L.ncx_vqa_train_workspace_bytes.argtypes = [P_VT, P_MP]
    L.ncx_vqa_train_forward.restype = C.c_int
    L.ncx_vqa_train_forward.argtypes = [P_VT, C.c_void_p, C.c_void_p, C.c_void_p, P_MP, C.c_void_p, C.c_void_p, C.c_size_t, C.c_void_p,
                                        C.c_void_p, C.c_void_p]
    L.ncx_ce_loss.restype = C.c_int
    L.ncx_ce_loss.argtypes = [C.c_void_p, C.c_void_p, C.c_int32, C.c_int32, C.c_float] + [C.c_void_p] * 7
    L.ncx_vqa_train_backward.restype = C.c_int
    L.ncx_vqa_train_backward.argtypes = [P_VT, P_MP, C.c_void_p, C.c_void_p, C.c_size_t, C.c_void_p, C.POINTER(NcxMutanGrads), C.c_void_p,
                                         C.c_void_p]
    L.ncx_vqa_train_ws_region.restype = C.c_int
    L.ncx_vqa_train_ws_region.argtypes = [P_VT, P_MP, C.c_int32, C.POINTER(C.c_size_t), C.POINTER(C.c_size_t)]
    P_LP = C.POINTER(NcxMlbParams)
    L.ncx_mlb_train_workspace_bytes.restype = C.c_size_t
    L.ncx_mlb_train_workspace_bytes.argtypes = [P_VT, P_LP]
    L.ncx_mlb_train_forward.restype = C.c_int
    L.ncx_mlb_train_forward.argtypes = [P_VT, C.c_void_p, C.c_void_p, C.c_void_p, P_LP, C.c_void_p, C.c_void_p, C.c_size_t, C.c_void_p,
                                        C.c_void_p, C.c_void_p]
    L.ncx_mlb_train_backward.restype = C.c_int
    L.ncx_mlb_train_backward.argtypes = [P_VT, P_LP, C.c_void_p, C.c_void_p, C.c_size_t, C.c_void_p, C.POINTER(NcxMlbGrads), C.c_void_p,
                                         C.c_void_p]
    L.ncx_mlb_train_ws_region.restype = C.c_int
    L.ncx_mlb_train_ws_region.argtypes = [P_VT, P_LP, C.c_int32, C.POINTER(C.c_size_t), C.POINTER(C.c_size_t)]
    P_AD, P_AT, P_AP = C.POINTER(NcxMlbAttDims), C.POINTER(NcxMlbAttTrain), C.POINTER(NcxMlbAttParams)
    L.ncx_mlb_att_train_workspace_bytes.restype = C.c_size_t
    L.ncx_mlb_att_train_workspace_bytes.argtypes = [P_AD, P_AT, P_AP]
    L.ncx_mlb_att_train_forward.restype = C.c_int
    L.ncx_mlb_att_train_forward.argtypes = [P_AD, P_AT, C.c_void_p, C.c_void_p, C.c_void_p, P_AP, C.c_void_p, C.c_void_p, C.c_size_t,
                                            C.c_void_p, C.c_void_p, C.c_void_p]
    L.ncx_mlb_att_train_forward_flags.restype = C.c_int
    L.ncx_mlb_att_train_forward_flags.argtypes = [P_AD, P_AT, C.c_void_p, C.c_void_p, C.c_void_p, P_AP, C.c_void_p, C.c_uint32, C.c_void_p,
                                                  C.c_size_t, C.c_void_p, C.c_void_p, C.c_void_p]
    L.ncx_mlb_att_train_backward.restype = C.c_int
    L.ncx_mlb_att_train_backward.argtypes = [P_AD, P_AT, C.c_void_p, C.c_void_p, C.c_void_p, P_AP, C.c_void_p, C.c_void_p, C.c_size_t,
                                             C.c_void_p, C.c_void_p, C.POINTER(NcxMlbAttGrads), C.c_void_p, C.c_void_p]
    L.ncx_mlb_att_train_backward_flags.restype = C.c_int
    L.ncx_mlb_att_train_backward_flags.argtypes = [P_AD, P_AT, C.c_void_p, C.c_void_p, C.c_void_p, P_AP, C.c_void_p, C.c_uint32, C.c_void_p,
                                                   C.c_size_t, C.c_void_p, C.c_void_p, C.POINTER(NcxMlbAttGrads), C.c_void_p, C.c_void_p]
    L.ncx_mlb_att_dwv_form.restype = C.c_int
    L.ncx_mlb_att_dwv_form.argtypes = [P_AD, C.c_uint32]
    L.ncx_mlb_att_train_ws_region.restype = C.c_int
    L.ncx_mlb_att_train_ws_region.argtypes = [P_AD, P_AT, P_AP, C.c_int32, C.POINTER(C.c_size_t), C.POINTER(C.c_size_t)]
    _lib = L
    return L


def check(rc, what):
    if rc == 0:
        return
    if rc < 0:
        raise NcxError("%s failed: %s" % (what, _ERR.get(rc, rc)))
    raise NcxError("%s failed: hipError_t %d" % (what, rc))


def version():
    return lib().ncx_version().decode()


GEMM_IDS = dict(GT=0, SH=1, MAIN=2, FWD_L=3, DW1C=4, DW1S=5, DE=6, DW1AK=7, DAGT=8, DWL=9, DXL=10)


def profile_begin(names, max_launches=4096):
    mask = 0
    for n in names:
        mask |= 1 << GEMM_IDS[n]
    check(lib().ncx_profile_begin(mask, max_launches), "ncx_profile_begin")


def profile_end(cap=4096):
    ms = (C.c_float * cap)()
    ids = (C.c_int32 * cap)()
    n = lib().ncx_profile_end(ms, ids, cap)
    if n < 0:
        check(n, "ncx_profile_end")
    inv = {v: k for k, v in GEMM_IDS.items()}
    out = {}
    for i in range(n):
        out.setdefault(inv[ids[i]], []).append(float(ms[i]))
    return out


def profile_stamps(buf=None):
    if buf is None:
        check(lib().ncx_profile_stamps(None, 0), "ncx_profile_stamps")
    else:
        check(lib().ncx_profile_stamps(C.c_void_p(buf.data_ptr()), buf.numel()), "ncx_profile_stamps")


NCX_QUERY_DW1_ROUTE = 32
DW1_FOLD_FORMS = ("none", "k_dw_km8", "k_dw_km_x6", "k_dw_km", "grouped")
DW1_TN_FORMS = ("grouped", "k_dw_tn8", "k_dw_tn8_x6")


NCX_QUERY_FUSED_ADAM = 33


NCX_QUERY_FWD_ROUTE = 34
FWD_ENGINES = ("generic", "chain", "fold", "bf16")
FWD_CHAIN_FORMS = ("48x128", "96x64", "96x128", "160x128", "64x64")


NCX_QUERY_BF16_ROUTE = 35
BF16_NT_FORMS = {0: "128x128", 1: "64x128", 2: "128x64", 3: "64x64", 8: "nt8"}


def bf16_layout(d):
    out = (C.c_int32 * 10)()
    check(lib().ncx_bf16_layout(C.byref(d), out), "ncx_bf16_layout")
    return dict(zip(("c_vk", "c_vm", "c_misc", "c_z", "c_p", "raw", "kc", "Hp", "dap", "Ap"), (int(v) for v in out)))


def plan_query(d, name):
    out = (C.c_int32 * 6)()
    if name == "BF16_ROUTE":
        check(lib().ncx_plan_query(C.byref(d), NCX_QUERY_BF16_ROUTE, out), "ncx_plan_query")
        if out[0] < 0:
            return None
        return dict(nt=out[0], nt_name=BF16_NT_FORMS[out[0]], tn8=bool(out[1]), S=out[2], chunk=out[3], nz=out[4],
                    vec_dpre=bool(out[5] & 1), vec_e=bool(out[5] & 2), vec_w1a=bool(out[5] & 4), vec_dg=bool(out[5] & 8))
    if name == "FWD_ROUTE":
        check(lib().ncx_plan_query(C.byref(d), NCX_QUERY_FWD_ROUTE, out), "ncx_plan_query")
        return dict(engine=out[0], engine_name=FWD_ENGINES[out[0]], tile=out[1],
                    tile_name=FWD_CHAIN_FORMS[out[1]] if out[0] == 1 else ("%dx64" % out[1] if out[0] == 2 else None),
                    split=out[2], dist_in_main=bool(out[3]), hidden_engine=out[4], hidden_split=out[5])
    if name == "FUSED_ADAM":
        check(lib().ncx_plan_query(C.byref(d), NCX_QUERY_FUSED_ADAM, out), "ncx_plan_query")
        return dict(fused=bool(out[0]), passengers=out[1])
    if name == "DW1_ROUTE":
        check(lib().ncx_plan_query(C.byref(d), NCX_QUERY_DW1_ROUTE, out), "ncx_plan_query")
        return dict(fold=DW1_FOLD_FORMS[out[0]], tn=DW1_TN_FORMS[out[1]], tn_pieces=out[2], tn_grid=out[3],
                    a_other_on_tn=bool(out[4]), tn_max_pieces=out[5])
    check(lib().ncx_plan_query(C.byref(d), GEMM_IDS[name], out), "ncx_plan_query")
    return dict(form=("NT", "TN", "NN")[out[0]], M=out[1], N=out[2], ksteps=out[3],
                tile=("64x64", "128x128", "96x128", "96x64", "128x64", "48x128", "48x64 (per-triplet fold of the two v segments)",
                      "96x64 (per-triplet fold of the two v segments, four triplets per workgroup)",
                      "192x64 (per-triplet fold of the two v segments, eight triplets per 8-wave workgroup, one workgroup per CU)")[out[4]], ksplit=out[5])


def comm_unique_id() -> bytes:
    buf = C.create_string_buffer(128)
    check(lib().ncx_comm_unique_id(buf), "ncx_comm_unique_id")
    return buf.raw


def comm_create(unique_id: bytes, nranks: int, rank: int) -> C.c_void_p:
    if len(unique_id) != 128:
        raise ValueError("unique id must be the 128 bytes ncx_comm_unique_id produced on rank 0")
    comm = C.c_void_p()
    check(lib().ncx_comm_create(C.create_string_buffer(unique_id, 128), int(nranks), int(rank), C.byref(comm)), "ncx_comm_create")
    return comm


def allreduce(comm: C.c_void_p, t, stream_ptr=None) -> None:
    import torch
    if t.dtype != torch.float32 or not t.is_contiguous() or not t.is_cuda:
        raise TypeError("ncx_allreduce takes a contiguous fp32 device tensor")
    sp = torch.cuda.current_stream(t.device).cuda_stream if stream_ptr is None else stream_ptr
    check(lib().ncx_allreduce(comm, C.c_void_p(t.data_ptr()), t.numel(), C.c_void_p(sp)), "ncx_allreduce")


def comm_destroy(comm: C.c_void_p) -> None:
    check(lib().ncx_comm_destroy(comm), "ncx_comm_destroy")
```

Before: 666,800 triplets/s.

## Fuse GT and shared-row forward GEMMs into one paired split-K launch

Adds a paired launch in which the answer-embedding GT GEMM and the shared (original image/question/z/gt-answer) GEMM run as a single k_main_fwd grid, each with its own split-K factor and a per-workgroup repetition count picked by a planner that balances the longest k-chain against the available CU slots. A combined vectorised fixup kernel reduces both slabs and applies the bias. Padded weight copies for the paired operands are folded into the existing prep/pack kernel via variable-row pack entries. The aim is to remove separate launches and tail underutilisation for these two small GEMMs, at the cost of extra slab traffic, a larger workspace, and more complex pack indexing.

```diff
diff --git a/include/neuralcx.h b/include/neuralcx.h
--- a/include/neuralcx.h
+++ b/include/neuralcx.h
@@ -378,6 +378,7 @@
 #define NCX_QUERY_FUSED_ADAM 33
 #define NCX_QUERY_FWD_ROUTE 34
 #define NCX_QUERY_BF16_ROUTE 35
+#define NCX_QUERY_GTSH_PAIR 36
 int ncx_profile_begin(uint32_t gemm_mask , int32_t max_launches);
 int ncx_profile_end(float* ms, int32_t* ids, int32_t cap);
 int ncx_profile_stamps(unsigned long long* stamps, int64_t words);
diff --git a/vqa-counterexamples_amd/csrc/ncx_diag.hip b/vqa-counterexamples_amd/csrc/ncx_diag.hip
--- a/vqa-counterexamples_amd/csrc/ncx_diag.hip
+++ b/vqa-counterexamples_amd/csrc/ncx_diag.hip
@@ -101,6 +101,15 @@
         out6[0] = b.nt_form; out6[1] = b.tn8; out6[2] = b.S; out6[3] = b.chunk; out6[4] = b.nz; out6[5] = b.vec;
         return NCX_OK;
     }
+    if (gemm_id == NCX_QUERY_GTSH_PAIR) {
+        const StepRoutes r = routes(*d);
+        SideStream* ss = side_stream();
+        out6[0] = r.gtsh_pair(*d, ss && ss->mode != 3) ? 1 : 0;
+        out6[1] = r.pair_s_gt; out6[2] = r.pair_s_sh;
+        out6[3] = r.pair_w_gt; out6[4] = r.pair_w_sh;
+        out6[5] = 3 * num_cus();
+        return NCX_OK;
+    }
     if (gemm_id == NCX_QUERY_FWD_ROUTE) {
         const StepRoutes r = routes(*d);
         GemmUse u[U_COUNT];
diff --git a/vqa-counterexamples_amd/csrc/ncx_forward.hip b/vqa-counterexamples_amd/csrc/ncx_forward.hip
--- a/vqa-counterexamples_amd/csrc/ncx_forward.hip
+++ b/vqa-counterexamples_amd/csrc/ncx_forward.hip
@@ -10,9 +10,12 @@
     else { for (int j = 0; j < valid; ++j) p[j] = f32_to_bf16(v[j]); }
 }
 
-struct PackArgs { const float* src[WPAD_N + 1]; float* dst[WPAD_N + 1]; long long lds[WPAD_N + 1]; int cols[WPAD_N + 1], ldd[WPAD_N + 1], zero_from[WPAD_N + 1]; int n, H; int nprep; };
+constexpr int PACK_N = WPAD_N + 1 + PAIR_WPAD_N;
+struct PackArgs { const float* src[PACK_N]; float* dst[PACK_N]; long long lds[PACK_N]; int cols[PACK_N], ldd[PACK_N], zero_from[PACK_N], first[PACK_N + 1]; int n; int nprep; };
 __device__ __forceinline__ void pack_rows_block(const PackArgs& a, int idx) {
-    const int h = idx % a.H, e = idx / a.H;
+    int e = 0;
+    while (e + 1 < a.n && idx >= a.first[e + 1]) ++e;
+    const int h = idx - a.first[e];
     float* drow = a.dst[e] + (long long)h * a.ldd[e];
     if (a.src[e]) {
         const float* srow = a.src[e] + (long long)h * a.lds[e];
@@ -265,18 +268,35 @@
     const bool bf16 = d.flags & NCX_F_BF16;
     u16* xc = bf16 ? (u16*)(ws + w.xc) : nullptr;
     struct { const float* ptr[WPAD_N]; int width[WPAD_N]; } wp{};
-    PackArgs pk{}; pk.H = H;
+    const bool pair = r.gtsh_pair(d, ss != nullptr);
+    struct { const float* ptr[PAIR_WPAD_N]; int width[PAIR_WPAD_N]; } pw{};
+    PackArgs pk{};
+    auto pack = [&](const float* src, long long lds, int cols, float* dst, int ldd, int zero_from, int rows) {
+        const int e = pk.n++;
+        pk.src[e] = src; pk.lds[e] = lds; pk.cols[e] = cols; pk.dst[e] = dst; pk.ldd[e] = ldd; pk.zero_from[e] = zero_from; pk.first[e + 1] = pk.first[e] + rows;
+    };
     {
         const float* srcs[WPAD_N] = {p->w1 + o.v_other, p->w1 + o.v_mult, p->w1 + o.v_dist, p->w1 + o.z_other, p->w1 + o.a_other, p->w2, p->w3};
         float* cur = (float*)(ws + w.wpad);
         for (int i = 0; i < WPAD_N; ++i) {
             wp.width[i] = wpad_width(d, i); wp.ptr[i] = cur;
             if (!wp.width[i]) continue;
-            const int e = pk.n++;
-            pk.src[e] = srcs[i]; pk.lds[e] = (i == 5 || i == 6) ? H : din; pk.cols[e] = wpad_cols(d, i); pk.dst[e] = cur; pk.ldd[e] = wp.width[i]; pk.zero_from[e] = pk.cols[e];
+            pack(srcs[i], (i == 5 || i == 6) ? H : din, wpad_cols(d, i), cur, wp.width[i], wpad_cols(d, i), H);
             cur += (size_t)H * wp.width[i];
         }
-        if (aemb && w.ldgt > d.A) { const int e = pk.n++; pk.src[e] = nullptr; pk.dst[e] = gt; pk.ldd[e] = w.ldgt; pk.zero_from[e] = d.A; pk.cols[e] = 0; }
+        if (aemb && w.ldgt > d.A) pack(nullptr, 0, 0, gt, w.ldgt, d.A, H);
+        if (pair) {
+            const float* psrc[PAIR_WPAD_N] = {p->w1 + o.v_orig, p->w1 + o.q_emb, p->w1 + o.z_orig, p->w1 + o.a_gt, p->answer_embedding};
+            const int pcols[PAIR_WPAD_N] = {d.dv, d.dq, d.dz, d.da, d.da};
+            float* pcur = (float*)(ws + w.pwpad);
+            for (int i = 0; i < PAIR_WPAD_N; ++i) {
+                const int rows = i == 4 ? d.A : H;
+                pw.width[i] = pair_wpad_width(d, r, i); pw.ptr[i] = pcur;
+                if (!pw.width[i]) continue;
+                pack(psrc[i], i == 4 ? d.da : din, pcols[i], pcur, pw.width[i], pcols[i], rows);
+                pcur += (size_t)rows * pw.width[i];
+            }
+        }
         if (d.flags & NCX_F_REUSE_GT) pk.n = 0;
     }
     const FwdRoute fr = forward_route(d, r);
@@ -285,7 +305,7 @@
     if (dist_in_main) dprep.flags |= NCX_F_PRIV_DIST_IN_MAIN;
     if (!do_rest) pk.n = 0;
     pk.nprep = do_pre ? (int)cdiv(M, 4) : 0;
-    const unsigned prep_grid = (unsigned)(pk.nprep + (long long)H * pk.n);
+    const unsigned prep_grid = (unsigned)(pk.nprep + (long long)pk.first[pk.n]);
     if (prep_grid > 0) {
         if (d.dv <= 2048 && d.A <= 2048)
             hipLaunchKernelGGL(k_prep<true>, dim3(prep_grid), dim3(256), 0, s, dprep, *in, idx_k, idx_o, idx_ob, mx, inv, misc, xc, bf16_cols(d), pk);
@@ -301,6 +321,27 @@
     FixupArgs fix_gt{}, fix_sh{};
     const bool merge_fix = !ss && !bf16 && aemb && !(d.flags & NCX_F_REUSE_GT) && u[U_GT].plan.cfg == u[U_SH].plan.cfg &&
                            !hook_env("NCX_NO_MERGE_FIX");
+    if (pair) {
+        auto seg = [&](MainArgs& a, int i, int kind, const float* x, long long lda, int klen, const int* idx, int slot, const float* wgt, long long ldb) {
+            MainSeg& g = a.seg[i]; g.kind = kind; g.a = x; g.lda = lda; g.idx = idx; g.klen = klen;
+            if (slot >= 0 && pw.width[slot]) { g.b = pw.ptr[slot]; g.ldb = pw.width[slot]; } else { g.b = wgt; g.ldb = ldb; } };
+        float* const pslab = (float*)(ws + w.slab2);
+        const size_t gt_elems = (size_t)r.pair_s_gt * H * d.A, sh_elems = (size_t)r.pair_s_sh * d.B * H;
+        if ((gt_elems + sh_elems) * 4 > w.slab2_bytes) return NCX_E_WORKSPACE;
+        MainArgs ag{}; ag.M = H; ag.N = d.A; ag.nseg = 4;
+        seg(ag, 0, MK_GATHER, nullptr, 0, 0, nullptr, -1, nullptr, 0);
+        seg(ag, 1, MK_PLAIN, p->w1 + o.a_other, din, d.da, nullptr, 4, p->answer_embedding, d.da);
+        seg(ag, 2, MK_PLAIN, nullptr, 0, 0, nullptr, -1, nullptr, 0);
+        seg(ag, 3, MK_GATHER, nullptr, 0, 0, nullptr, -1, nullptr, 0);
+        ag.out = gt; ag.ldo = w.ldgt; ag.split = r.pair_s_gt; ag.slab = pslab;
+        MainArgs as{}; as.M = d.B; as.N = H; as.nseg = 4;
+        seg(as, 0, MK_GATHER, in->feats, d.dv, d.dv, idx_ob, 0, p->w1 + o.v_orig, din);
+        seg(as, 1, MK_PLAIN, in->q_emb, d.dq, d.dq, nullptr, 1, p->w1 + o.q_emb, din);
+        seg(as, 2, MK_PLAIN, in->z_orig, d.dz, d.dz, nullptr, 2, p->w1 + o.z_orig, din);
+        seg(as, 3, MK_GATHER, p->answer_embedding, d.da, d.da, in->answer_aids, 3, p->w1 + o.a_gt, din);
+        as.out = sh; as.ldo = H; as.split = r.pair_s_sh; as.slab = pslab + gt_elems; as.epi.bias = p->b1;
+        rc = profiled(U_SH, s, [&] { return main_forward_pair(ag, as, r.pair_s_gt / r.pair_w_gt, r.pair_s_sh / r.pair_w_sh, s); }); if (rc) return rc;
+    } else
     if (aemb && bf16 && !(d.flags & NCX_F_REUSE_GT)) {
         const Bf16Emb m = bf16_emb_layout(d, ws + w.bf_emb);
         rc = bf16_pack_embedding(d, p->answer_embedding, p->w1, m, s2); if (rc) return rc;
@@ -315,7 +356,7 @@
                       merge_fix ? w.slab2_bytes : slab_side_bytes, nullptr, s2);
         if (rc) return rc;
     }
-    {
+    if (!pair) {
         GemmArgs a{}; a.mode = MODE_CHAIN; a.nseg = 4; a.M = d.B;
         a.a[0] = ss ? x_gather_strided(in->feats, d.dv, in->img_idx, d.K + 1, d.B, d.dv)
                     : x_gather(in->feats, d.dv, idx_ob, d.B, d.dv);
diff --git a/vqa-counterexamples_amd/csrc/ncx_internal.h b/vqa-counterexamples_amd/csrc/ncx_internal.h
--- a/vqa-counterexamples_amd/csrc/ncx_internal.h
+++ b/vqa-counterexamples_amd/csrc/ncx_internal.h
@@ -70,6 +70,7 @@
     size_t km_slab;
     size_t mslab, mslab_bytes;
     size_t wpad;
+    size_t pwpad;
     int ldm;
     int ldgt;
     size_t total;
@@ -105,6 +106,7 @@
 int main_chain_form(long long M, long long N, long long T, int split, bool single_gather, bool wide_ok);
 int main_forward_adam(MainArgs& a, bool rowmap, hipStream_t s);
 int main_adam_passengers();
+int main_forward_pair(const MainArgs& gt, const MainArgs& sh, int reps_gt, int reps_sh, hipStream_t s);
 int main_forward_mlb(MainArgs& a, hipStream_t s);
 int main_split(long long M, long long N, long long T);
 int main_fold_rows_eff(long long M, long long N, int rowdiv);
diff --git a/vqa-counterexamples_amd/csrc/ncx_main.h b/vqa-counterexamples_amd/csrc/ncx_main.h
--- a/vqa-counterexamples_amd/csrc/ncx_main.h
+++ b/vqa-counterexamples_amd/csrc/ncx_main.h
@@ -12,12 +12,15 @@
 template <int V> struct IntC { static constexpr int value = V; };
 
 constexpr int MF6_P = 80;
+struct MainPairArgs { MainArgs p[2]; int wg0, reps[2]; };
 template <int BM_, int BN_, int WGM_, int WGN_, int DEPTH_, int OCC_, int T_ = MF_T, bool X6_ = false>
 struct MainCfg {
+    typedef MainArgs KArgs;
     static constexpr int BM = BM_, BN = BN_, WGM = WGM_, WGN = WGN_, DEPTH = DEPTH_, OCC = OCC_, T = T_;
     static constexpr bool X6 = X6_;
     static constexpr int EPI = 0;
     static constexpr bool ADAM = false;
+    static constexpr bool PAIR = false;
     static constexpr int RP = T / 8;
     static constexpr int BM_LDS = (BM + RP - 1) / RP * RP;
     static constexpr int LDS6 = 2 * 3 * (BM_LDS + BN) * MF6_P;
@@ -34,13 +37,24 @@
 template <class CFG> struct WithMlbEpi : CFG { static constexpr int EPI = EPI_MLB; };
 template <class CFG> struct WithRowMap : CFG { static constexpr int EPI = EPI_ROWMAP; };
 template <class CFG> struct WithAdam : CFG { static constexpr bool ADAM = true; };
+template <class CFG> struct WithPair : CFG { static constexpr bool PAIR = true; typedef MainPairArgs KArgs; };
 
 typedef const __attribute__((address_space(1))) float* gfptr;
 typedef const __attribute__((address_space(1))) int* giptr;
 typedef const __attribute__((address_space(1))) f32x4u* gf4ptr;
 
+__device__ __forceinline__ const MainArgs& main_args_of(const MainArgs& a, int&, int&) { return a; }
+__device__ __forceinline__ const MainArgs& main_args_of(const MainPairArgs& pa, int& wg, int& reps) {
+    const int sel = wg >= pa.wg0 ? 1 : 0;
+    wg -= sel ? pa.wg0 : 0;
+    reps = pa.reps[sel];
+    return pa.p[sel];
+}
+
 template <class CFG, bool DIST, int K0, int K1 = -1, int K2 = -1, int K3 = -1, int K4 = -1>
-__global__ __launch_bounds__(CFG::T, CFG::OCC) void k_main_fwd(const MainArgs args) {
+__global__ __launch_bounds__(CFG::T, CFG::OCC) void k_main_fwd(const typename CFG::KArgs kargs) {
+    int wg = blockIdx.x, reps = 1;
+    const MainArgs& args = main_args_of(kargs, wg, reps);
     constexpr bool VFOLD = K0 == MK_VFOLD;
     constexpr int DIST_SEG = VFOLD ? 1 : 2;
     static_assert(!DIST || (VFOLD ? K1 == MK_PLAIN : (K1 == MK_GATHER_MUL && K2 == MK_PLAIN)), "DIST: v_o, v_k segment followed by the dist | rank segment");
@@ -64,7 +78,7 @@
     const int M = args.M, N = args.N;
     const int tiles_m = (M + BM - 1) / BM, tiles_n = (N + BN - 1) / BN;
     const int S = args.split > 1 ? args.split : 1;
-    int bid = blockIdx.x;
+    int bid = wg;
     if constexpr (CFG::ADAM) {
         const int pa = args.adam.pass_at, np = args.adam.n_pass;
         if (bid >= pa && bid < pa + np) { adam_passenger(args.adam, bid - pa, tid, MT); return; }
@@ -72,8 +86,10 @@
     }
     const int id = bid, xcd = id & 7, local = id >> 3;
     const int tn = local % tiles_n, unit = (local / tiles_n) * 8 + xcd;
-    if (unit >= tiles_m * S) return;
-    const int tm = unit / S, z = unit - tm * S;
+    int wpt = S;
+    if constexpr (CFG::PAIR) wpt = S / reps;
+    if (unit >= tiles_m * wpt) return;
+    const int tm = unit / wpt, z0 = (unit - tm * wpt) * (CFG::PAIR ? reps : 1);
     const int m0 = tm * BM, n0 = tn * BN;
     const int quad = tid & 7, trow = tid >> 3;
     unsigned long long* const stamps = args.stamps ? args.stamps + (size_t)blockIdx.x * 16 : nullptr;
@@ -83,6 +99,9 @@
     if (stamps && tid == 0) { stamps[14] = __builtin_amdgcn_s_memrealtime(); stamps[13] = __builtin_amdgcn_s_getreg((3 << 11) | (0 << 6) | 20); }
     stamp(0);
 
+    int rep = 0;
+    do {
+    const int z = z0 + rep;
     f32x4 acc[WM][WN];
 #pragma unroll
     for (int i = 0; i < WM; ++i)
@@ -917,9 +936,10 @@
     static_assert(BM * SP * 4 <= CFG::LDS, "the staged tile lies inside the launch's LDS (MainCfg::LDS_STAGE)");
     constexpr int QR = BN / 4;
     const EpiArgs& e = args.epi;
-    float* const dst = S > 1 ? args.slab + (long long)z * M * N : args.out;
-    const long long ldd = S > 1 ? (long long)N : args.ldo;
-    const bool plain = CFG::ADAM || S > 1 || !(e.rowadd || e.bias || e.relu || e.dropout || e.gate);
+    const bool to_slab = CFG::PAIR || S > 1;
+    float* const dst = to_slab ? args.slab + (long long)z * M * N : args.out;
+    const long long ldd = to_slab ? (long long)N : args.ldo;
+    const bool plain = CFG::ADAM || to_slab || !(e.rowadd || e.bias || e.relu || e.dropout || e.gate);
     auto item = [&](int f, int& r, int& n, int& nl) __attribute__((always_inline)) {
         const int rr = f / QR, cq = f - rr * QR;
         r = m0 + rr; n = n0 + 4 * cq;
@@ -1038,18 +1058,29 @@
 #pragma unroll 1
         for (int f = tid; f < BM * QR; f += MT) piece(f, 0);
     }
+    if constexpr (CFG::PAIR) __syncthreads();
+    } while (CFG::PAIR && ++rep < reps);
     stamp(8);
     if (stamps && tid == 0) stamps[15] = __builtin_amdgcn_s_memrealtime();
 }
 
-__global__ __launch_bounds__(256) void k_main_fixup(const MainArgs a) {
-    const int M = a.M, N = a.N, S = a.split;
+template <bool VEC>
+__device__ __forceinline__ void main_fixup_body(const MainArgs& a, const int block, const int S) {
+    const int M = a.M, N = a.N;
     const int nq = (N + 3) / 4;
-    const long long i = (long long)blockIdx.x * 256 + threadIdx.x;
+    const long long i = (long long)block * 256 + threadIdx.x;
     if (i >= (long long)M * nq) return;
     const int r = (int)(i / nq), n0 = (int)(i - (long long)r * nq) * 4;
     float v[4] = {0.f, 0.f, 0.f, 0.f};
     const long long mn = (long long)M * N, off = (long long)r * N + n0;
+    if (VEC && (N & 3) == 0) {
+#pragma unroll 4
+        for (int z = 0; z < S; ++z) {
+            const f32x4 w = *(const f32x4u*)(a.slab + z * mn + off);
+#pragma unroll
+            for (int j = 0; j < 4; ++j) v[j] += w[j];
+        }
+    } else
     for (int z = 0; z < S; ++z)
 #pragma unroll
         for (int j = 0; j < 4; ++j) if (n0 + j < N) v[j] += a.slab[z * mn + off + j];
@@ -1060,6 +1091,12 @@
         if (n >= N) break;
         a.out[(long long)r * a.ldo + n] = apply_epilogue(e, v[j], r, n, N);
     }
+}
+__global__ __launch_bounds__(256) void k_main_fixup(const MainArgs a) { main_fixup_body<false>(a, (int)blockIdx.x, a.split); }
+__global__ __launch_bounds__(256) void k_main_fixup_pair(const MainPairArgs pa, const int blocks0) {
+    const int sel = (int)blockIdx.x >= blocks0 ? 1 : 0;
+    const MainArgs& a = pa.p[sel];
+    main_fixup_body<true>(a, (int)blockIdx.x - (sel ? blocks0 : 0), a.split > 1 ? a.split : 1);
 }
 
 static inline bool main_fwd_operand_ok(int klen) { return klen >= 4 && klen % 4 == 0; }
@@ -1157,6 +1194,44 @@
 
 
 template <class CFG>
+static inline int launch_main_fwd_pair(MainPairArgs& pa, hipStream_t s) {
+    static_assert(CFG::PAIR && sizeof(MainPairArgs) <= 4096, "the pair form; its arguments fit the kernel-argument segment");
+    long long wgs[2], blocks[2];
+    for (int q = 0; q < 2; ++q) {
+        const MainArgs& a = pa.p[q];
+        if (a.nseg != 4 || a.M < 1 || a.N < 1) return NCX_E_DIMS;
+        if (a.seg[0].kind != MK_GATHER || a.seg[1].kind != MK_PLAIN || a.seg[2].kind != MK_PLAIN || a.seg[3].kind != MK_GATHER) return NCX_E_FLAGS;
+        if (!a.slab || !a.out) return NCX_E_WORKSPACE;
+        const EpiArgs& e = a.epi;
+        if (a.dist_out || a.stamps || e.rowadd || e.relu || e.dropout || e.gate) return NCX_E_FLAGS;
+        const bool lone = a.seg[0].klen == 0 && a.seg[2].klen == 0 && a.seg[3].klen == 0;
+        long long T = 0;
+        for (int i = 0; i < 4; ++i) {
+            if (lone && i != 1) continue;
+            if (!main_fwd_operand_ok(a.seg[i].klen)) return NCX_E_DIMS;
+            if (a.seg[i].kind == MK_GATHER && !a.seg[i].idx) return NCX_E_NULL;
+            T += (a.seg[i].klen + MF_BK - 1) / MF_BK;
+        }
+        const long long S = a.split > 1 ? a.split : 1;
+        const long long R = pa.reps[q];
+        if (S > T || R < 1 || S % R) return NCX_E_DIMS;
+        const long long tiles_m = (a.M + CFG::BM - 1) / CFG::BM, tiles_n = (a.N + CFG::BN - 1) / CFG::BN;
+        wgs[q] = ((tiles_m * (S / R) + 7) / 8) * 8 * tiles_n;
+        blocks[q] = ((long long)a.M * ((a.N + 3) / 4) + 255) / 256;
+    }
+    if (wgs[0] + wgs[1] > (1ll << 30) || blocks[0] + blocks[1] > (1ll << 30)) return NCX_E_DIMS;
+    pa.wg0 = (int)wgs[0];
+    constexpr int lds = CFG::LDS;
+    static DevMask attr{0};
+    NCX_HIP_TRY(set_max_lds_once(attr, (const void*)k_main_fwd<CFG, false, MK_GATHER, MK_PLAIN, MK_PLAIN, MK_GATHER>, lds));
+    hipLaunchKernelGGL((k_main_fwd<CFG, false, MK_GATHER, MK_PLAIN, MK_PLAIN, MK_GATHER>), dim3((unsigned)(wgs[0] + wgs[1])), dim3(CFG::T), lds, s, pa);
+    NCX_HIP_TRY(hipGetLastError());
+    hipLaunchKernelGGL(k_main_fixup_pair, dim3((unsigned)(blocks[0] + blocks[1])), dim3(256), 0, s, pa, (int)blocks[0]);
+    NCX_HIP_TRY(hipGetLastError());
+    return NCX_OK;
+}
+
+template <class CFG>
 static inline int launch_main_fwd_adam(MainArgs& a, int n_pass, int pass_at_hint, hipStream_t s) {
     static_assert(CFG::ADAM && CFG::EPI != EPI_MLB && !CFG::X6, "the answer-embedding gradient's forms");
     if (a.nseg != 2 || a.M < 1 || a.N < 1 || a.split > 1 || a.dist_out || !a.out) return NCX_E_FLAGS;
diff --git a/vqa-counterexamples_amd/csrc/ncx_main.hip b/vqa-counterexamples_amd/csrc/ncx_main.hip
--- a/vqa-counterexamples_amd/csrc/ncx_main.hip
+++ b/vqa-counterexamples_amd/csrc/ncx_main.hip
@@ -75,6 +75,20 @@
     return rowmap ? launch_main_fwd_adam<WithAdam<WithRowMap<MainCfg3>>>(a, np, at, s) : launch_main_fwd_adam<WithAdam<MainCfg3>>(a, np, at, s);
 }
 
+int main_forward_pair(const MainArgs& gt, const MainArgs& sh, int reps_gt, int reps_sh, hipStream_t s) {
+    auto steps = [](const MainArgs& a, int reps) {
+        long long T = 0;
+        for (int i = 0; i < a.nseg; ++i) T += (a.seg[i].klen + MF_BK - 1) / MF_BK;
+        const long long S = a.split > 1 ? a.split : 1, W = S / (reps > 0 ? reps : 1);
+        return (T + W - 1) / (W > 0 ? W : 1);
+    };
+    MainPairArgs pa{};
+    const bool gt_first = steps(gt, reps_gt) >= steps(sh, reps_sh);
+    pa.p[0] = gt_first ? gt : sh; pa.p[1] = gt_first ? sh : gt;
+    pa.reps[0] = gt_first ? reps_gt : reps_sh; pa.reps[1] = gt_first ? reps_sh : reps_gt;
+    return launch_main_fwd_pair<WithPair<MainCfg3>>(pa, s);
+}
+
 int main_forward_mlb(MainArgs& a, hipStream_t s) {
     const long long tiles96 = (long long)((a.M + 95) / 96) * ((a.N + 127) / 128);
     if (tiles96 * 10 >= (long long)num_cus() * 9) return launch_main_fwd<WithMlbEpi<MainCfg2>>(a, s);
diff --git a/vqa-counterexamples_amd/csrc/ncx_plan.h b/vqa-counterexamples_amd/csrc/ncx_plan.h
--- a/vqa-counterexamples_amd/csrc/ncx_plan.h
+++ b/vqa-counterexamples_amd/csrc/ncx_plan.h
@@ -17,7 +17,13 @@
     bool de_skip;
     long long cand_ksteps;
     bool dw1ak_on_tn8(bool side) const { return tn8 && emb_nt && !side; }
+    bool pair_ok; int pair_s_gt, pair_s_sh, pair_w_gt, pair_w_sh;
+    bool gtsh_pair(const ncx_dims& d, bool side) const { return pair_ok && !(d.flags & NCX_F_REUSE_GT) && !side; }
 };
+struct PairPlan { int s_gt, s_sh, w_gt, w_sh; long long tiles_gt, tiles_sh, t_gt, t_sh, slots; };
+PairPlan plan_gtsh_pair(const ncx_dims& d, const StepRoutes& r);
+constexpr int PAIR_WPAD_N = 5;
+int pair_wpad_width(const ncx_dims& d, const StepRoutes& r, int i);
 StepRoutes routes(const ncx_dims& d);
 struct FwdRoute { bool vfold, dist_in_fold, dist_in_main; };
 FwdRoute forward_route(const ncx_dims& d, const StepRoutes& r);
diff --git a/vqa-counterexamples_amd/csrc/ncx_plan.hip b/vqa-counterexamples_amd/csrc/ncx_plan.hip
--- a/vqa-counterexamples_amd/csrc/ncx_plan.hip
+++ b/vqa-counterexamples_amd/csrc/ncx_plan.hip
@@ -90,7 +90,52 @@
     r.emb_nt = aemb && !bf16 && !hook_env("NCX_NO_EMB_NT");
     r.de_skip = r.emb_nt && d.A <= NCX_PERM_MAX_A && !hook_env("NCX_NO_DE_SKIP");
     r.cand_ksteps = ksteps(d.dv) * ((d.flags & NCX_F_V_MULT) ? 2 : 1) + ksteps(d.K + 1) + ksteps(d.dz) + ksteps(aemb ? d.A : d.da);
+    r.pair_s_gt = r.pair_s_sh = 1; r.pair_w_gt = r.pair_w_sh = 0;
+    r.pair_ok = false;
+    if (aemb && !bf16 && d.dv % 4 == 0 && d.dq % 4 == 0 && d.dz % 4 == 0 && d.da % 4 == 0 && main_fwd_extents_ok(d) &&
+        (long long)d.B * d.dq * 4 < (1ll << 32) - 65536 && !hook_env("NCX_NO_GTSH_PAIR")) {
+        const PairPlan p = plan_gtsh_pair(d, r);
+        r.pair_s_gt = p.s_gt; r.pair_s_sh = p.s_sh; r.pair_w_gt = p.w_gt; r.pair_w_sh = p.w_sh;
+        r.pair_ok = p.w_gt > 0 && (p.s_gt > 1 || p.s_sh > 1);
+    }
     return r;
+}
+
+PairPlan plan_gtsh_pair(const ncx_dims& d, const StepRoutes& r) {
+    PairPlan p{};
+    const long long tm_gt = cdiv(d.H, 64), tn_gt = cdiv(d.A, 64), tm_sh = cdiv(d.B, 64), tn_sh = cdiv(d.H, 64);
+    p.tiles_gt = tm_gt * tn_gt; p.t_gt = ksteps(d.da);
+    p.tiles_sh = tm_sh * tn_sh; p.t_sh = ksteps(d.dv) + ksteps(d.dq) + ksteps(d.dz) + ksteps(d.da);
+    p.slots = 3ll * num_cus();
+    p.s_gt = p.s_sh = 1; p.w_gt = p.w_sh = 0;
+    GemmUse u[U_COUNT];
+    list_uses(d, r, u);
+    if (u[U_GT].plan.cfg != CFG_64x64 || u[U_SH].plan.cfg != CFG_64x64) return p;
+    p.s_gt = u[U_GT].plan.split > 1 ? u[U_GT].plan.split : 1;
+    p.s_sh = u[U_SH].plan.split > 1 ? u[U_SH].plan.split : 1;
+    if (p.s_gt > p.t_gt || p.s_sh > p.t_sh) return p;
+    if (const char* e = hook_env("NCX_PAIR_WPT")) {
+        int wg = 0, ws = 0;
+        if (sscanf(e, "%d,%d", &wg, &ws) == 2 && wg >= 1 && ws >= 1 && p.s_gt % wg == 0 && p.s_sh % ws == 0) { p.w_gt = wg; p.w_sh = ws; }
+        return p;
+    }
+    const long long xcd_slots = p.slots / 8;
+    long long best_work = -1, best_long = 0;
+    for (long long wg = 1; wg <= p.s_gt; ++wg)
+        for (long long ws = 1; ws <= p.s_sh; ++ws) {
+            if (p.s_gt % wg || p.s_sh % ws) continue;
+            const long long n_gt = cdiv(tm_gt * wg, 8) * tn_gt, n_sh = cdiv(tm_sh * ws, 8) * tn_sh;
+            if (n_gt + n_sh > xcd_slots) continue;
+            const long long cg = cdiv(p.t_gt, wg), cs = cdiv(p.t_sh, ws), lng = cg > cs ? cg : cs;
+            const long long work = n_gt * cg + n_sh * cs;
+            if (best_work < 0 || lng < best_long || (lng == best_long && work < best_work)) { best_work = work; best_long = lng; p.w_gt = (int)wg; p.w_sh = (int)ws; }
+        }
+    return p;
+}
+
+int pair_wpad_width(const ncx_dims& d, const StepRoutes& r, int i) {
+    const int c[PAIR_WPAD_N] = {d.dv, d.dq, d.dz, d.da, d.da};
+    return (!r.pair_ok || c[i] % 32 == 0) ? 0 : pad_to(c[i], 32);
 }
 
 int dw1c_seg_split(long long cols, int S, long long ksteps) {
@@ -226,6 +271,8 @@
         if (u[U_SH].slab_elems > s2) s2 = u[U_SH].slab_elems;
         if (u[U_DW1AK].slab_elems > s2) s2 = u[U_DW1AK].slab_elems;
         if (u[U_DE].slab_elems > s2) s2 = u[U_DE].slab_elems;
+        const long long pair = r.pair_ok ? (long long)r.pair_s_gt * d.H * d.A + (long long)r.pair_s_sh * d.B * d.H : 0;
+        if (pair > s2) s2 = pair;
         w.slab2_bytes = (size_t)s2 * 4;
         w.slab2 = take(w.slab2_bytes);
     }
@@ -247,6 +294,11 @@
         w.dpre_bf = take(bf16_dpre_bytes(d)); w.bf_slab = take(bf16_slab_bytes(d));
         w.bf_emb = take(bf16_emb_bytes(d));
     }
+    {
+        size_t e = 0;
+        for (int i = 0; i < PAIR_WPAD_N; ++i) e += (size_t)(i == 4 ? d.A : d.H) * pair_wpad_width(d, r, i);
+        w.pwpad = take(e * 4);
+    }
     w.total = off;
     return w;
 }
diff --git a/vqa-counterexamples_amd/neuralcx/_lib.py b/vqa-counterexamples_amd/neuralcx/_lib.py
--- a/vqa-counterexamples_amd/neuralcx/_lib.py
+++ b/vqa-counterexamples_amd/neuralcx/_lib.py
@@ -412,6 +412,9 @@
 BF16_NT_FORMS = {0: "128x128", 1: "64x128", 2: "128x64", 3: "64x64", 8: "nt8"}
 
 
+NCX_QUERY_GTSH_PAIR = 36
+
+
 def bf16_layout(d):
     out = (C.c_int32 * 10)()
     check(lib().ncx_bf16_layout(C.byref(d), out), "ncx_bf16_layout")
@@ -431,6 +434,9 @@
         return dict(engine=out[0], engine_name=FWD_ENGINES[out[0]], tile=out[1],
                     tile_name=FWD_CHAIN_FORMS[out[1]] if out[0] == 1 else ("%dx64" % out[1] if out[0] == 2 else None),
                     split=out[2], dist_in_main=bool(out[3]), hidden_engine=out[4], hidden_split=out[5])
+    if name == "GTSH_PAIR":
+        check(lib().ncx_plan_query(C.byref(d), NCX_QUERY_GTSH_PAIR, out), "ncx_plan_query")
+        return dict(taken=bool(out[0]), s_gt=out[1], s_sh=out[2], w_gt=out[3], w_sh=out[4], slots=out[5])
     if name == "FUSED_ADAM":
         check(lib().ncx_plan_query(C.byref(d), NCX_QUERY_FUSED_ADAM, out), "ncx_plan_query")
         return dict(fused=bool(out[0]), passengers=out[1])
```

Result: faster. 681,800 triplets/s, median of 6 (+2.2%).
